# traveller59/second.pytorch

Measured on AMD Instinct MI355X. Metric: frames/sec VoxelNet fwd (car.fhd, ~16k active voxels), higher is better.
Workload: dtype bf16; 1 GPU; car.fhd.config VoxelNet forward (voxelise+VFE+SpMiddleFHD+RPNV2+rotated NMS), inference, batch=8 synthetic KITTI clouds/GPU (17000 pts, 16000 voxels each), random-init weights, inputs resident in HBM; parallelism=frame-dp1, launch_mode=graph, graph_branches=1, steps_in_flight=4, rpn_segments_serialized=True, rulebook_numbering=sorted, points_per_frame=17000

## Files before the change

include/second_hip.h:

```cpp
#ifndef SECOND_HIP_H
#define SECOND_HIP_H

#include <stddef.h>
#include <stdint.h>

#ifdef __cplusplus
extern "C" {
#endif

#define SEC_OK 0
#define SEC_E_INVALID -1
#define SEC_E_WORKSPACE -2
#define SEC_E_UNSUPPORTED -3
#define SEC_E_LAUNCH -4

#define SEC_F32 0
#define SEC_F16 1
#define SEC_BF16 2

#define SEC_ABI_VERSION 9
int sec_abi_version(void);
int sec_tensors_checksum(const void *const *h_ptrs, const long long *h_nbytes, int count, unsigned long long *sums, void *stream);
const char *sec_last_error(void);
const char *sec_last_kernel_name(void);

size_t sec_voxelize_workspace_bytes(int num_points, int batch, int max_voxels, int max_points);
int sec_simple_voxel_f32(const float *voxels, const int *num_points, int n, const int *num_dev, int max_points, int num_features,
                         int mean_features, void *mean, int mean_dtype, void *stream);
int sec_rows_differ_f32(const float *a, long long rows, const float *b, long long n, int *flag, void *stream);
int sec_voxelize_encode_f32(const float *points, const int *point_offsets, int num_points, int num_features,
                            int batch, const float *h_range6, const float *h_voxel_size3, int max_points,
                            int max_voxels, int cap_mode, float *voxels, int *coors,
                            int *num_points_per_voxel, int *voxel_offsets, void *mean, int mean_features,
                            int mean_dtype, int encoder, int out_pitch, void *workspace, size_t workspace_bytes, void *stream);
int sec_simple_voxel_radius_f32(const float *voxels, const int *num_points, int n, const int *num_dev, int max_points, int num_features,
                                int mean_features, void *out, int out_pitch, int out_dtype, void *stream);
int sec_voxelize_f32(const float *points, const int *point_offsets, int num_points, int num_features,
                     int batch, const float *h_range6, const float *h_voxel_size3, int max_points,
                     int max_voxels, int cap_mode, float *voxels, int *coors,
                     int *num_points_per_voxel, int *voxel_offsets, void *mean, int mean_features,
                     int mean_dtype, void *workspace, size_t workspace_bytes, void *stream);

size_t sec_rulebook_workspace_bytes(int n_in, int kvol, int max_out_per_in);


int sec_rulebook_subm3d(const int *indices, int n_in, const int *n_in_dev, int batch,
                        const int *h_shape3, const int *h_ksize3, const int *h_dilation3, int *nbr_out,
                        int *pairs, int *pair_num, void *workspace, size_t workspace_bytes,
                        void *stream);

int sec_rulebook_subm3d_after_conv(const int *indices, int n_in, const int *n_in_dev, int batch,
                                   const int *h_shape3, const int *h_ksize3, const int *h_dilation3,
                                   int *nbr_out, const void *conv_workspace, size_t conv_workspace_bytes,
                                   int conv_n_in, const int *h_conv_ksize3, const int *h_conv_stride3,
                                   const int *h_conv_dilation3, int conv_out_per_in_hint, void *stream);

int sec_rulebook_subm3d_after_voxelize(const int *indices, int n_in, const int *n_in_dev, int batch,
                                       const int *h_shape3, const int *h_ksize3, const int *h_dilation3,
                                       int *nbr_out, const void *vox_workspace, size_t vox_workspace_bytes,
                                       int vox_num_points, int vox_max_voxels, int vox_max_points,
                                       const int *h_vox_grid3_zyx, void *stream);

int sec_rulebook_conv3d_build(const int *indices, int n_in, const int *n_in_dev, int batch,
                              const int *h_in_shape3,
                              const int *h_out_shape3, const int *h_ksize3, const int *h_stride3,
                              const int *h_padding3, const int *h_dilation3, int *out_indices,
                              int out_cap, int *num_out, int out_per_in_hint, int *prefill_nbr_out,
                              int prefill_nbr_out_rows, int *prefill_nbr_in, void *workspace,
                              size_t workspace_bytes, void *stream);
int sec_rulebook_conv3d_tables(int n_in, const int *h_ksize3, const int *h_stride3,
                               const int *h_dilation3, int out_per_in_hint, int *nbr_out,
                               int nbr_out_rows, int *nbr_in, int prefilled, int *pairs, int *pair_num,
                               void *workspace, size_t workspace_bytes, void *stream);
size_t sec_rulebook_sorted_workspace_bytes(int n_in, int kvol, int batch, const int *h_out_shape3);
int sec_rulebook_conv3d_build_sorted(const int *indices, int n_in, const int *n_in_dev, int batch,
                                     const int *h_in_shape3, const int *h_out_shape3, const int *h_ksize3,
                                     const int *h_stride3, const int *h_padding3, const int *h_dilation3,
                                     int *out_indices, int out_cap, int *num_out, int *prefill_nbr_out,
                                     int prefill_nbr_out_rows, int *prefill_nbr_in,
                                     int *prefill_extra, long long prefill_extra_words,
                                     const void *in_sites_workspace, size_t in_sites_workspace_bytes,
                                     void *workspace, size_t workspace_bytes, void *stream);
int sec_rulebook_conv3d_tables_sorted(const int *indices, int n_in, const int *n_in_dev, int batch,
                                      const int *h_in_shape3, const int *h_out_shape3, const int *h_ksize3,
                                      const int *h_stride3, const int *h_padding3, const int *h_dilation3,
                                      int *nbr_out, int nbr_out_rows, int *nbr_in, int prefilled, int *out_indices,
                                      int out_cap, int *pairs, int *pair_num, void *workspace,
                                      size_t workspace_bytes, void *stream);
int sec_rulebook_subm3d_after_conv_sorted(const int *indices, int n_in, const int *n_in_dev, int batch,
                                          const int *h_shape3, const int *h_ksize3, const int *h_dilation3,
                                          int *nbr_out, int prefilled, const void *conv_workspace,
                                          size_t conv_workspace_bytes, void *stream);
void sec_conv_output_shape(const int *h_in_shape3, const int *h_ksize3, const int *h_stride3,
                           const int *h_padding3, const int *h_dilation3, int *h_out_shape3);

size_t sec_packed_weight_bytes(int kvol, int cin, int cout, int dtype);
size_t sec_packed_weight_x3_bytes(int kvol, int cin, int cout);
int sec_pack_conv_weight(const void *weight, int kvol, int cin, int cout, int dtype, void *packed,
                         void *stream);
int sec_indice_conv_fwd(const void *features, int n_in, int cin, const void *weight,
                        const void *packed_weight, int kvol, int cout, const int *nbr_out, int n_out,
                        const int *num_out_dev, const float *scale, const float *shift, int relu,
                        void *out, int dtype, int out_dtype, void *stream);
int sec_indice_conv_fwd_plan(int cin, int cout, int kvol, int n_out, int dtype, int out_dtype, int has_packed);
int sec_indice_conv_set_variant(int variant);
#define SEC_FP32_SPLIT16 0
#define SEC_FP32_EXACT 1
int sec_set_fp32_mode(int mode);
int sec_get_fp32_mode(void);
size_t sec_indice_conv_bwd_workspace_bytes(int kvol, int cin, int cout, int dtype);
int sec_indice_conv_bwd(const void *features, int n_in, int cin, const void *weight, int kvol, int cout,
                        const int *nbr_out, const int *nbr_in, int n_out, const void *dout,
                        void *dfeat, float *dweight, int dtype, void *workspace, size_t workspace_bytes,
                        const void *packed_dgrad, int dweight_zeroed, void *stream);
int sec_pack_conv_weight_train(const float *weight, int kvol, int cin, int cout, int subm, int dtype, void *weight16,
                               void *packed_fwd, void *packed_dgrad, float *zero_dweight, void *stream);
int sec_pack_conv_weight_train_multi(int n, const float *const *weights, const int *kvol, const int *cin, const int *cout,
                                     const int *subm, int dtype, void *const *weight16, void *const *packed_fwd,
                                     void *const *packed_dgrad, float *const *zero_dweight, void *stream);

int sec_sparse_to_dense(const void *features, const int *indices, int n, int c, const int *num_dev,
                        void *out, size_t out_elems, int64_t stride_b, int64_t stride_c,
                        int64_t stride_z, int64_t stride_y, int64_t stride_x, int dtype, void *stream);

int sec_sparse_site_map(const int *indices, int n, const int *num_dev, int batch, int d, int h, int w,
                        int *site_map, void *stream);
int sec_sparse_site_map_sorted(const void *conv_workspace, size_t conv_workspace_bytes, const int *num_dev, int rows_cap,
                               int batch, int d, int h, int w, int *site_map, void *stream);
size_t sec_rulebook_chain_workspace_bytes(int batch, int levels, const int *h_shapes);
int sec_rulebook_chain_sorted(const int *indices0, int n0, const int *n0_dev, int batch, int levels, const int *h_shapes,
                              const int *h_ksize, const int *h_stride, const int *h_pad, const int *h_out_cap,
                              int *const *h_nbr_out, int *const *h_out_indices, int *const *h_num_out,
                              int *const *h_subm_nbr, const void *vox_workspace, size_t vox_workspace_bytes,
                              int vox_num_points, int vox_max_voxels, int vox_max_points, const int *h_vox_grid3_zyx,
                              int *site_map, void *workspace, size_t workspace_bytes, void *stream);
int sec_conv2d_nhwc_gather(const void *features, long long feature_rows, const int *site_map, int batch, int h,
                           int w, const void *packed_weight, const float *bias, int cout, int relu,
                           const unsigned short *tile_order, const int *live_counts, const void *background, void *y,
                           int dtype, void *stream);

int sec_conv2d_nhwc_into(const void *x, int batch, int h, int w, int cin, const void *packed_weight, const float *bias, int cout,
                         int ksize, int stride, int pad, int relu, void *y, int y_channels, int y_channel_offset, int dtype, void *stream);

int sec_conv2d_nhwc_rows(const void *rows, long long feature_rows, const int *site_map, int batch, int h, int w, int cin,
                         const void *packed_weight, const float *bias, int cout, int ksize, int stride, int pad, int relu, void *y,
                         int dtype, void *stream);

size_t sec_rpn_tile_live_workspace_bytes(int batch, int h, int w);
int sec_rpn_tile_live(const int *site_map, int batch, int h, int w, int layers, unsigned short *tile_order, int *live_counts,
                      void *workspace, size_t workspace_bytes, void *stream);
int sec_conv2d_nhwc_tiles(const void *x, int batch, int h, int w, const void *packed_weight, const float *bias, int cout,
                          int relu, const unsigned short *tile_order, const int *live_counts, const void *background, void *y,
                          int dtype, void *stream);
int sec_conv1x1_chain_nhwc_tiles(const void *x, int batch, int h, int w, const void *packed_w1, const float *bias1, int relu1,
                                 const void *packed_w2, const float *bias2, int cout2, const unsigned short *tile_order,
                                 const int *live_counts, const void *background, void *y, int dtype, void *stream);
#define SEC_CHAIN_X_LIVE_ONLY 2
int sec_rpn_tile_live_masks(const int *site_map, int batch, int h, int w, int layers, unsigned short *tile_order, int *live_counts,
                            unsigned short *nbr_masks, void *workspace, size_t workspace_bytes, void *stream);
int sec_conv2d_nhwc_tiles_lazy(const void *x, int batch, int h, int w, const void *packed_weight, const float *bias, int cout,
                               int relu, const unsigned short *tile_order, const int *live_counts, const void *background,
                               const unsigned short *nbr_masks, const void *background_in, void *y, int dtype, void *stream);
int sec_conv2d_nhwc_tiles_tail(const void *x, int batch, int h, int w, const void *packed_weight, const float *bias, int relu,
                               const unsigned short *tile_order, const int *live_counts, const unsigned short *nbr_masks,
                               const void *background_in, const void *packed_w1, const float *bias1, int relu1, const void *packed_w2,
                               const float *bias2, int cout2, void *y_heads, int dtype, void *stream);

size_t sec_rpn_tile_cover_lds_bytes(int h, int w, int layers);
int sec_rpn_tile_cover(const int *site_map, int batch, int h, int w, int layers, unsigned short *tile_order, int *live_counts,
                       unsigned short *cover_order, int *cover_counts, unsigned *cover_cols, unsigned *cover_halo, void *workspace,
                       size_t workspace_bytes, void *stream);
int sec_conv2d_nhwc_gather_cover(const void *features, long long feature_rows, const int *site_map, int batch, int h, int w,
                                 const void *packed_weight, const float *bias, int cout, int relu, const unsigned short *cover_order,
                                 const int *cover_counts, void *y, int dtype, void *stream);
int sec_conv2d_nhwc_tiles_cover(const void *x, int batch, int h, int w, const void *packed_weight, const float *bias, int cout,
                                int relu, const unsigned short *cover_order, const int *cover_counts, const unsigned *cover_halo,
                                const void *background_in, void *y, int dtype, void *stream);
int sec_conv2d_nhwc_tiles_tail_cover(const void *x, int batch, int h, int w, const void *packed_weight, const float *bias, int relu,
                                     const unsigned short *cover_order, const int *cover_counts, const unsigned *cover_halo,
                                     const void *background_in, const void *packed_w1, const float *bias1, int relu1,
                                     const void *packed_w2, const float *bias2, int cout2, void *y_heads, int dtype, void *stream);

int sec_dense_to_sparse(const void *dense, const int *indices, int n, int c, const int *num_dev, void *rows,
                        int64_t stride_b, int64_t stride_c, int64_t stride_z, int64_t stride_y,
                        int64_t stride_x, int dtype, void *stream);

int sec_pillar_scatter(const void *features, const int *coords, int p, int c, const int *num_dev,
                       void *out, size_t out_elems, int64_t stride_b, int64_t stride_c, int64_t stride_y,
                       int64_t stride_x, int dtype, void *stream);

int sec_pfn_fwd(const float *voxels, const int *num_points, const int *coords, int num_pillars,
                const int *num_dev, int max_points, int num_features, const float *weight_t,
                const float *scale, const float *shift, int channels, float vx, float vy,
                float x_offset, float y_offset, void *out, int out_dtype, void *stream);
int sec_pfn_fwd_slots(const float *points, const void *vox_workspace, size_t vox_workspace_bytes, int vox_num_points,
                      int vox_batch, int vox_max_voxels, int max_points, int num_features, const int *num_points_per_voxel,
                      const int *coords, int num_pillars, const int *num_dev, const float *weight_t, const float *scale,
                      const float *shift, int channels, float vx, float vy, float x_offset, float y_offset, void *out,
                      int out_dtype, void *stream);
int sec_pfn_radius_fwd(const float *voxels, const int *num_points, const int *coords, int num_pillars,
                       const int *num_dev, int max_points, int num_features, const float *weight_t,
                       const float *scale, const float *shift, int channels, float vx, float vy,
                       float x_offset, float y_offset, void *out, int out_dtype, void *stream);
int sec_pfn_radius_fwd_slots(const float *points, const void *vox_workspace, size_t vox_workspace_bytes, int vox_num_points,
                             int vox_batch, int vox_max_voxels, int max_points, int num_features, const int *num_points_per_voxel,
                             const int *coords, int num_pillars, const int *num_dev, const float *weight_t, const float *scale,
                             const float *shift, int channels, float vx, float vy, float x_offset, float y_offset, void *out,
                             int out_dtype, void *stream);

size_t sec_pfn_train_workspace_bytes(int num_pillars, int channels);
int sec_pfn_train_fwd(const float *voxels, const int *num_points, const int *coords, int num_pillars, int max_points,
                      int num_features, const float *weight_t, const float *gamma, const float *beta, float eps, float momentum,
                      float *running_mean, float *running_var, int channels, float vx, float vy, float x_offset, float y_offset,
                      float *out, signed char *argmax, float *stats, void *workspace, size_t workspace_bytes, void *stream);
int sec_pfn_train_bwd(const float *voxels, const int *num_points, const int *coords, int num_pillars, int max_points,
                      int num_features, const float *weight_t, const float *gamma, const float *stats, int channels, float vx,
                      float vy, float x_offset, float y_offset, const float *grad_out, const float *out, const signed char *argmax,
                      float *dweight_t, float *dgamma, float *dbeta, void *workspace, size_t workspace_bytes, void *stream);
// ... 306 lines not shown
```

second.pytorch_amd/csrc/indice_conv.hip:

```cpp
#include "common.hpp"
#include <stdlib.h>
#include <type_traits>

namespace sec {

template <typename T> struct Cvt;
template <> struct Cvt<float> {
    static __device__ __forceinline__ float to(float v) { return v; }
    static __device__ __forceinline__ float from(float v) { return v; }
};
template <> struct Cvt<__half> {
    static __device__ __forceinline__ float to(__half v) { return __half2float(v); }
    static __device__ __forceinline__ __half from(float v) { return __float2half_rn(v); }
};
template <> struct Cvt<__hip_bfloat16> {
    static __device__ __forceinline__ float to(__hip_bfloat16 v) { return __bfloat162float(v); }
    static __device__ __forceinline__ __hip_bfloat16 from(float v) { return __float2bfloat16(v); }
};

__device__ __forceinline__ float epilogue(float v, const float *scale, const float *shift, int c, int relu) {
    if (scale) v = __fmul_rn(v, scale[c]);
    if (shift) v = __fadd_rn(v, shift[c]);
    if (relu) v = v > 0.0f ? v : 0.0f;
    return v;
// ... 412 lines not shown
    static constexpr int ASLOT = 32 * LPR, BSLOT = BPIECES * 64;
    static constexpr int RING = 3;
};

typedef float f32x2p __attribute__((ext_vector_type(2)));
template <typename T> __device__ __forceinline__ unsigned pack2_16(float a, float b);
template <> __device__ __forceinline__ unsigned pack2_16<__hip_bfloat16>(float a, float b) {
    typedef __bf16 bf16x2p __attribute__((ext_vector_type(2)));
    const f32x2p v = {a, b};
    return __builtin_bit_cast(unsigned, __builtin_convertvector(v, bf16x2p));
}
template <> __device__ __forceinline__ unsigned pack2_16<__half>(float a, float b) {
    typedef _Float16 f16x2p __attribute__((ext_vector_type(2)));
    const f32x2p v = {a, b};
    return __builtin_bit_cast(unsigned, __builtin_convertvector(v, f16x2p));
}

template <typename T, int COUT, bool FUSED>
__device__ __forceinline__ void rows_store_impl(f32x16 (&acc)[(COUT + 31) / 32], T *__restrict__ out, long long row, bool valid, int h,
                                                const float *__restrict__ aff, bool has_scale, bool has_shift, int relu) {
    if (FUSED) { has_scale = has_shift = true; relu = 1; }
    constexpr int NT = (COUT + 31) / 32, NG = COUT >= 32 ? 4 : COUT / 8;
    static_assert(COUT % 16 == 0, "whole 16-byte runs per half-wave pair");
    T *orow = out + (size_t)row * COUT;
    float4 sc4[NT][NG], sh4[NT][NG];
#pragma unroll
    for (int t = 0; t < NT; ++t)
#pragma unroll
        for (int g = 0; g < NG; ++g) {
            const int c = t * 32 + 8 * g + 4 * h;
            if (has_scale) sc4[t][g] = *reinterpret_cast<const float4 *>(aff + c);
            if (has_shift) sh4[t][g] = *reinterpret_cast<const float4 *>(aff + COUT + c);
        }
#pragma unroll
    for (int t = 0; t < NT; ++t) {
        unsigned lo[NG], hi[NG];
#pragma unroll
        for (int g = 0; g < NG; ++g) {
            const float sc[4] = {sc4[t][g].x, sc4[t][g].y, sc4[t][g].z, sc4[t][g].w};
            const float sh[4] = {sh4[t][g].x, sh4[t][g].y, sh4[t][g].z, sh4[t][g].w};
            float v4[4];
#pragma unroll
            for (int j = 0; j < 4; ++j) v4[j] = epilogue_v(acc[t][4 * g + j], sc[j], sh[j], has_scale, has_shift, relu);
            lo[g] = pack2_16<T>(v4[0], v4[1]);
            hi[g] = pack2_16<T>(v4[2], v4[3]);
        }
#pragma unroll
        for (int pr = 0; pr < NG / 2; ++pr) {
            const auto sx = __builtin_amdgcn_permlane32_swap(lo[2 * pr], lo[2 * pr + 1], false, false);
            const auto sy = __builtin_amdgcn_permlane32_swap(hi[2 * pr], hi[2 * pr + 1], false, false);
            if (valid) *reinterpret_cast<uint4 *>(orow + t * 32 + 8 * (2 * pr + h)) = make_uint4(sx[0], sy[0], sx[1], sy[1]);
        }
    }
}
template <typename T, int COUT>
__device__ __forceinline__ void rows_store(f32x16 (&acc)[(COUT + 31) / 32], T *__restrict__ out, long long row, bool valid, int h,
                                           const float *__restrict__ aff, bool has_scale, bool has_shift, int relu) {
    if (has_scale && has_shift && relu) rows_store_impl<T, COUT, true>(acc, out, row, valid, h, aff, true, true, 1);
    else rows_store_impl<T, COUT, false>(acc, out, row, valid, h, aff, has_scale, has_shift, relu);
}

template <int COUT>
__device__ __forceinline__ void rows_stage_affine(float *aff, const float *__restrict__ scale, const float *__restrict__ shift) {
    const int c = threadIdx.x;
    if (c < COUT) {
        if (scale) aff[c] = scale[c];
        if (shift) aff[COUT + c] = shift[c];
    }
}

#ifdef SEC_CONV_TIMELINE
#define SEC_RTL(...) __VA_ARGS__
#else
#define SEC_RTL(...)
#endif

#ifdef SEC_CONV_EXPERIMENTS
#include "../../tools/kernel_experiments/indice_conv_rows_ab.inc"
#endif

typedef unsigned int u32x4_t __attribute__((ext_vector_type(4)));
constexpr int kBalWgs = 256;
enum : int {
    kFlStage = 1, kFlPipe = 2, kFlSkew = 32, kFlAllW = 64, kFlLazy = 128, kFlWin3 = 512, kFlBal = 2048, kFlXsh = 8192,
    kFlAblNoGather = 4, kFlAblFewLines = 8, kFlAblOneLine = 16, kFlAblNoWeights = 4096,
};
#if defined(__HIP_DEVICE_COMPILE__) && defined(SEC_PACKED_F32_EXEMPTION)
#define SEC_PACKED_F32_OK __attribute__((target("packed-fp32-ops")))
#else
#define SEC_PACKED_F32_OK
#endif
template <int CTRL> __device__ __forceinline__ int rows_lane_shift(int v) {
    return __builtin_amdgcn_mov_dpp(v, CTRL, 0xf, 0xf, true);
}
constexpr int kDppWaveShl1 = 0x130, kDppWaveShr1 = 0x138;
template <bool LEFT> __device__ __forceinline__ bool rows_xshare(int t, int c, int r) {
    const int n = rows_lane_shift<LEFT ? kDppWaveShr1 : kDppWaveShl1>(c);
    return t >= 0 && t == n && (LEFT ? r > 0 : r < 31);
}
template <typename T, int CIN, int COUT, int KVOL, int DIST, int WAVES, int MINW, int FL>
SEC_PACKED_F32_OK __global__ __launch_bounds__(WAVES * 64, MINW) void k_conv_rows_buf(const T *__restrict__ feat, long long feat_bytes,
                                                                   const T *__restrict__ packed, const int *__restrict__ nbr,
                                                                   int n_out, const int *__restrict__ num_out_dev,
                                                                   const float *__restrict__ scale, const float *__restrict__ shift,
                                                                   int relu, T *__restrict__ out) {
    using C = RowsCfg<T, CIN, COUT>;
    constexpr int NBW = (C::BPIECES + WAVES - 1) / WAVES;
    constexpr int ROWB = CIN * (int)sizeof(T);
    constexpr bool STAGE = (FL & kFlStage) != 0, PIPE = (FL & kFlPipe) != 0;
    constexpr bool ALLW = (FL & kFlAllW) != 0;
    constexpr bool LAZY = (FL & kFlLazy) != 0 && STAGE && !ALLW;
    constexpr bool SKEW = (FL & kFlSkew) != 0 && WAVES == 8 && PIPE;
    const bool early = SKEW && __builtin_amdgcn_readfirstlane((int)threadIdx.x >> 8) != 0;
    constexpr int TBL16 = 32 * KVOL / 4;
    static_assert(NBW >= 1 && NBW <= 2, "one or two weight pieces per wave");
    static_assert(C::KS <= 4, "up to four 16-channel k-steps per row");
    static_assert(!STAGE || (32 * KVOL) % 4 == 0, "tile table in whole 16-byte pieces");
    static_assert(!ALLW || (STAGE && PIPE), "the all-weights form stages its tables and double-buffers its B fragments");
    constexpr bool WIN3 = (FL & kFlWin3) != 0;
    constexpr bool XSH = (FL & kFlXsh) != 0 && STAGE && KVOL == 27 && DIST >= 3 && (ALLW || (WIN3 && LAZY));
    static_assert(!WIN3 || (STAGE && !PIPE && !ALLW && KVOL % 3 == 0 && DIST <= 3), "window form: non-pipelined, 3 offsets per window");
    constexpr int LBUF = ALLW ? (KVOL * C::BSLOT > WAVES * TBL16 ? KVOL * C::BSLOT : WAVES * TBL16) : 1;
    __shared__ __attribute__((aligned(16))) uint4 lbuf[LBUF];
    __shared__ __attribute__((aligned(16))) uint4 bring[ALLW ? 1 : (WIN3 ? 6 : 3)][ALLW ? 1 : C::BSLOT];
    __shared__ __attribute__((aligned(16))) float aff[2 * COUT];
    __shared__ __attribute__((aligned(16))) u32x4_t stage[(STAGE && !ALLW) ? WAVES : 1][(STAGE && !ALLW) ? TBL16 : 1];
    rows_stage_affine<COUT>(aff, scale, shift);
    const int n_cap = n_out;
    if (num_out_dev) n_out = *num_out_dev;
    const int lane = threadIdx.x & 63, w = threadIdx.x >> 6;
    const int r = lane & 31, h = lane >> 5;
    constexpr bool BAL = (FL & kFlBal) != 0;
    int rw = 32;
    if constexpr (BAL) {
        const int per_wg = (n_out + kBalWgs - 1) / kBalWgs;
        rw = ((per_wg + WAVES - 1) / WAVES + 3) & ~3;
        rw = rw < 4 ? 4 : (rw > 32 ? 32 : rw);
    }
    int bid = blockIdx.x;
    if (relu & 0x10000) {
        const int nact = (int)(((long long)n_out + rw * WAVES - 1) / (rw * WAVES));
        const int per = (nact + 7) >> 3;
        bid = (bid & 7) * per + (bid >> 3);
        if ((int)(blockIdx.x >> 3) >= per) return;
    }
    relu &= 1;
    if ((long long)bid * (rw * WAVES) >= n_out) return;
    const long long row = (long long)bid * (rw * WAVES) + w * rw + r;
    const bool valid = row < n_out && r < rw;
    SEC_RTL(long long *tl = g_timeline; long long tl0 = 0, tl1 = 0, tl2 = 0; if (tl) tl0 = clock64();)
    const __amdgpu_buffer_rsrc_t rsrc = __builtin_amdgcn_make_buffer_rsrc(const_cast<T *>(feat), 0, (int)feat_bytes, 0x00020000);
    const int piece0 = (w * NBW) % C::BPIECES;
    const u32x4_t *wpv = reinterpret_cast<const u32x4_t *>(packed) + (size_t)piece0 * 64 + lane;
    unsigned off[KVOL];
    unsigned shm = 0;
    if constexpr (STAGE) {
        const long long tile_row0 = (long long)bid * (rw * WAVES) + w * rw;
        const long long tbl_bytes = (long long)n_cap * KVOL * 4;
        const int *tile = nbr + tile_row0 * KVOL;
        const long long left = tbl_bytes - tile_row0 * KVOL * 4;
        const __amdgpu_buffer_rsrc_t trs = __builtin_amdgcn_make_buffer_rsrc(
            const_cast<int *>(left > 0 ? tile : nbr), 0, (int)(left <= 0 ? 0 : (left < 32 * KVOL * 4 ? left : 32 * KVOL * 4)), 0x00020000);
        u32x4_t *stg = ALLW ? reinterpret_cast<u32x4_t *>(lbuf) + w * TBL16 : &stage[w][0];
#pragma unroll
        for (int i = 0; i < (TBL16 + 63) / 64; ++i) {
            const int p16 = i * 64 + lane;
            if (p16 < TBL16) stg[p16] = __builtin_amdgcn_raw_buffer_load_b128(trs, p16 * 16, 0, 0);
        }
        __builtin_amdgcn_wave_barrier();
        const int *mine = reinterpret_cast<const int *>(stg) + r * KVOL;
        if constexpr (!LAZY) {
#pragma unroll
            for (int k = 0; k < KVOL; ++k) {
                int t = valid ? mine[k] : -1;
                if constexpr (XSH) {
                    if (k % 3 != 1) {
                        const int c = valid ? mine[k - k % 3 + 1] : -1;
                        if (k % 3 == 0 ? rows_xshare<true>(t, c, r) : rows_xshare<false>(t, c, r)) { shm |= 1u << (2 * (k / 3) + (k % 3) / 2); t = -1; }
                    }
                }
                off[k] = t >= 0 ? (unsigned)t * ROWB + h * 16 : 0x80000000u;
            }
        }
    } else {
        const int *nrow = nbr + (size_t)(valid ? row : 0) * KVOL;
#pragma unroll
        for (int k = 0; k < KVOL; ++k) {
            const int t = valid ? nrow[k] : -1;
            off[k] = t >= 0 ? (unsigned)t * ROWB + h * 16 : 0x80000000u;
        }
    }
#ifdef SEC_CONV_ABLATIONS
    if constexpr ((FL & kFlAblNoGather) != 0) {
#pragma unroll
        for (int k = 0; k < KVOL; ++k) off[k] = 0x80000000u;
    }
    if constexpr ((FL & kFlAblFewLines) != 0) {
#pragma unroll
        for (int k = 0; k < KVOL; ++k) off[k] = (unsigned)__shfl((int)off[k], lane & ~3, 64);
    }
    if constexpr ((FL & kFlAblOneLine) != 0) {
#pragma unroll
        for (int k = 0; k < KVOL; ++k) off[k] = h * 16;
    }
#endif
    SEC_RTL(if (tl) { cwait_vmcnt<0>(); tl1 = clock64(); })
    f32x16 acc[C::NT];
#pragma unroll
    for (int t = 0; t < C::NT; ++t)
#pragma unroll
        for (int i = 0; i < 16; ++i) acc[t][i] = 0.0f;
    u32x4_t areg[DIST][C::KS];
    auto afrag = [&](int k, int s) __attribute__((always_inline)) -> uint4 {
        u32x4_t a = areg[k % DIST][s];
        if constexpr (XSH) {
            if (k % 3 != 1) {
                const bool sh = ((shm >> (2 * (k / 3) + (k % 3) / 2)) & 1u) != 0;
                const u32x4_t c = areg[(k - k % 3 + 1) % DIST][s];
#pragma unroll
                for (int i = 0; i < 4; ++i) {
                    const int n = k % 3 == 0 ? rows_lane_shift<kDppWaveShr1>((int)c[i]) : rows_lane_shift<kDppWaveShl1>((int)c[i]);
                    a[i] = sh ? (unsigned)n : a[i];
                }
            }
        }
        return __builtin_bit_cast(uint4, a);
    };
#define SEC_XSH_REFILL(k, FETCH)                                                                                      \
    if constexpr (XSH) {                                                                                              \
        if ((k) % 3 == 0) { if ((k) + DIST < KVOL) FETCH((k) + DIST) }                                                \
        else if ((k) % 3 == 2) {                                                                                      \
            if ((k) - 1 + DIST < KVOL) FETCH((k) - 1 + DIST)                                                          \
            if ((k) + DIST < KVOL) FETCH((k) + DIST)                                                                  \
        }                                                                                                             \
    } else {                                                                                                          \
        if ((k) + DIST < KVOL) FETCH((k) + DIST)                                                                      \
    }
    if constexpr (ALLW) {
#define SEC_FETCH_A(k)                                                                                                \
    {                                                                                                                 \
        areg[(k) % DIST][0] = __builtin_amdgcn_raw_buffer_load_b128(rsrc, off[k], 0, 0);                              \
        if (C::KS > 1) areg[(k) % DIST][1 % C::KS] = __builtin_amdgcn_raw_buffer_load_b128(rsrc, off[k] + 32, 0, 0);  \
        if (C::KS > 2) areg[(k) % DIST][2 % C::KS] = __builtin_amdgcn_raw_buffer_load_b128(rsrc, off[k] + 64, 0, 0);  \
        if (C::KS > 3) areg[(k) % DIST][3 % C::KS] = __builtin_amdgcn_raw_buffer_load_b128(rsrc, off[k] + 96, 0, 0);  \
    }
#pragma unroll
        for (int k = 0; k < DIST && k < KVOL; ++k) SEC_FETCH_A(k)
        __syncthreads();
        {
            const uint4 *pk = reinterpret_cast<const uint4 *>(packed);
            for (int i = threadIdx.x; i < KVOL * C::BSLOT; i += WAVES * 64) lbuf[i] = pk[i];
        }
        __syncthreads();
        uint4 bf[2][C::KS * C::NT];
#pragma unroll
        for (int i = 0; i < C::KS * C::NT; ++i) bf[0][i] = lbuf[i * 64 + lane];
#pragma unroll
        for (int k = 0; k < KVOL; ++k) {
            if (k + 1 < KVOL) {
#pragma unroll
                for (int i = 0; i < C::KS * C::NT; ++i) bf[(k + 1) & 1][i] = lbuf[(k + 1) * C::BSLOT + i * 64 + lane];
            }
            __builtin_amdgcn_sched_barrier(0);
#pragma unroll
            for (int s = 0; s < C::KS; ++s) {
                const uint4 a = afrag(k, s);
#pragma unroll
                for (int t = 0; t < C::NT; ++t) acc[t] = Mfma<T>::run(bf[k & 1][s * C::NT + t], a, acc[t]);
            }
            __builtin_amdgcn_sched_barrier(0);
            SEC_XSH_REFILL(k, SEC_FETCH_A)
        }
#undef SEC_FETCH_A
        SEC_RTL(if (tl) tl2 = clock64();)
        rows_store<T, COUT>(acc, out, row, valid, h, aff, scale != nullptr, shift != nullptr, relu);
        return;
    }
    u32x4_t wr0[DIST], wr1[DIST];
    u32x4_t *bslot = reinterpret_cast<u32x4_t *>(&bring[0][piece0 * 64 + lane]);
    const int *lazy_tbl = reinterpret_cast<const int *>(&stage[(STAGE && !ALLW) ? w : 0][0]) + r * KVOL;
    auto off_of = [&](int k) -> unsigned {
        if constexpr (LAZY) {
            int t = valid ? lazy_tbl[k] : -1;
            if constexpr (XSH) {
                if (k % 3 != 1) {
                    const int c = valid ? lazy_tbl[k - k % 3 + 1] : -1;
                    if (k % 3 == 0 ? rows_xshare<true>(t, c, r) : rows_xshare<false>(t, c, r)) { shm |= 1u << (2 * (k / 3) + (k % 3) / 2); t = -1; }
                }
            }
#ifdef SEC_CONV_ABLATIONS
            if constexpr ((FL & kFlAblNoGather) != 0) return 0x80000000u;
            if constexpr ((FL & kFlAblOneLine) != 0) return t >= 0 ? (unsigned)(h * 16) : 0x80000000u;
#endif
            return t >= 0 ? (unsigned)t * ROWB + h * 16 : 0x80000000u;
        } else {
            return off[k];
        }
    };
#define SEC_FETCH(k)                                                                                                  \
    {                                                                                                                 \
        const unsigned o_ = off_of(k);                                                                                \
        wr0[(k) % DIST] = wpv[(size_t)(k) * C::BSLOT];                                                                \
        if (NBW > 1) wr1[(k) % DIST] = wpv[(size_t)(k) * C::BSLOT + 64];                                              \
        areg[(k) % DIST][0] = __builtin_amdgcn_raw_buffer_load_b128(rsrc, o_, 0, 0);                                  \
        if (C::KS > 1) areg[(k) % DIST][1 % C::KS] = __builtin_amdgcn_raw_buffer_load_b128(rsrc, o_ + 32, 0, 0);      \
        if (C::KS > 2) areg[(k) % DIST][2 % C::KS] = __builtin_amdgcn_raw_buffer_load_b128(rsrc, o_ + 64, 0, 0);      \
        if (C::KS > 3) areg[(k) % DIST][3 % C::KS] = __builtin_amdgcn_raw_buffer_load_b128(rsrc, o_ + 96, 0, 0);      \
    }
#define SEC_WPUT(k)                                                                                                   \
    {                                                                                                                 \
        bslot[((k) % 3) * C::BSLOT] = wr0[(k) % DIST];                                                                \
        if (NBW > 1) bslot[((k) % 3) * C::BSLOT + 64] = wr1[(k) % DIST];                                              \
    }
    if constexpr (!(WIN3 && XSH)) {
#pragma unroll
        for (int k = 0; k < DIST && k < KVOL; ++k) SEC_FETCH(k)
    }
    SEC_RTL(long long ts_wait = 0, ts_comp = 0, ts_issue = 0;)
    if constexpr (WIN3) {
        u32x4_t ww0[3], ww1[3];
#define SEC_GFETCH(k)                                                                                                 \
    {                                                                                                                 \
        const unsigned o_ = off_of(k);                                                                                \
        areg[(k) % DIST][0] = __builtin_amdgcn_raw_buffer_load_b128(rsrc, o_, 0, 0);                                  \
        if (C::KS > 1) areg[(k) % DIST][1 % C::KS] = __builtin_amdgcn_raw_buffer_load_b128(rsrc, o_ + 32, 0, 0);      \
        if (C::KS > 2) areg[(k) % DIST][2 % C::KS] = __builtin_amdgcn_raw_buffer_load_b128(rsrc, o_ + 64, 0, 0);      \
        if (C::KS > 3) areg[(k) % DIST][3 % C::KS] = __builtin_amdgcn_raw_buffer_load_b128(rsrc, o_ + 96, 0, 0);      \
    }
#ifdef SEC_CONV_ABLATIONS
#define SEC_WLOAD(g)                                                                                                  \
    {                                                                                                                 \
        _Pragma("unroll") for (int j_ = 0; j_ < 3; ++j_) {                                                            \
            if constexpr ((FL & kFlAblNoWeights) != 0) { ww0[j_] = u32x4_t{(unsigned)lane, 0u, 0u, 0u}; if (NBW > 1) ww1[j_] = ww0[j_]; }  \
            else {                                                                                                    \
            ww0[j_] = wpv[(size_t)(3 * (g) + j_) * C::BSLOT];                                                         \
            if (NBW > 1) ww1[j_] = wpv[(size_t)(3 * (g) + j_) * C::BSLOT + 64];                                       \
            }                                                                                                         \
        }                                                                                                             \
    }
#else
#define SEC_WLOAD(g)                                                                                                  \
    {                                                                                                                 \
        _Pragma("unroll") for (int j_ = 0; j_ < 3; ++j_) {                                                            \
            ww0[j_] = wpv[(size_t)(3 * (g) + j_) * C::BSLOT];                                                         \
            if (NBW > 1) ww1[j_] = wpv[(size_t)(3 * (g) + j_) * C::BSLOT + 64];                                       \
        }                                                                                                             \
    }
#endif
#define SEC_WSTORE(g)                                                                                                 \
    {                                                                                                                 \
        _Pragma("unroll") for (int j_ = 0; j_ < 3; ++j_) {                                                            \
            bslot[((((g) & 1) * 3) + j_) * C::BSLOT] = ww0[j_];                                                       \
            if (NBW > 1) bslot[((((g) & 1) * 3) + j_) * C::BSLOT + 64] = ww1[j_];                                     \
        }                                                                                                             \
    }
        SEC_WLOAD(0)
#pragma unroll
        for (int k = 0; k < DIST && k < KVOL; ++k) SEC_GFETCH(k)
        SEC_WSTORE(0)
        if (KVOL > 3) SEC_WLOAD(1)
#pragma unroll
        for (int g = 0; g < KVOL / 3; ++g) {
            __syncthreads();
#pragma unroll
            for (int j = 0; j < 3; ++j) {
                const int k = 3 * g + j;
                uint4 bf[C::KS * C::NT];
#pragma unroll
                for (int i = 0; i < C::KS * C::NT; ++i) bf[i] = bring[(g & 1) * 3 + j][i * 64 + lane];
                __builtin_amdgcn_sched_barrier(0);
#pragma unroll
                for (int s2 = 0; s2 < C::KS; ++s2) {
                    const uint4 a = afrag(k, s2);
#pragma unroll
                    for (int t = 0; t < C::NT; ++t) acc[t] = Mfma<T>::run(bf[s2 * C::NT + t], a, acc[t]);
                }
                __builtin_amdgcn_sched_barrier(0);
                SEC_XSH_REFILL(k, SEC_GFETCH)
            }
            if (g + 1 < KVOL / 3) {
                SEC_WSTORE(g + 1)
                if (g + 2 < KVOL / 3) SEC_WLOAD(g + 2)
            }
        }
#undef SEC_GFETCH
#undef SEC_WLOAD
#undef SEC_WSTORE
    } else if constexpr (!PIPE) {
        SEC_WPUT(0)
#pragma unroll
        for (int k = 0; k < KVOL; ++k) {
            SEC_RTL(long long s0 = 0, s1 = 0, s2 = 0; if (tl) s0 = clock64();)
            if (k + 1 < KVOL) SEC_WPUT(k + 1)
            __syncthreads();
            SEC_RTL(if (tl) s1 = clock64();)
            uint4 bf[C::KS * C::NT];
#pragma unroll
            for (int i = 0; i < C::KS * C::NT; ++i) bf[i] = bring[k % 3][i * 64 + lane];
            __builtin_amdgcn_sched_barrier(0);
#pragma unroll
            for (int s = 0; s < C::KS; ++s) {
                const uint4 a = __builtin_bit_cast(uint4, areg[k % DIST][s]);
#pragma unroll
                for (int t = 0; t < C::NT; ++t) acc[t] = Mfma<T>::run(bf[s * C::NT + t], a, acc[t]);
            }
            __builtin_amdgcn_sched_barrier(0);
            SEC_RTL(if (tl) s2 = clock64();)
            if (k + DIST < KVOL) SEC_FETCH(k + DIST)
            SEC_RTL(if (tl) { const long long s3 = clock64(); ts_wait += s1 - s0; ts_comp += s2 - s1; ts_issue += s3 - s2; })
        }
    } else {
        static_assert(!PIPE || DIST >= 3, "W[k+2] must have left the ring before its registers are refilled");
        uint4 bf[2][C::KS * C::NT];
        SEC_WPUT(0)
        if (KVOL > 1) SEC_WPUT(1)
        __syncthreads();
#pragma unroll
        for (int i = 0; i < C::KS * C::NT; ++i) bf[0][i] = bring[0][i * 64 + lane];
#pragma unroll
        for (int k = 0; k < KVOL; ++k) {
            if (k + 2 < KVOL) SEC_WPUT(k + 2)
            if (k + 1 < KVOL) {
                __syncthreads();
#pragma unroll
                for (int i = 0; i < C::KS * C::NT; ++i) bf[(k + 1) & 1][i] = bring[(k + 1) % 3][i * 64 + lane];
            }
            __builtin_amdgcn_sched_barrier(0);
            if constexpr (SKEW) {
                if (early && k >= 1 && k - 1 + DIST < KVOL) SEC_FETCH(k - 1 + DIST)
                __builtin_amdgcn_sched_barrier(0);
            }
#pragma unroll
            for (int s = 0; s < C::KS; ++s) {
                const uint4 a = __builtin_bit_cast(uint4, areg[k % DIST][s]);
#pragma unroll
                for (int t = 0; t < C::NT; ++t) acc[t] = Mfma<T>::run(bf[k & 1][s * C::NT + t], a, acc[t]);
            }
            __builtin_amdgcn_sched_barrier(0);
            if (!(SKEW && early) && k + DIST < KVOL) SEC_FETCH(k + DIST)
// ... 77 lines not shown
        const u32x4_t *wp = reinterpret_cast<const u32x4_t *>(packed) + lane;
        typedef unsigned int u32x2_t __attribute__((ext_vector_type(2)));
        u32x4_t bfr[7];
        u32x2_t lo[7], hi[7];
#pragma unroll
        for (int s = 0; s < 7; ++s) {
            bfr[s] = wp[s * 64];
            const int k0 = 4 * s + 2 * h, k1 = k0 + 1;
            const int t0 = valid ? mine[k0] : -1;
            const int t1 = (valid && k1 < KVOL) ? mine[k1 < KVOL ? k1 : 0] : -1;
            lo[s] = __builtin_amdgcn_raw_buffer_load_b64(rsrc, t0 >= 0 ? (unsigned)t0 * 8u : 0x80000000u, 0, 0);
            hi[s] = __builtin_amdgcn_raw_buffer_load_b64(rsrc, t1 >= 0 ? (unsigned)t1 * 8u : 0x80000000u, 0, 0);
        }
        f32x16 acc[1];
#pragma unroll
        for (int i = 0; i < 16; ++i) acc[0][i] = 0.0f;
#pragma unroll
        for (int s = 0; s < 7; ++s) {
            const uint4 a = make_uint4(lo[s].x, lo[s].y, hi[s].x, hi[s].y);
            acc[0] = Mfma<T>::run(__builtin_bit_cast(uint4, bfr[s]), a, acc[0]);
        }
        __syncthreads();
        rows_store<T, COUT>(acc, out, row, valid, h, aff, scale != nullptr, shift != nullptr, relu);
    } else {
        __syncthreads();
    }
}

enum ConvVariant : int {
    kVarWave = 0,
    kVarAuto = 1,
    kVarSks = 8,
    kVarRows = 22,
    kVarAutoPlain = 29,
    kVarF32Valu = 30,
    kVarF32Mfma = 31,
    kVarF32SplitUnpacked = 32,
    kVarWgradCompact = 41,
    kVarXshOffAuto = 80, kVarXshOnAuto = 81,
    kVarXshOffRows = 82, kVarXshOnRows = 83,
};
static int g_variant_override = -1;
static int g_fp32_mode = 0;

struct ConvSetting { int variant, xshare; };
static ConvSetting conv_setting() {
    switch (g_variant_override) {
    case kVarXshOffAuto: return {kVarAuto, 0};
    case kVarXshOnAuto: return {kVarAuto, 1};
    case kVarXshOffRows: return {kVarRows, 0};
    case kVarXshOnRows: return {kVarRows, 1};
    default: break;
    }
    static int env = -2;
    if (env == -2) { const char *e = getenv("SEC_CONV_XSHARE"); env = e ? (atoi(e) != 0) : -1; }
    return {g_variant_override < 0 ? kVarAuto : g_variant_override, env};
}
static int conv_variant() { return conv_setting().variant; }

enum { PLAN_GENERIC = 0, PLAN_TILED = 1, PLAN_C4 = 2, PLAN_MFMA_WAVE = 3, PLAN_MFMA_SK = 4, PLAN_MFMA_SKS = 5, PLAN_ROWS = 6,
       PLAN_ROWS_COMPACT = 7, PLAN_ROWS_TOUCH = 8, PLAN_ROWS_COMPACT_TOUCH = 9, PLAN_ROWS_REG = 10, PLAN_ROWS_BUF = 11, PLAN_C4_MFMA = 12, PLAN_ROWS_M2 = 13, PLAN_ROWS_LDS = 14, PLAN_ROWS_KS = 15, PLAN_EXPERIMENT = 99 };

#define SEC_MFMA_SHAPES(X) X(16, 16) X(16, 32) X(32, 32) X(32, 64) X(64, 64) X(64, 128) X(128, 128) X(16, 64) X(64, 32) X(32, 16) X(128, 64)
static bool mfma_shape(int cin, int cout) {
#define SEC_IS(CI, CO) if (cin == CI && cout == CO) return true;
    SEC_MFMA_SHAPES(SEC_IS)
#undef SEC_IS
    return false;
}

constexpr int kRowsMin = 40000, kRowsMinSmall = 8192;

constexpr bool rows_shape_narrow(int cin, int cout) { return (cin == 16 && (cout == 16 || cout == 32)) || (cin == 32 && cout == 32); }
constexpr bool rows_shape_wide(int cin, int cout) { return cin == 32 && cout == 64; }
constexpr bool rows_shape_64(int cin, int cout) { return cin == 64 && cout == 64; }
constexpr bool buf_shape(int cin, int cout, int kvol) {
    if (kvol == 3) return rows_shape_64(cin, cout);
    return kvol == 27 && (rows_shape_narrow(cin, cout) || rows_shape_wide(cin, cout) || rows_shape_64(cin, cout));
}
constexpr int kFlNarrow = kFlStage + kFlPipe + kFlAllW + kFlBal;
constexpr int kFlWide = kFlStage + kFlPipe + kFlBal;
constexpr int kFl64 = kFlStage + kFlLazy + kFlWin3 + kFlBal;
constexpr int kFl64K3 = kFlStage + kFlPipe;
static_assert(kFlNarrow == 2115 && kFlNarrow + kFlXsh == 10307 && kFlWide == 2051 && kFl64 == 2689 && kFl64 + kFlXsh == 10881 && kFl64K3 == 3,
              "the decimal FL values are part of the kernel names that tests and bench tables quote");
constexpr bool kXshare32 = true, kXshare64w8 = true, kXshare64w4 = false;
enum RowsForm : int { kRowsNone = 0, kRowsNarrow, kRowsNarrowXsh, kRowsWide, kRows64W8, kRows64W8Xsh, kRows64W4, kRows64W4Xsh, kRows64K3 };

static int rows_form(int cin, int cout, int kvol, bool mid, int xshare) {
    auto xsh = [&](bool dflt) { return xshare < 0 ? dflt : xshare != 0; };
    if (kvol == 3) return kRows64K3;
    if (rows_shape_narrow(cin, cout)) return cin == 32 && xsh(kXshare32) ? kRowsNarrowXsh : kRowsNarrow;
    if (rows_shape_wide(cin, cout)) return kRowsWide;
    if (mid) return xsh(kXshare64w4) ? kRows64W4Xsh : kRows64W4;
    return xsh(kXshare64w8) ? kRows64W8Xsh : kRows64W8;
}

struct ConvPlan { int id, form; };
#ifdef SEC_CONV_EXPERIMENTS
#include "../../tools/kernel_experiments/indice_conv_dispatch.inc"
#endif

static ConvPlan conv_fwd_decide(int cin, int cout, int kvol, int rows, bool same_dtype, bool has_packed, bool has_feat, long long feat_bytes,
                                int variant, int xshare) {
    const bool fits = feat_bytes < 0x7fffffffll;
    if (!has_packed) return {PLAN_GENERIC, kRowsNone};
    if (cin == 4 && cout == 16 && kvol == 27)
        return {same_dtype && variant != kVarAutoPlain && fits ? PLAN_C4_MFMA : PLAN_GENERIC, kRowsNone};
    if (!mfma_shape(cin, cout)) return {PLAN_GENERIC, kRowsNone};
    ConvPlan p = {PLAN_MFMA_SK, kRowsNone};
    if (variant == kVarSks || ((variant == kVarAuto || variant == kVarAutoPlain) && cout <= 32)) p.id = PLAN_MFMA_SKS;
    else if (variant == kVarWave) p.id = PLAN_MFMA_WAVE;
    if (same_dtype && has_feat && fits && buf_shape(cin, cout, kvol)) {
        const bool mid = rows_shape_64(cin, cout) && kvol == 27 && rows >= kRowsMinSmall && rows < kRowsMin;
        if (variant == kVarRows || (variant == kVarAuto && (rows >= kRowsMin || mid)))
            p = {PLAN_ROWS_BUF, rows_form(cin, cout, kvol, variant == kVarAuto && mid, xshare)};
    }
#ifdef SEC_CONV_EXPERIMENTS
    experiment_plan(cin, cout, kvol, rows, same_dtype, has_feat, fits, variant, xshare, &p);
#endif
    return p;
}
static ConvPlan conv_fwd_plan_now(int cin, int cout, int kvol, int rows, bool same_dtype, bool has_packed, bool has_feat, long long feat_bytes) {
    const ConvSetting cs = conv_setting();
    return conv_fwd_decide(cin, cout, kvol, rows, same_dtype, has_packed, has_feat, feat_bytes, cs.variant, cs.xshare);
}

template <typename T, int CIN, int COUT>
static bool launch_rows_form(int form, const void *feat, long long n_feat, const void *packed, const int *nbr, int n_out, const int *num_out_dev,
                             const float *scale, const float *shift, int relu, void *out, hipStream_t st) {
#define SEC_FORM(FORM, SHAPE, KV, D, W, M, FLG)                                                                                  \
    case FORM:                                                                                                                   \
        if constexpr (SHAPE) {                                                                                                   \
            launch_rows_buf<T, CIN, COUT, D, W, M, FLG, KV>(feat, n_feat, packed, nbr, n_out, num_out_dev, scale, shift, relu, out, st); \
            return true;                                                                                                         \
        }                                                                                                                        \
        break;
    switch (form) {
    SEC_FORM(kRowsNarrow, rows_shape_narrow(CIN, COUT), 27, 6, 8, 2, kFlNarrow)
    SEC_FORM(kRowsNarrowXsh, rows_shape_narrow(CIN, COUT) && CIN == 32, 27, 6, 8, 2, kFlNarrow + kFlXsh)
    SEC_FORM(kRowsWide, rows_shape_wide(CIN, COUT), 27, 4, 8, 2, kFlWide)
    SEC_FORM(kRows64W8, rows_shape_64(CIN, COUT), 27, 3, 8, 3, kFl64)
    SEC_FORM(kRows64W8Xsh, rows_shape_64(CIN, COUT), 27, 3, 8, 3, kFl64 + kFlXsh)
    SEC_FORM(kRows64W4, rows_shape_64(CIN, COUT), 27, 3, 4, 2, kFl64)
    SEC_FORM(kRows64W4Xsh, rows_shape_64(CIN, COUT), 27, 3, 4, 2, kFl64 + kFlXsh)
    SEC_FORM(kRows64K3, rows_shape_64(CIN, COUT), 3, 3, 8, 2, kFl64K3)
    default: break;
    }
#undef SEC_FORM
    return false;
}

template <typename T, typename OT, int CIN, int COUT>
static void launch_mfma(const ConvPlan &p, const void *feat, long long n_feat, const void *packed, const int *nbr, int n_out,
                        const int *num_out_dev, int kvol, const float *scale, const float *shift, int relu, void *out, hipStream_t st) {
#ifdef SEC_CONV_EXPERIMENTS
    if (experiment_launch<T, OT, CIN, COUT>(p, feat, n_feat, packed, nbr, n_out, num_out_dev, kvol, scale, shift, relu, out, st)) return;
#endif
    if constexpr (std::is_same<T, OT>::value && buf_shape(CIN, COUT, 27)) {
        if (p.id == PLAN_ROWS_BUF && launch_rows_form<T, CIN, COUT>(p.form, feat, n_feat, packed, nbr, n_out, num_out_dev, scale, shift, relu, out, st))
            return;
    }
    if (p.id == PLAN_MFMA_SKS) {
        hipLaunchKernelGGL((k_conv_mfma_sks<T, OT, CIN, COUT, 4>), dim3((div_up(n_out, 32) + 7) / 8 * 8, (COUT + 31) / 32),
                           dim3(256), 0, st, (const T *)feat, (const T *)packed, nbr, n_out, num_out_dev, kvol, scale, shift,
                           relu, (OT *)out);
        return;
    }
    if (p.id == PLAN_MFMA_WAVE) {
        constexpr int MT = 1;
        int rows_per_block = (kBlock / 64) * 32 * MT;
        hipLaunchKernelGGL((k_conv_mfma<T, OT, CIN, COUT, MT>), dim3(div_up(n_out, rows_per_block)), dim3(kBlock), 0, st,
                           (const T *)feat, (const T *)packed, nbr, n_out, num_out_dev, kvol, scale, shift, relu, (OT *)out);
        return;
    }
    constexpr int NW = 4;
    hipLaunchKernelGGL((k_conv_mfma_sk<T, OT, CIN, COUT, NW>), dim3((div_up(n_out, 32) + 7) / 8 * 8), dim3(NW * 64), 0, st,
                       (const T *)feat, (const T *)packed, nbr, n_out, num_out_dev, kvol, scale, shift,
                       relu | kReluXcdOrder, (OT *)out);
}

template <typename T, typename OT>
static bool dispatch_mfma(const ConvPlan &p, int cin, int cout, const void *feat, long long n_feat, const void *packed, const int *nbr,
                          int n_out, const int *num_out_dev, int kvol, const float *scale, const float *shift, int relu, void *out,
                          hipStream_t st) {
    if (p.id == PLAN_GENERIC || p.id == PLAN_C4_MFMA) return false;
#define SEC_CASE(CI, CO)                                                                                         \
    if (cin == CI && cout == CO) {                                                                               \
        launch_mfma<T, OT, CI, CO>(p, feat, n_feat, packed, nbr, n_out, num_out_dev, kvol, scale, shift, relu, out, st); \
        return true;                                                                                             \
    }
    SEC_MFMA_SHAPES(SEC_CASE)
#undef SEC_CASE
    return false;
}

template <int CIN, int COUT, int WAVES>
__global__ __launch_bounds__(WAVES * 64) void k_conv_rows_x3_f32(const float *__restrict__ feat, const float *__restrict__ w,
                                                                const int *__restrict__ nbr, int n_out, const int *__restrict__ num_out_dev,
                                                                int kvol, int w_t, int mirror, const float *__restrict__ scale,
                                                                const float *__restrict__ shift, int relu, float *__restrict__ out) {
    static_assert(CIN % 16 == 0 && COUT % 32 == 0, "16-channel k-steps, 32-column MFMA tiles");
    constexpr int KS = CIN / 16, NT = COUT / 32, ROWS = WAVES * 32, NTH = WAVES * 64;
    constexpr int PIECES = KS * NT * 64;
    constexpr int PPT = (PIECES + NTH - 1) / NTH;
    __shared__ __attribute__((aligned(16))) uint4 sB[2][2][PIECES];
    __shared__ int s_nbr[ROWS * 27];
    if (num_out_dev) n_out = *num_out_dev;
    const int tid = threadIdx.x, wave = tid >> 6, lane = tid & 63, r = lane & 31, h = lane >> 5;
    const long long base = (long long)blockIdx.x * ROWS;
    if (base >= n_out) return;
    {
        const long long lim = ((long long)n_out - base) * kvol;
        const int *src = nbr + base * kvol;
        for (int e = tid; e < ROWS * kvol; e += NTH) s_nbr[e] = e < lim ? src[e] : -1;
    }
    float wreg[PPT][8];
    auto load_w = [&](int k) {
        const float *wk = w + (size_t)(mirror ? kvol - 1 - k : k) * CIN * COUT;
#pragma unroll
        for (int q = 0; q < PPT; ++q) {
            const int p = q * NTH + tid;
            if (PIECES % NTH != 0 && p >= PIECES) break;
            const int l = p & 63, st = p >> 6, t = st % NT, sidx = st / NT;
            const int ci = sidx * 16 + (l >> 5) * 8, co = t * 32 + (l & 31);
            if (w_t) {
                const float4 a = *reinterpret_cast<const float4 *>(wk + (size_t)co * CIN + ci);
                const float4 b = *reinterpret_cast<const float4 *>(wk + (size_t)co * CIN + ci + 4);
                wreg[q][0] = a.x; wreg[q][1] = a.y; wreg[q][2] = a.z; wreg[q][3] = a.w;
                wreg[q][4] = b.x; wreg[q][5] = b.y; wreg[q][6] = b.z; wreg[q][7] = b.w;
            } else {
#pragma unroll
                for (int e = 0; e < 8; ++e) wreg[q][e] = wk[(size_t)(ci + e) * COUT + co];
            }
        }
    };
    auto split8 = [](const float (&v)[8], uint4 &hi, uint4 &lo) {
        const unsigned h0 = pack2_16<__hip_bfloat16>(v[0], v[1]), h1 = pack2_16<__hip_bfloat16>(v[2], v[3]);
        const unsigned h2 = pack2_16<__hip_bfloat16>(v[4], v[5]), h3 = pack2_16<__hip_bfloat16>(v[6], v[7]);
        hi = make_uint4(h0, h1, h2, h3);
        lo = make_uint4(pack2_16<__hip_bfloat16>(v[0] - __uint_as_float(h0 << 16), v[1] - __uint_as_float(h0 & 0xffff0000u)),
                        pack2_16<__hip_bfloat16>(v[2] - __uint_as_float(h1 << 16), v[3] - __uint_as_float(h1 & 0xffff0000u)),
                        pack2_16<__hip_bfloat16>(v[4] - __uint_as_float(h2 << 16), v[5] - __uint_as_float(h2 & 0xffff0000u)),
                        pack2_16<__hip_bfloat16>(v[6] - __uint_as_float(h3 << 16), v[7] - __uint_as_float(h3 & 0xffff0000u)));
    };
    auto store_w = [&](int buf) {
#pragma unroll
        for (int q = 0; q < PPT; ++q) {
            const int p = q * NTH + tid;
            if (PIECES % NTH != 0 && p >= PIECES) break;
            uint4 hi, lo;
            split8(wreg[q], hi, lo);
            sB[buf][0][p] = hi;
            sB[buf][1][p] = lo;
        }
    };
    load_w(0);
    store_w(0);
    f32x16 acc[NT];
#pragma unroll
    for (int t = 0; t < NT; ++t)
#pragma unroll
        for (int i = 0; i < 16; ++i) acc[t][i] = 0.0f;
    float4 a[2 * KS], an[2 * KS];
    auto gather = [&](int k, float4 (&dst)[2 * KS]) -> bool {
        const int idx = s_nbr[(wave * 32 + r) * kvol + k];
        const bool any = __ballot(idx >= 0) != 0ull;
        if (any) {
            const float4 *row = reinterpret_cast<const float4 *>(feat + (size_t)(idx >= 0 ? idx : 0) * CIN) + 2 * h;
#pragma unroll
            for (int sidx = 0; sidx < KS; ++sidx) {
                dst[2 * sidx] = idx >= 0 ? row[4 * sidx] : make_float4(0.0f, 0.0f, 0.0f, 0.0f);
// ... 782 lines not shown
    if (cin == CI && cout == CO) {                                                                                        \
        set_last_kernel("k_conv_wgrad_tiled<%s, %d, %d> chunk=%d", dtype_name<T>(), CI, CO, chunk);                       \
        hipLaunchKernelGGL((k_conv_wgrad_tiled<T, CI, CO>), grid, dim3(kBlock), 0, st, (const T *)feat, (const T *)dout, nbr,  \
                           n_out, kvol, chunk, dw);                                                                       \
        return true;                                                                                                      \
    }
    SEC_WG(4, 16) SEC_WG(16, 16) SEC_WG(16, 32) SEC_WG(32, 32) SEC_WG(32, 64) SEC_WG(64, 64) SEC_WG(64, 128) SEC_WG(128, 128)
#undef SEC_WG
    return false;
}

static size_t elt_size(int dtype) { return dtype == SEC_F32 ? 4 : 2; }

}

using namespace sec;

#ifdef SEC_CONV_TIMELINE
extern "C" __attribute__((visibility("default"))) int sec__debug_timeline(long long *buf) {
    return hipMemcpyToSymbol(HIP_SYMBOL(sec::g_timeline), &buf, sizeof(buf)) == hipSuccess ? 0 : -4;
}
#endif

SEC_API size_t sec_packed_weight_bytes(int kvol, int cin, int cout, int dtype) {
    if (dtype != SEC_F32 && cin == 4 && cout == 16 && kvol == 27) return (size_t)7 * 64 * 8 * elt_size(dtype);
    if (dtype == SEC_F32 || cin % 16 != 0 || kvol <= 0 || cout <= 0) return 0;
    return (size_t)kvol * cin * ((cout + 31) / 32) * 32 * elt_size(dtype);
}

SEC_API int sec_pack_conv_weight(const void *weight, int kvol, int cin, int cout, int dtype, void *packed, void *stream) {
    if (!weight || !packed || sec_packed_weight_bytes(kvol, cin, cout, dtype) == 0) return SEC_E_INVALID;
    hipStream_t st = (hipStream_t)stream;
    if (cin == 4) {
        if (dtype == SEC_BF16)
            hipLaunchKernelGGL(k_pack_weight_c4<__hip_bfloat16>, dim3(div_up(7 * 64 * 8, kBlock)), dim3(kBlock), 0, st,
                               (const __hip_bfloat16 *)weight, cout, (__hip_bfloat16 *)packed);
        else
            hipLaunchKernelGGL(k_pack_weight_c4<__half>, dim3(div_up(7 * 64 * 8, kBlock)), dim3(kBlock), 0, st, (const __half *)weight, cout,
                               (__half *)packed);
        return check_launch();
    }
    long long total = (long long)kvol * cin * ((cout + 31) / 32) * 32;
    if (dtype == SEC_BF16)
        hipLaunchKernelGGL(k_pack_weight<__hip_bfloat16>, dim3(div_up(total, kBlock)), dim3(kBlock), 0, st,
                           (const __hip_bfloat16 *)weight, kvol, cin, cout, (__hip_bfloat16 *)packed);
    else
        hipLaunchKernelGGL(k_pack_weight<__half>, dim3(div_up(total, kBlock)), dim3(kBlock), 0, st, (const __half *)weight,
                           kvol, cin, cout, (__half *)packed);
    return check_launch();
}

SEC_API int sec_set_fp32_mode(int mode) {
    if (mode != 0 && mode != 1) return SEC_E_INVALID;
    g_fp32_mode = mode;
    return SEC_OK;
}
SEC_API int sec_get_fp32_mode(void) { return g_fp32_mode; }

SEC_API int sec_indice_conv_set_variant(int variant) {
    g_variant_override = variant;
    return SEC_OK;
}

SEC_API int sec_indice_conv_fwd_plan(int cin, int cout, int kvol, int n_out, int dtype, int out_dtype, int has_packed) {
    if (dtype != SEC_F32) {
        const ConvPlan p = conv_fwd_plan_now(cin, cout, kvol, n_out, out_dtype == dtype, has_packed != 0, true, -1);
        if (p.id != PLAN_GENERIC) return p.id;
    }
    if (cin == 4 && cout == 16 && (size_t)kvol * 4 * 16 * sizeof(float) <= 48 * 1024) return PLAN_C4;
    static const int tiled_shapes[][2] = {{16, 16}, {16, 32}, {32, 16}, {32, 32}, {32, 64}, {64, 32}, {64, 64}};
    for (auto &sh : tiled_shapes)
        if (sh[0] == cin && sh[1] == cout) return PLAN_TILED;
    return PLAN_GENERIC;
}

SEC_API size_t sec_packed_weight_x3_bytes(int kvol, int cin, int cout) {
    return x3p_shape(cin, cout, kvol) ? (size_t)kvol * 2 * cin * ((cout + 31) / 32 * 32) * 2 : 0;
}

SEC_API int sec_indice_conv_fwd(const void *features, int n_in, int cin, const void *weight, const void *packed_weight,
                                int kvol, int cout, const int *nbr_out, int n_out, const int *num_out_dev,
                                const float *scale, const float *shift, int relu, void *out, int dtype, int out_dtype,
                                void *stream) {
    if (n_in < 0 || n_out < 0 || cin <= 0 || cout <= 0 || kvol <= 0 || !weight) return SEC_E_INVALID;
    if (dtype < 0 || dtype > 2 || (out_dtype != dtype && out_dtype != SEC_F32)) return SEC_E_UNSUPPORTED;
    if (n_out == 0) return SEC_OK;
    if (!nbr_out || !out || (n_in > 0 && !features)) return SEC_E_INVALID;
    hipStream_t st = (hipStream_t)stream;
    bool done = false;
    ConvPlan p = {PLAN_GENERIC, kRowsNone};
    if (dtype != SEC_F32)
        p = conv_fwd_plan_now(cin, cout, kvol, n_out, out_dtype == dtype, packed_weight != nullptr, features != nullptr, (long long)n_in * cin * 2);
    if (p.id == PLAN_C4_MFMA) {
        const long long fb = (long long)n_in * 8;
        const int c4_xcd = rows_xcd_order();
        const int c4_blocks = c4_xcd ? (div_up(n_out, 128) + 7) / 8 * 8 : div_up(n_out, 128);
        const int c4_relu = (relu & 1) | (c4_xcd << 16);
        if (dtype == SEC_BF16)
            hipLaunchKernelGGL((k_conv_c4_mfma<__hip_bfloat16, 16>), dim3(c4_blocks), dim3(kBlock), 0, st, (const __hip_bfloat16 *)features,
                               fb, (const __hip_bfloat16 *)packed_weight, nbr_out, n_out, num_out_dev, scale, shift, c4_relu, (__hip_bfloat16 *)out);
        else
            hipLaunchKernelGGL((k_conv_c4_mfma<__half, 16>), dim3(c4_blocks), dim3(kBlock), 0, st, (const __half *)features, fb,
                               (const __half *)packed_weight, nbr_out, n_out, num_out_dev, scale, shift, c4_relu, (__half *)out);
        return check_launch();
    }
    if (p.id != PLAN_GENERIC) {
        if (dtype == SEC_BF16) {
            done = out_dtype == SEC_F32
                       ? dispatch_mfma<__hip_bfloat16, float>(p, cin, cout, features, n_in, packed_weight, nbr_out, n_out, num_out_dev, kvol, scale, shift, relu, out, st)
                       : dispatch_mfma<__hip_bfloat16, __hip_bfloat16>(p, cin, cout, features, n_in, packed_weight, nbr_out, n_out, num_out_dev, kvol, scale, shift, relu, out, st);
        } else {
            done = out_dtype == SEC_F32
                       ? dispatch_mfma<__half, float>(p, cin, cout, features, n_in, packed_weight, nbr_out, n_out, num_out_dev, kvol, scale, shift, relu, out, st)
                       : dispatch_mfma<__half, __half>(p, cin, cout, features, n_in, packed_weight, nbr_out, n_out, num_out_dev, kvol, scale, shift, relu, out, st);
        }
    }
    if (!done && packed_weight && dtype == SEC_F32 && out_dtype == SEC_F32 && conv_variant() != kVarF32Valu && conv_variant() != kVarF32Mfma &&
        conv_variant() != kVarF32SplitUnpacked && g_fp32_mode == 0)
        done = launch_x3p(features, n_in, packed_weight, nbr_out, n_out, num_out_dev, cin, cout, kvol, scale, shift, relu, out, st);
    if (!done) {
#define SEC_GEN(T, OT) launch_generic<T, OT>(features, weight, nbr_out, n_out, num_out_dev, cin, cout, kvol, scale, shift, relu, out, st)
        if (dtype == SEC_F32) SEC_GEN(float, float);
        else if (dtype == SEC_BF16) { if (out_dtype == SEC_F32) SEC_GEN(__hip_bfloat16, float); else SEC_GEN(__hip_bfloat16, __hip_bfloat16); }
        else { if (out_dtype == SEC_F32) SEC_GEN(__half, float); else SEC_GEN(__half, __half); }
#undef SEC_GEN
    }
    return check_launch();
}

template <typename T>
__device__ __forceinline__ void pack_weight_train_at(long long g, const float *__restrict__ w, int kvol, int cin, int cout, int mirror,
                                                     T *__restrict__ w16, T *__restrict__ packed, long long total_fwd,
                                                     T *__restrict__ packed_t, long long total_t, float *__restrict__ zero_dw) {
    const long long total0 = (long long)kvol * cin * cout;
    if (g < total0) w16[g] = Cvt<T>::from(w[g]);
    if (zero_dw && g < total0) zero_dw[g] = 0.0f;
    const int e = (int)(g & 7), lane = (int)((g >> 3) & 63);
    if (packed && g < total_fwd) {
        if (cin == 4) {
            const int s_ = (int)(g >> 9);
            const int K = s_ * 16 + (lane >> 5) * 8 + e, kk = K >> 2, ci = K & 3, c = lane & 31;
            packed[g] = (kk < 27 && c < cout) ? Cvt<T>::from(w[((size_t)kk * 4 + ci) * cout + c]) : Cvt<T>::from(0.0f);
        } else {
            const int ks = cin / 16, nt = (cout + 31) / 32;
            long long q = g >> 9;
            const int t = (int)(q % nt);
            q /= nt;
            const int sidx = (int)(q % ks), k = (int)(q / ks);
            const int ci = sidx * 16 + (lane >> 5) * 8 + e, co = t * 32 + (lane & 31);
            packed[g] = co < cout ? Cvt<T>::from(w[((size_t)k * cin + ci) * cout + co]) : Cvt<T>::from(0.0f);
        }
    }
    if (packed_t && g < total_t) {
        const int ks = cout / 16, nt = (cin + 31) / 32;
        long long q = g >> 9;
        const int t = (int)(q % nt);
        q /= nt;
        const int sidx = (int)(q % ks), k = (int)(q / ks);
        const int co = sidx * 16 + (lane >> 5) * 8 + e, ci = t * 32 + (lane & 31);
        const int km = mirror ? kvol - 1 - k : k;
        packed_t[g] = ci < cin ? Cvt<T>::from(w[((size_t)km * cin + ci) * cout + co]) : Cvt<T>::from(0.0f);
    }
}

template <typename T>
__global__ __launch_bounds__(kBlock) void k_pack_weight_train(const float *__restrict__ w, int kvol, int cin, int cout, int mirror,
                                                             T *__restrict__ w16, T *__restrict__ packed, long long total_fwd,
                                                             T *__restrict__ packed_t, long long total_t, float *__restrict__ zero_dw) {
    pack_weight_train_at<T>((long long)blockIdx.x * kBlock + threadIdx.x, w, kvol, cin, cout, mirror, w16, packed, total_fwd, packed_t, total_t, zero_dw);
}

constexpr int kPackMulti = 16;
struct PackSparseDesc {
    const float *w;
    void *w16, *packed, *packed_t;
    float *zero_dw;
    long long total_fwd, total_t;
    int kvol, cin, cout, mirror, blk0;
};
struct PackSparseArgs {
    PackSparseDesc d[kPackMulti];
    int n;
};
template <typename T>
__global__ __launch_bounds__(kBlock) void k_pack_weight_train_multi(PackSparseArgs a) {
    int i = 0;
    while (i + 1 < a.n && (int)blockIdx.x >= a.d[i + 1].blk0) ++i;
    const PackSparseDesc &d = a.d[i];
    pack_weight_train_at<T>((long long)(blockIdx.x - d.blk0) * kBlock + threadIdx.x, d.w, d.kvol, d.cin, d.cout, d.mirror, (T *)d.w16, (T *)d.packed,
                            d.total_fwd, (T *)d.packed_t, d.total_t, d.zero_dw);
}

template <typename T>
static int run_bwd(const void *features, int n_in, int cin, const void *weight, int kvol, int cout, const int *nbr_out,
                   const int *nbr_in, int n_out, const void *dout, void *dfeat, float *dweight, void *workspace,
                   size_t workspace_bytes, int dtype, hipStream_t st, const void *packed_dgrad = nullptr, bool dweight_zeroed = false) {
    int rc;
// ... 107 lines not shown
```

second.pytorch_amd/csrc/rulebook.hip:

```cpp
#include "common.hpp"

namespace sec {

constexpr int kMaxKvol = 128;

struct RbGeom {
    int in_shape[3], out_shape[3], ksize[3], stride[3], pad[3], dil[3];
    int kvol, n_in, batch;
    int cand[3], ncand;
    uint32_t mask;
};

__device__ __forceinline__ unsigned long long cell_key(int b, int z, int y, int x, const int *shape) {
    unsigned long long vol = (unsigned long long)shape[0] * shape[1] * shape[2];
    return (unsigned long long)b * vol + ((unsigned long long)z * shape[1] + y) * shape[2] + x;
}

__device__ __forceinline__ int live_rows(const RbGeom &g, const int *n_dev) {
    if (!n_dev) return g.n_in;
    int n = *n_dev;
    return n < g.n_in ? n : g.n_in;
}

__global__ __launch_bounds__(kBlock) void k_rb_init(unsigned long long *__restrict__ a, long long na, unsigned long long va,
// ... 651 lines not shown
    int r = prefix8[blk];
    const unsigned w[8] = {a.x, a.y, a.z, a.w, b.x, b.y, b.z, b.w};
    unsigned word = 0u;
#pragma unroll
    for (int q = 0; q < 8; ++q) {
        word = wi == (unsigned)q ? w[q] : word;
        r += wi > (unsigned)q ? __popc(w[q]) : 0;
    }
    return (word & bit) ? r + __popc(word & (bit - 1u)) : -1;
}

__global__ __launch_bounds__(kBlock) void k_bm_site_map(const unsigned *__restrict__ bm, const int *__restrict__ prefix8,
                                                       const int *__restrict__ num_dev, int rows_cap, long long cells,
                                                       int *__restrict__ map) {
    const long long i = (long long)blockIdx.x * kBlock + threadIdx.x;
    if (i >= cells) return;
    int rows = num_dev ? *num_dev : rows_cap;
    if (rows > rows_cap) rows = rows_cap;
    const int r = bm_rank(bm, prefix8, (unsigned)i);
    map[i] = (r >= 0 && r < rows) ? r + 1 : 0;
}

template <int GEO>
__global__ __launch_bounds__(kBlock) void k_bm_tables(const int *__restrict__ indices, RbGeom g, const int *__restrict__ n_dev,
                                                     const unsigned *__restrict__ bm, const int *__restrict__ prefix,
                                                     int *__restrict__ nbr_in, int *__restrict__ nbr_out, int nbr_out_rows,
                                                     int *__restrict__ out_indices, int out_cap) {
    using G = Geo<GEO>;
    const int ncand = G::fixed ? G::NCAND : g.ncand, kvol = G::fixed ? G::KVOL : g.kvol;
    long long t = (long long)blockIdx.x * kBlock + threadIdx.x;
    if (t >= (long long)g.n_in * ncand) return;
    const int j = (int)(t / ncand), c = (int)(t % ncand);
    if (j >= live_rows(g, n_dev)) return;
    const int4 q = *reinterpret_cast<const int4 *>(indices + (size_t)j * 4);
    int k, out[3];
    unsigned lin;
    if (!bm_candidate<GEO>(g, q, c, &k, &lin, out)) return;
    const int o = bm_rank(bm, prefix, lin);
    if (o < 0) return;
    if (nbr_in) nbr_in[(size_t)j * kvol + k] = o;
    if (o < nbr_out_rows) nbr_out[(size_t)o * kvol + k] = j;
    if (out_indices && o < out_cap) *reinterpret_cast<int4 *>(out_indices + (size_t)o * 4) = make_int4(q.x, out[0], out[1], out[2]);
}

template <bool K3>
__global__ __launch_bounds__(kBlock) void k_subm_nbr_bm(const int *__restrict__ indices, RbGeom g, const int *__restrict__ n_dev,
                                                       const unsigned *__restrict__ bm, const int *__restrict__ prefix,
                                                       int *__restrict__ nbr) {
    if (K3) { g.kvol = 27; g.ksize[0] = g.ksize[1] = g.ksize[2] = 3; }
    const int half = K3 ? 13 : g.kvol / 2;
    long long t = (long long)blockIdx.x * kBlock + threadIdx.x;
    if (t >= (long long)live_rows(g, n_dev) * (half + 1)) return;
    int o = (int)(t / (half + 1)), k = (int)(t % (half + 1));
    if (k == half) { nbr[(size_t)o * g.kvol + half] = o; return; }
    int kx = K3 ? k % 3 : k % g.ksize[2], ky = K3 ? (k / 3) % 3 : (k / g.ksize[2]) % g.ksize[1],
        kz = K3 ? k / 9 : k / (g.ksize[2] * g.ksize[1]);
    int4 c = *reinterpret_cast<const int4 *>(indices + (size_t)o * 4);
    int z = c.y + (kz - g.ksize[0] / 2) * g.dil[0];
    int y = c.z + (ky - g.ksize[1] / 2) * g.dil[1];
    int x = c.w + (kx - g.ksize[2] / 2) * g.dil[2];
    if (z >= 0 && z < g.in_shape[0] && y >= 0 && y < g.in_shape[1] && x >= 0 && x < g.in_shape[2]) {
        const unsigned lin = (((unsigned)c.x * g.in_shape[0] + z) * g.in_shape[1] + y) * g.in_shape[2] + x;
        const int j = bm_rank(bm, prefix, lin);
        if ((unsigned)j < (unsigned)g.n_in) {
            nbr[(size_t)o * g.kvol + k] = j;
            nbr[(size_t)j * g.kvol + (g.kvol - 1 - k)] = o;
        }
    }
}


constexpr int kChainMaxLevels = 6;
struct ChainLevel {
    int shape[3];
    int ksize[3], pad[3];
    int geo, kvol;
    int out_cap;
    long long n_words;
    unsigned *bm;
    int *prefix8;
    unsigned long long *status;
    int tile0, ntiles, wpt64;
    int *nbr_out, *out_indices, *num_out, *subm_nbr;
    int sblk0, sblks, cblk0, cblks;
    int eblk0, eblks;
};
struct ChainParams {
    ChainLevel lv[kChainMaxLevels + 1];
    int levels, batch;
    int n0;
    const int *indices0, *n0_dev;
    int *ticket;
    int cand_blks, map_blk0;
    int *site_map;
    long long map_cells;
};

__device__ __forceinline__ int chain_live0(const ChainParams &P) {
    if (!P.n0_dev) return P.n0;
    const int n = *P.n0_dev;
    return n < P.n0 ? n : P.n0;
}

__global__ __launch_bounds__(kBlock) void k_chain_front(const int *__restrict__ indices, RbGeom gs, RbGeom gc, const int *__restrict__ n_dev,
                                                       const unsigned long long *__restrict__ keys, const int *__restrict__ svid,
                                                       int *__restrict__ subm0, unsigned *__restrict__ bm1, int nb_subm, int nb_set,
                                                       int *__restrict__ fill, long long fill_words) {
    const int grp = blockIdx.x / 10, role = blockIdx.x % 10;
    const int blk = role < 7 ? grp * 7 + role : role < 9 ? nb_subm + grp * 2 + (role - 7) : nb_subm + nb_set + grp;
    if (role < 7 ? blk >= nb_subm : role < 9 ? blk >= nb_subm + nb_set : false) return;
    if (blk < nb_subm) {
        const long long t = (long long)blk * kBlock + threadIdx.x;
        if (t >= (long long)live_rows(gs, n_dev) * 14) return;
        const int o = (int)(t / 14), k = (int)(t % 14);
        if (k == 13) { subm0[(size_t)o * 27 + 13] = o; return; }
        const int kx = k % 3, ky = (k / 3) % 3, kz = k / 9;
        const int4 c = *reinterpret_cast<const int4 *>(indices + (size_t)o * 4);
        const int z = c.y + kz - 1, y = c.z + ky - 1, x = c.w + kx - 1;
        if (z >= 0 && z < gs.in_shape[0] && y >= 0 && y < gs.in_shape[1] && x >= 0 && x < gs.in_shape[2]) {
            const int s = hash_find(keys, gs.mask, cell_key(c.x, z, y, x, gs.in_shape));
            const int j = s >= 0 ? svid[s] : -1;
            if ((unsigned)j < (unsigned)gs.n_in) {
                subm0[(size_t)o * 27 + k] = j;
                subm0[(size_t)j * 27 + (26 - k)] = o;
            }
        }
        return;
    }
    if (blk < nb_subm + nb_set) {
        const long long t = (long long)(blk - nb_subm) * kBlock + threadIdx.x;
        if (t >= (long long)gc.n_in * 4) return;
        const int j = (int)(t >> 2), c = (int)(t & 3);
        if (j >= live_rows(gc, n_dev)) return;
        const int4 q = *reinterpret_cast<const int4 *>(indices + (size_t)j * 4);
        int kz, ky, oz, oy;
        if (!cand_offset_fixed<3, 2>(q.y, gc.pad[0], gc.out_shape[0], c >> 1, &kz, &oz)) return;
        if (!cand_offset_fixed<3, 2>(q.z, gc.pad[1], gc.out_shape[1], c & 1, &ky, &oy)) return;
        int kx, ox0, ox1;
        const bool v0 = cand_offset_fixed<3, 2>(q.w, gc.pad[2], gc.out_shape[2], 0, &kx, &ox0);
        const bool v1 = cand_offset_fixed<3, 2>(q.w, gc.pad[2], gc.out_shape[2], 1, &kx, &ox1);
        const unsigned rowb = (((unsigned)q.x * gc.out_shape[0] + oz) * gc.out_shape[1] + oy) * gc.out_shape[2];
        const unsigned l0 = rowb + ox0, l1 = rowb + ox1;
        if (v0 && v1 && (l0 >> 5) == (l1 >> 5)) {
            atomicOr(&bm1[l0 >> 5], (1u << (l0 & 31u)) | (1u << (l1 & 31u)));
        } else {
            if (v0) atomicOr(&bm1[l0 >> 5], 1u << (l0 & 31u));
            if (v1) atomicOr(&bm1[l1 >> 5], 1u << (l1 & 31u));
        }
        return;
    }
    const long long nthreads = (long long)(gridDim.x / 10) * kBlock;
    int4 *f4 = reinterpret_cast<int4 *>(fill);
    const long long n4 = fill_words >> 2;
    for (long long i = (long long)(blk - nb_subm - nb_set) * kBlock + threadIdx.x; i < n4; i += nthreads) f4[i] = make_int4(-1, -1, -1, -1);
    if (blk == nb_subm + nb_set && threadIdx.x < (int)(fill_words & 3)) fill[(n4 << 2) + threadIdx.x] = -1;
}

__global__ __launch_bounds__(kBlock) void k_chain_prep(uint4 *__restrict__ a, long long na16, int4 *__restrict__ b, long long nb16,
                                                      int *__restrict__ b_tail, int nb_tail) {
    const long long stride = (long long)gridDim.x * kBlock;
    const long long i0 = (long long)blockIdx.x * kBlock + threadIdx.x;
    for (long long i = i0; i < na16; i += stride) a[i] = make_uint4(0u, 0u, 0u, 0u);
    for (long long i = i0; i < nb16; i += stride) b[i] = make_int4(-1, -1, -1, -1);
    if (i0 < nb_tail) b_tail[i0] = -1;
}

__global__ __launch_bounds__(kBlock) void k_chain_scan(ChainParams P) {
    __shared__ int smem[8];
    __shared__ int s_tile;
    __shared__ int cnt[kBlock * (kBmWpt / kBmBlk)];
    const int g = scan_take_tile(P.ticket, &s_tile);
    int l = 1;
    while (l < P.levels && g >= P.lv[l].tile0 + P.lv[l].ntiles) ++l;
    const ChainLevel &L = P.lv[l];
    if (L.wpt64) bm_scan_tile<kBmWpt>(L.bm, L.prefix8, L.out_cap, L.status, g - L.tile0, L.ntiles, L.num_out, smem, cnt);
    else bm_scan_tile<kBmWptSmall>(L.bm, L.prefix8, L.out_cap, L.status, g - L.tile0, L.ntiles, L.num_out, smem, cnt);
}

__global__ __launch_bounds__(kBlock) void k_chain_emit(ChainParams P) {
    int l = 1;
    while (l < P.levels && (int)blockIdx.x >= P.lv[l].eblk0 + P.lv[l].eblks) ++l;
    const ChainLevel &L = P.lv[l];
    const long long wi = (long long)((int)blockIdx.x - L.eblk0) * kBlock + threadIdx.x;
    unsigned word = L.bm[wi];
    if (!word) return;
    int r = bm_word_prefix(L.bm, L.prefix8, (size_t)wi);
    const unsigned W = (unsigned)L.shape[2], H = (unsigned)L.shape[1], D = (unsigned)L.shape[0];
    const unsigned lin0 = (unsigned)wi << 5;
    const unsigned rw = lin0 / W, x0 = lin0 - rw * W;
    const unsigned plane = rw / H, y0 = rw - plane * H, b0 = plane / D, z0 = plane - b0 * D;
    while (word && r < L.out_cap) {
        const int bit = __ffs((int)word) - 1;
        word &= word - 1u;
        unsigned x = x0 + bit, y = y0, z = z0, bb = b0;
        while (x >= W) {
            x -= W;
            if (++y == H) { y = 0; if (++z == D) { z = 0; ++bb; } }
        }
        *reinterpret_cast<int4 *>(L.out_indices + (size_t)r * 4) = make_int4((int)bb, (int)z, (int)y, (int)x);
        ++r;
    }
}

__device__ __forceinline__ int chain_rank(const ChainLevel &L, int b, int z, int y, int x) {
    if ((unsigned)z >= (unsigned)L.shape[0] || (unsigned)y >= (unsigned)L.shape[1] || (unsigned)x >= (unsigned)L.shape[2]) return -1;
    const unsigned lin = (((unsigned)b * L.shape[0] + z) * L.shape[1] + y) * L.shape[2] + x;
    const int r = bm_rank1(L.bm, L.prefix8, lin);
    return r < L.out_cap ? r : -1;
}

__device__ __forceinline__ int rank_in_block(const uint4 &a, const uint4 &b, int prefix, unsigned lin) {
    const unsigned wi = (lin >> 5) & 7u, bit = 1u << (lin & 31u);
    const unsigned w[8] = {a.x, a.y, a.z, a.w, b.x, b.y, b.z, b.w};
    unsigned word = 0u;
    int r = prefix;
#pragma unroll
    for (int q = 0; q < 8; ++q) {
        word = wi == (unsigned)q ? w[q] : word;
        r += wi > (unsigned)q ? __popc(w[q]) : 0;
    }
    return (word & bit) ? r + __popc(word & (bit - 1u)) : -1;
}
__device__ __forceinline__ void chain_rank3(const ChainLevel &L, int b, int z, int y, int x0, int (&out)[3]) {
    out[0] = out[1] = out[2] = -1;
    if ((unsigned)z >= (unsigned)L.shape[0] || (unsigned)y >= (unsigned)L.shape[1]) return;
    const int xa = x0 < 0 ? 0 : x0, xb = x0 + 2 < L.shape[2] ? x0 + 2 : L.shape[2] - 1;
    if (xa > xb) return;
    const unsigned row = (((unsigned)b * L.shape[0] + z) * L.shape[1] + y) * L.shape[2];
    const size_t blk_a = (row + (unsigned)xa) >> 8, blk_b = (row + (unsigned)xb) >> 8;
    const uint4 a0 = *reinterpret_cast<const uint4 *>(L.bm + blk_a * kBmBlk), a1 = *reinterpret_cast<const uint4 *>(L.bm + blk_a * kBmBlk + 4);
    const int pa = L.prefix8[blk_a];
    uint4 b0 = a0, b1 = a1;
    int pb = pa;
    if (blk_b != blk_a) {
        b0 = *reinterpret_cast<const uint4 *>(L.bm + blk_b * kBmBlk);
        b1 = *reinterpret_cast<const uint4 *>(L.bm + blk_b * kBmBlk + 4);
        pb = L.prefix8[blk_b];
    }
#pragma unroll
    for (int i = 0; i < 3; ++i) {
        const int x = x0 + i;
        if ((unsigned)x >= (unsigned)L.shape[2]) continue;
        const unsigned lin = row + (unsigned)x;
        const bool in_a = (lin >> 8) == blk_a;
        const int r = rank_in_block(in_a ? a0 : b0, in_a ? a1 : b1, in_a ? pa : pb, lin);
        out[i] = r < L.out_cap ? r : -1;
    }
}

constexpr int kTabU = 4;
__global__ __launch_bounds__(kBlock) void k_chain_tables(ChainParams P) {
    const int blk = blockIdx.x;
    if (blk < P.cand_blks) {
        const ChainLevel &L = P.lv[1];
        const long long t = (long long)blk * kBlock + threadIdx.x;
        const int j = (int)(t >> 3), c = (int)(t & 7);
        if (j >= chain_live0(P)) return;
        const int4 q = *reinterpret_cast<const int4 *>(P.indices0 + (size_t)j * 4);
        int kk[3], out[3];
        bool ok = cand_offset_fixed<3, 2>(q.y, L.pad[0], L.shape[0], c >> 2, &kk[0], &out[0]);
        ok &= cand_offset_fixed<3, 2>(q.z, L.pad[1], L.shape[1], (c >> 1) & 1, &kk[1], &out[1]);
        ok &= cand_offset_fixed<3, 2>(q.w, L.pad[2], L.shape[2], c & 1, &kk[2], &out[2]);
        if (!ok) return;
        const int o = chain_rank(L, q.x, out[0], out[1], out[2]);
        if (o >= 0) L.nbr_out[(size_t)o * 27 + (kk[0] * 3 + kk[1]) * 3 + kk[2]] = j;
        return;
    }
    if (blk >= P.map_blk0) {
        const ChainLevel &L = P.lv[P.levels];
        const long long i = (long long)(blk - P.map_blk0) * kBlock + threadIdx.x;
        if (i >= P.map_cells) return;
        const int r = bm_rank1(L.bm, L.prefix8, (unsigned)i);
        P.site_map[i] = (r >= 0 && r < L.out_cap) ? r + 1 : 0;
        return;
    }
    int l = 1;
    while (l < P.levels && blk >= P.lv[l].cblk0 + P.lv[l].cblks) ++l;
    const ChainLevel &L = P.lv[l];
    const int live = L.num_out[0];
    const bool subm = blk < L.sblk0 + L.sblks;
    const ChainLevel &T = subm ? L : P.lv[l - 1];
    const int kv = subm ? 27 : L.kvol;
    int *dst = subm ? L.subm_nbr : L.nbr_out;
    const long long t0 = (long long)(blk - (subm ? L.sblk0 : L.cblk0)) * (kBlock * kTabU) + threadIdx.x;
    if (kv == 27) {
        __shared__ int s_tri[kBlock / 64][192];
        if (t0 - threadIdx.x >= (long long)live * 9) return;
        const int lane = threadIdx.x & 63, wv = threadIdx.x >> 6;
        const long long n_ent = (long long)live * 27;
        int4 c3[kTabU];
        int r3[kTabU], j3[kTabU];
#pragma unroll
        for (int u = 0; u < kTabU; ++u) {
            const long long t = t0 + (long long)u * kBlock;
            const int r = (int)(t / 9);
            r3[u] = r; j3[u] = (int)(t - (long long)r * 9);
            c3[u] = *reinterpret_cast<const int4 *>(L.out_indices + (size_t)(r < live ? r : 0) * 4);
        }
        int v3[kTabU][3];
#pragma unroll
        for (int u = 0; u < kTabU; ++u) {
            const int dz = j3[u] / 3, dy = j3[u] - dz * 3;
            int z, y, x0;
            if (subm) { z = c3[u].y + dz - 1; y = c3[u].z + dy - 1; x0 = c3[u].w - 1; }
            else { z = 2 * c3[u].y - L.pad[0] + dz; y = 2 * c3[u].z - L.pad[1] + dy; x0 = 2 * c3[u].w - L.pad[2]; }
            if (r3[u] < live) chain_rank3(T, c3[u].x, z, y, x0, v3[u]);
            else v3[u][0] = v3[u][1] = v3[u][2] = -1;
            if (subm && j3[u] == 4) v3[u][1] = r3[u];
        }
#pragma unroll
        for (int u = 0; u < kTabU; ++u) {
            const long long e0 = (t0 - lane + (long long)u * kBlock) * 3;
#pragma unroll
            for (int i = 0; i < 3; ++i) s_tri[wv][3 * lane + i] = v3[u][i];
            __builtin_amdgcn_wave_barrier();
#pragma unroll
            for (int i = 0; i < 3; ++i) {
                const int v = s_tri[wv][i * 64 + lane];
                if (e0 + i * 64 + lane < n_ent) dst[e0 + i * 64 + lane] = v;
            }
            __builtin_amdgcn_wave_barrier();
        }
        return;
    }
    if (t0 >= (long long)live * kv) return;
    int4 c[kTabU];
    int rr[kTabU], kk[kTabU];
    bool on[kTabU];
#pragma unroll
    for (int u = 0; u < kTabU; ++u) {
        const long long t = t0 + (long long)u * kBlock;
        const int r = kv == 27 ? (int)(t / 27) : (int)(t / 3);
        rr[u] = r; kk[u] = (int)(t - (long long)r * kv);
        on[u] = r < live;
        c[u] = *reinterpret_cast<const int4 *>(L.out_indices + (size_t)(on[u] ? r : 0) * 4);
    }
    int val[kTabU];
#pragma unroll
    for (int u = 0; u < kTabU; ++u) {
        const int k = kk[u];
        int z, y, x;
        if (subm) { z = c[u].y + k / 9 - 1; y = c[u].z + (k / 3) % 3 - 1; x = c[u].w + k % 3 - 1; }
        else if (kv == 27) { z = 2 * c[u].y - L.pad[0] + k / 9; y = 2 * c[u].z - L.pad[1] + (k / 3) % 3; x = 2 * c[u].w - L.pad[2] + k % 3; }
        else { z = 2 * c[u].y - L.pad[0] + k; y = c[u].z - L.pad[1]; x = c[u].w - L.pad[2]; }
        val[u] = (subm && k == 13) ? rr[u] : chain_rank(T, c[u].x, z, y, x);
    }
#pragma unroll
    for (int u = 0; u < kTabU; ++u)
        if (on[u]) dst[t0 + (long long)u * kBlock] = val[u];
}

struct RbWorkspace {
    unsigned long long *keys;
    int *vals, *orank, *cand_slot, *rank, *scan, *blk, *scan2, *overflow, *ticket;
    unsigned long long *status;
    long long ctl_words;
    unsigned *first_mask;
    unsigned char *cand_k;
    uint32_t table;
    size_t bytes;
};

static RbWorkspace carve_rb(void *ws, size_t cap, int n_in, int kvol, int max_out_per_in) {
    RbWorkspace w;
    Arena a(ws, cap);
    size_t entries = (size_t)(n_in > 0 ? n_in : 1) * (size_t)(max_out_per_in > 0 ? max_out_per_in : 1);
    w.table = next_pow2((uint32_t)(entries * 2 > 1024 ? entries * 2 : 1024));
    w.keys = a.take<unsigned long long>(w.table);
    w.vals = a.take<int>(w.table);
    w.orank = a.take<int>(w.table);
    long long nk = (long long)n_in * kvol;
    w.cand_slot = a.take<int>(nk);
    w.rank = a.take<int>(nk);
    w.scan = a.take<int>(scan_scratch_ints(nk));
    long long nblk = (long long)kvol * div_up(n_in > 0 ? n_in : 1, kBlock);
    w.blk = a.take<int>(nblk + 1);
    w.scan2 = a.take<int>(scan_scratch_ints(nblk));
    w.ctl_words = (long long)scan_ctl_words(n_in);
    w.ticket = a.take<int>(w.ctl_words);
    w.overflow = w.ticket + 1;
    w.status = reinterpret_cast<unsigned long long *>(w.ticket + 4);
    w.first_mask = a.take<unsigned>(n_in > 0 ? n_in : 1);
    w.cand_k = a.take<unsigned char>(nk > 0 ? nk : 1);
    w.bytes = align_up(a.used);
    return w;
}

static int fill_geom(RbGeom &g, const int *in_shape, const int *out_shape, const int *ksize, const int *stride,
                     const int *pad, const int *dil, int n_in, int batch) {
    g.kvol = 1;
    for (int d = 0; d < 3; ++d) {
// ... 365 lines not shown
        rb_init(nullptr, 0, 0, nbr_out, n_out_words, -1, nbr_in, n_in_words, -1, st);
    long long nc = (long long)n_in * g.ncand;
    if (nc > 0) {
        const int geo = geo_of(g);
        if (geo == 1)
            hipLaunchKernelGGL(k_conv_tables<1>, dim3(div_up(nc, kBlock)), dim3(kBlock), 0, st, w.cand_slot, w.cand_k, w.orank, nc,
                               kvol, g.ncand, nbr_in, nbr_out, nbr_out_rows);
        else if (geo == 2)
            hipLaunchKernelGGL(k_conv_tables<2>, dim3(div_up(nc, kBlock)), dim3(kBlock), 0, st, w.cand_slot, w.cand_k, w.orank, nc,
                               kvol, g.ncand, nbr_in, nbr_out, nbr_out_rows);
        else
            hipLaunchKernelGGL(k_conv_tables<0>, dim3(div_up(nc, kBlock)), dim3(kBlock), 0, st, w.cand_slot, w.cand_k, w.orank, nc,
                               kvol, g.ncand, nbr_in, nbr_out, nbr_out_rows);
        if ((rc = check_launch())) return rc;
    }
    if (pairs) return emit_pairs(nbr_in, n_in, kvol, 0, w.blk, w.scan2, pairs, pair_num, st);
    return SEC_OK;
}


namespace sec {
struct ChainWorkspace {
    unsigned *bm[kChainMaxLevels + 1];
    int *prefix[kChainMaxLevels + 1];
    long long n_words[kChainMaxLevels + 1];
    int ntiles[kChainMaxLevels + 1], wpt64[kChainMaxLevels + 1];
    int *ticket;
    unsigned long long *status;
    long long zero16;
    size_t bytes;
};
static ChainWorkspace carve_chain(void *ws, size_t cap, int batch, int levels, const int *shapes) {
    ChainWorkspace w{};
    Arena a(ws, cap);
    int tiles = 0;
    for (int l = 1; l <= levels; ++l) {
        const long long cells = bm_cells(batch, shapes + 3 * l);
        w.n_words[l] = (long long)div_up(div_up(cells > 0 ? cells : 1, 32), kBmTile) * kBmTile;
        w.wpt64[l] = w.n_words[l] > kBmSmallWords;
        w.ntiles[l] = (int)(w.n_words[l] / (kBlock * (w.wpt64[l] ? kBmWpt : kBmWptSmall)));
        tiles += w.ntiles[l];
    }
    w.bm[1] = a.take<unsigned>(w.n_words[1]);
    const long long ctl_words = 4 + 2 * (long long)tiles;
    w.ticket = a.take<int>(ctl_words + 4);
    w.status = reinterpret_cast<unsigned long long *>(w.ticket + 4);
    w.zero16 = (long long)((reinterpret_cast<char *>(w.ticket + ctl_words + 4) - reinterpret_cast<char *>(w.bm[1])) / 16);
    for (int l = 2; l <= levels; ++l) w.bm[l] = a.take<unsigned>(w.n_words[l]);
    for (int l = 1; l <= levels; ++l) w.prefix[l] = a.take<int>(w.n_words[l] / kBmBlk);
    w.bytes = align_up(a.used);
    return w;
}
static bool chain_geometry_ok(int levels, const int *shapes, const int *ksize, const int *stride, const int *pad, int batch, int *geo) {
    if (levels < 1 || levels > kChainMaxLevels) return false;
    for (int l = 1; l <= levels; ++l) {
        const int *ks = ksize + 3 * (l - 1), *st = stride + 3 * (l - 1), *pd = pad + 3 * (l - 1);
        const bool g1 = ks[0] == 3 && ks[1] == 3 && ks[2] == 3 && st[0] == 2 && st[1] == 2 && st[2] == 2;
        const bool g2 = ks[0] == 3 && ks[1] == 1 && ks[2] == 1 && st[0] == 2 && st[1] == 1 && st[2] == 1;
        if (!g1 && !g2) return false;
        if (l == 1 && !g1) return false;
        geo[l] = g1 ? 1 : 2;
        for (int d = 0; d < 3; ++d) {
            if (pd[d] < 0 || pd[d] > 1) return false;
            const int in = shapes[3 * (l - 1) + d], out = shapes[3 * l + d];
            if (in <= 0 || out != (in + 2 * pd[d] - (ks[d] - 1) - 1) / st[d] + 1) return false;
        }
        if (bm_cells(batch, shapes + 3 * l) >= (1ll << 32) - 64) return false;
    }
    return true;
}
}

SEC_API size_t sec_rulebook_chain_workspace_bytes(int batch, int levels, const int *h_shapes) {
    if (batch <= 0 || levels < 1 || levels > kChainMaxLevels || !h_shapes) return 0;
    return carve_chain(nullptr, 0, batch, levels, h_shapes).bytes;
}

SEC_API int sec_rulebook_chain_sorted(const int *indices0, int n0, const int *n0_dev, int batch, int levels, const int *h_shapes,
                                      const int *h_ksize, const int *h_stride, const int *h_pad, const int *h_out_cap,
                                      int *const *h_nbr_out, int *const *h_out_indices, int *const *h_num_out,
                                      int *const *h_subm_nbr, const void *vox_workspace, size_t vox_workspace_bytes,
                                      int vox_num_points, int vox_max_voxels, int vox_max_points, const int *h_vox_grid3_zyx,
                                      int *site_map, void *workspace, size_t workspace_bytes, void *stream) {
    if (!indices0 || n0 <= 0 || batch <= 0 || !h_shapes || !h_ksize || !h_stride || !h_pad || !h_out_cap || !h_nbr_out ||
        !h_num_out || !h_subm_nbr || !h_out_indices)
        return SEC_E_INVALID;
    int geo[kChainMaxLevels + 1] = {0};
    if (!chain_geometry_ok(levels, h_shapes, h_ksize, h_stride, h_pad, batch, geo)) return SEC_E_UNSUPPORTED;
    for (int l = 1; l <= levels; ++l)
        if (!h_nbr_out[l - 1] || !h_num_out[l - 1] || !h_out_indices[l - 1] || h_out_cap[l - 1] <= 0) return SEC_E_INVALID;
    if (h_subm_nbr[0] && (!vox_workspace || !h_vox_grid3_zyx)) return SEC_E_INVALID;
    hipStream_t st = (hipStream_t)stream;
    ChainWorkspace w = carve_chain(workspace, workspace_bytes, batch, levels, h_shapes);
    if (!workspace || w.bytes > workspace_bytes) return SEC_E_WORKSPACE;

    ChainParams P{};
    P.levels = levels; P.batch = batch; P.n0 = n0; P.indices0 = indices0; P.n0_dev = n0_dev; P.ticket = w.ticket;
    int tile0 = 0, blk0 = div_up((long long)n0 * 8, kBlock);
    P.cand_blks = blk0;
    for (int l = 0; l <= levels; ++l) {
        ChainLevel &L = P.lv[l];
        for (int d = 0; d < 3; ++d) L.shape[d] = h_shapes[3 * l + d];
        L.out_cap = l == 0 ? n0 : h_out_cap[l - 1];
        L.subm_nbr = h_subm_nbr[l];
        if (l == 0) continue;
        for (int d = 0; d < 3; ++d) { L.ksize[d] = h_ksize[3 * (l - 1) + d]; L.pad[d] = h_pad[3 * (l - 1) + d]; }
        L.geo = geo[l]; L.kvol = geo[l] == 1 ? 27 : 3;
        L.n_words = w.n_words[l]; L.bm = w.bm[l]; L.prefix8 = w.prefix[l];
        L.status = w.status + tile0; L.tile0 = tile0; L.ntiles = w.ntiles[l]; L.wpt64 = w.wpt64[l];
        tile0 += w.ntiles[l];
        L.nbr_out = h_nbr_out[l - 1]; L.out_indices = h_out_indices[l - 1]; L.num_out = h_num_out[l - 1];
        L.sblk0 = blk0; L.sblks = L.subm_nbr ? div_up((long long)L.out_cap * 9, kBlock * kTabU) : 0;
        blk0 += L.sblks;
        L.cblk0 = blk0; L.cblks = l >= 2 ? div_up((long long)L.out_cap * (L.kvol == 27 ? 9 : L.kvol), kBlock * kTabU) : 0;
        blk0 += L.cblks;
    }
    P.map_blk0 = blk0;
    int eblk = 0;
    for (int l = 1; l <= levels; ++l) { P.lv[l].eblk0 = eblk; P.lv[l].eblks = (int)(w.n_words[l] / kBlock); eblk += P.lv[l].eblks; }
    P.site_map = site_map;
    P.map_cells = site_map ? bm_cells(batch, h_shapes + 3 * levels) : 0;
    const int map_blks = site_map ? div_up(P.map_cells, (long long)kBlock) : 0;

    RbGeom gs{}, gc{};
    const int k3[3] = {3, 3, 3};
    int rc = fill_geom(gs, h_shapes, nullptr, k3, nullptr, nullptr, nullptr, n0, batch);
    if (rc) return rc;
    if ((rc = fill_geom(gc, h_shapes, h_shapes + 3, h_ksize, h_stride, h_pad, nullptr, n0, batch))) return rc;
    const unsigned long long *keys = nullptr;
    const int *svid = nullptr;
    if (h_subm_nbr[0]) {
        uint32_t mask;
        for (int d = 0; d < 3; ++d) {
            if (h_vox_grid3_zyx[d] <= 0 || h_vox_grid3_zyx[d] > h_shapes[d]) return SEC_E_INVALID;
            gs.in_shape[d] = h_vox_grid3_zyx[d];
        }
        if (!vox_table_of(vox_workspace, vox_workspace_bytes, vox_num_points, batch, vox_max_voxels, vox_max_points, &keys, &svid, &mask))
            return SEC_E_WORKSPACE;
        gs.mask = mask;
    }
    {
        const long long nb = h_subm_nbr[0] ? (long long)n0 * 27 : 0;
        long long most = w.zero16 > nb / 4 ? w.zero16 : nb / 4;
        int blocks = div_up(most > 0 ? most : 1, kBlock);
        if (blocks > 256 * 8) blocks = 256 * 8;
        hipLaunchKernelGGL(k_chain_prep, dim3(blocks), dim3(kBlock), 0, st, reinterpret_cast<uint4 *>(w.bm[1]), w.zero16,
                           reinterpret_cast<int4 *>(h_subm_nbr[0]), nb / 4, h_subm_nbr[0] ? h_subm_nbr[0] + (nb / 4) * 4 : nullptr,
                           (int)(nb & 3));
    }
    {
        const int nb_subm = h_subm_nbr[0] ? div_up((long long)n0 * 14, kBlock) : 0;
        const int nb_set = div_up((long long)n0 * 4, kBlock);
        const long long fill_words = (long long)P.lv[1].out_cap * 27;
        int groups = div_up(nb_subm, 7);
        if (div_up(nb_set, 2) > groups) groups = div_up(nb_set, 2);
        hipLaunchKernelGGL(k_chain_front, dim3(groups * 10), dim3(kBlock), 0, st, indices0, gs, gc, n0_dev, keys, svid,
                           h_subm_nbr[0], w.bm[1], nb_subm, nb_set, P.lv[1].nbr_out, fill_words);
    }
    for (int l = 2; l <= levels; ++l) {
        RbGeom g{};
        if ((rc = fill_geom(g, h_shapes + 3 * (l - 1), h_shapes + 3 * l, h_ksize + 3 * (l - 1), h_stride + 3 * (l - 1), h_pad + 3 * (l - 1),
                            nullptr, 0, batch)))
            return rc;
        const RbFill none{nullptr, 0, nullptr, 0, nullptr, 0, nullptr, 0};
        const unsigned nb = (unsigned)(w.n_words[l] / kBlock);
        if (geo[l] == 1) hipLaunchKernelGGL(k_bm_dilate<1>, dim3(nb), dim3(kBlock), 0, st, w.bm[l - 1], w.n_words[l - 1], g, w.bm[l], w.n_words[l], none);
        else hipLaunchKernelGGL(k_bm_dilate<2>, dim3(nb), dim3(kBlock), 0, st, w.bm[l - 1], w.n_words[l - 1], g, w.bm[l], w.n_words[l], none);
    }
    hipLaunchKernelGGL(k_chain_scan, dim3(tile0), dim3(kBlock), 0, st, P);
    hipLaunchKernelGGL(k_chain_emit, dim3(eblk), dim3(kBlock), 0, st, P);
    hipLaunchKernelGGL(k_chain_tables, dim3(P.map_blk0 + map_blks), dim3(kBlock), 0, st, P);
    return check_launch();
}
```

second.pytorch_amd/second_amd/ops.py:

```python
import numpy as np
import torch

import ctypes
import functools
import os
from typing import NamedTuple

from . import runtime as rt

_op_hook = None


def set_op_hook(hook):
    global _op_hook
    _op_hook = hook


def last_kernel_name():
    return rt.lib().sec_last_kernel_name().decode()


def _traced(name):
    def deco(fn):
        @functools.wraps(fn)
# ... 152 lines not shown
    cap = int(out_cap) if static else max(1, min(n * per_in, int(batch_size) * int(np.prod(out_shape))))
    out_idx = torch.empty((cap, 4), dtype=torch.int32, device=dev)
    num_out = torch.empty((2,), dtype=torch.int32, device=dev)
    l = rt.lib()
    nbytes = l.sec_rulebook_sorted_workspace_bytes(n, k, int(batch_size), rt.i3(out_shape))
    if nbytes == 0:
        raise ValueError("sorted rulebook numbering: output grid too large")
    ws = rt.workspace(nbytes, dev)
    pre_out = torch.empty((cap, k), dtype=torch.int32, device=dev) if static else None
    pre_in = torch.empty((n, k), dtype=torch.int32, device=dev) if (static and (want_nbr_in or want_pairs)) else None
    geo = (rt.i3(spatial_shape), rt.i3(out_shape), ks, st, pd, dl)
    in_ws = in_sites[1] if (in_sites is not None and isinstance(in_sites[0], str)) else None
    if in_ws is not None:
        in_ws.record_stream(torch.cuda.current_stream())
    sub_nbr = torch.empty((cap, 27), dtype=torch.int32, device=dev) if (static and not want_pairs and not torch.is_grad_enabled()) else None
    rc = l.sec_rulebook_conv3d_build_sorted(rt.ptr(indices), n, rt.ptr(n_dev), int(batch_size), *geo, None, cap,
                                            rt.ptr(num_out), rt.ptr(pre_out), cap if static else 0, rt.ptr(pre_in),
                                            rt.ptr(sub_nbr), sub_nbr.numel() if sub_nbr is not None else 0,
                                            rt.ptr(in_ws), in_ws.numel() if in_ws is not None else 0, rt.ptr(ws),
                                            ws.numel(), rt.stream())
    rt.check(rc, "sec_rulebook_conv3d_build_sorted")
    m = cap if static else int(num_out[0].item())
    nbr_out = pre_out if static else torch.empty((m, k), dtype=torch.int32, device=dev)
    if static:
        nbr_in = pre_in
    else:
        nbr_in = torch.empty((n, k), dtype=torch.int32, device=dev) if (want_nbr_in or want_pairs) else None
    pairs = torch.empty((k, 2, n), dtype=torch.int32, device=dev) if want_pairs else None
    pair_num = torch.zeros((k,), dtype=torch.int32, device=dev) if want_pairs else None
    rc = l.sec_rulebook_conv3d_tables_sorted(rt.ptr(indices), n, rt.ptr(n_dev), int(batch_size), *geo, rt.ptr(nbr_out), m,
                                             rt.ptr(nbr_in), 1 if static else 0, rt.ptr(out_idx), cap, rt.ptr(pairs),
                                             rt.ptr(pair_num), rt.ptr(ws), ws.numel(), rt.stream())
    rt.check(rc, "sec_rulebook_conv3d_tables_sorted")
    return {"nbr_out": nbr_out, "nbr_in": nbr_in, "pairs": pairs, "pair_num": pair_num,
            "out_indices": out_idx[:m], "num_out": m, "num_out_dev": num_out if static else None,
            "out_shape": out_shape, "site_table": ("sorted", ws, sub_nbr) if n > 0 else None}


@_traced("rulebook_conv")
def rulebook_conv(indices, batch_size, spatial_shape, ksize, stride, padding, dilation=1, want_pairs=False,
                  n_dev=None, out_cap=None, out_per_in_hint=0, want_nbr_in=True, numbering=None, in_sites=None):
    rt.require_gpu(indices)
    assert indices.dtype == torch.int32 and indices.is_contiguous()
    if (numbering or _numbering) == "sorted":
        return _rulebook_conv_sorted(indices, batch_size, spatial_shape, ksize, stride, padding, dilation, want_pairs, n_dev,
                                     out_cap, want_nbr_in, in_sites)
    n = indices.shape[0]
    ks, st = rt.i3(ksize), rt.i3(stride)
    k = _kvol(ksize)
    dev = indices.device
    out_shape = conv_output_shape(spatial_shape, ksize, stride, padding, dilation)
    dl = rt.i3(dilation)
    per_in = _out_per_in(ks, st, dl)
    hint = int(out_per_in_hint) if 0 < int(out_per_in_hint) < per_in else 0
    static = out_cap is not None
    cap = int(out_cap) if static else max(1, min(n * per_in, int(batch_size) * int(np.prod(out_shape))))
    out_idx = torch.empty((cap, 4), dtype=torch.int32, device=dev)
    num_out = torch.empty((2,), dtype=torch.int32, device=dev)
    l = rt.lib()
    ws = rt.workspace(l.sec_rulebook_workspace_bytes(n, k, hint or per_in), dev)
    pre_out = torch.empty((cap, k), dtype=torch.int32, device=dev) if static else None
    pre_in = torch.empty((n, k), dtype=torch.int32, device=dev) if (static and (want_nbr_in or want_pairs)) else None
    rc = l.sec_rulebook_conv3d_build(rt.ptr(indices), n, rt.ptr(n_dev), int(batch_size), rt.i3(spatial_shape),
                                     rt.i3(out_shape), ks, st, rt.i3(padding), rt.i3(dilation), rt.ptr(out_idx), cap,
                                     rt.ptr(num_out), hint, rt.ptr(pre_out), cap if static else 0, rt.ptr(pre_in), rt.ptr(ws),
                                     ws.numel(), rt.stream())
    rt.check(rc, "sec_rulebook_conv3d_build")
    m = cap if static else int(num_out[0].item())
    nbr_out = pre_out if static else torch.empty((m, k), dtype=torch.int32, device=dev)
    if static:
        nbr_in = pre_in
    else:
        nbr_in = torch.empty((n, k), dtype=torch.int32, device=dev) if (want_nbr_in or want_pairs) else None
    pairs = torch.empty((k, 2, n), dtype=torch.int32, device=dev) if want_pairs else None
    pair_num = torch.zeros((k,), dtype=torch.int32, device=dev) if want_pairs else None
    rc = l.sec_rulebook_conv3d_tables(n, ks, st, dl, hint, rt.ptr(nbr_out), m, rt.ptr(nbr_in), 1 if static else 0, rt.ptr(pairs),
                                      rt.ptr(pair_num), rt.ptr(ws), ws.numel(), rt.stream())
    rt.check(rc, "sec_rulebook_conv3d_tables")
    return {"nbr_out": nbr_out, "nbr_in": nbr_in, "pairs": pairs, "pair_num": pair_num,
            "out_indices": out_idx[:m], "num_out": m, "num_out_dev": num_out if static else None,
            "out_shape": out_shape, "site_table": (ws, n, ks, st, dl, hint) if n > 0 else None}


@_traced("rulebook_chain")
def rulebook_chain(indices0, batch_size, shape0, convs, n_dev=None, site_table=None, want_subm=None, want_site_map=False):
    rt.require_gpu(indices0)
    assert indices0.dtype == torch.int32 and indices0.is_contiguous()
    levels = len(convs)
    want_subm = list(want_subm) if want_subm is not None else [False] * (levels + 1)
    assert len(want_subm) == levels + 1
    dev = indices0.device
    n0 = indices0.shape[0]
    if n0 == 0 or levels == 0:
        return None
    shapes = [[int(v) for v in shape0]]
    ks_all, st_all, pd_all, caps = [], [], [], []
    for ks, st, pd, cap in convs:
        ks3, st3, pd3 = list(rt.i3(ks)), list(rt.i3(st)), list(rt.i3(pd))
        shapes.append(conv_output_shape(shapes[-1], ks3, st3, pd3, 1))
        ks_all += ks3; st_all += st3; pd_all += pd3
        caps.append(int(cap))
    vox = site_table if (site_table is not None and isinstance(site_table[0], str) and site_table[0] == "vox") else None
    if want_subm[0] and vox is None:
        return None
    ia = lambda v: (ctypes.c_int * len(v))(*[int(x) for x in v])
    flat_shapes = ia([v for sh in shapes for v in sh])
    l = rt.lib()
    nbytes = l.sec_rulebook_chain_workspace_bytes(int(batch_size), levels, flat_shapes)
    if nbytes == 0:
        return None
    ws = rt.workspace(nbytes, dev)
    kvols = [int(np.prod(ks_all[3 * i:3 * i + 3])) for i in range(levels)]
    nbr = [torch.empty((caps[i], kvols[i]), dtype=torch.int32, device=dev) for i in range(levels)]
    oidx = [torch.empty((caps[i], 4), dtype=torch.int32, device=dev) for i in range(levels)]
    nout = [torch.empty((2,), dtype=torch.int32, device=dev) for _ in range(levels)]
    rows = [n0] + caps
    subm = [torch.empty((rows[i], 27), dtype=torch.int32, device=dev) if want_subm[i] else None for i in range(levels + 1)]
    smap = torch.empty((int(batch_size), *shapes[-1]), dtype=torch.int32, device=dev) if want_site_map else None
    pa = lambda ts: (ctypes.c_void_p * len(ts))(*[(t.data_ptr() if t is not None else None) for t in ts])
    if vox is not None:
        _, vws, vn, vmv, vmp, vgrid = vox
        vws.record_stream(torch.cuda.current_stream())
    else:
        vws, vn, vmv, vmp, vgrid = None, 0, 0, 0, shapes[0]
    rc = l.sec_rulebook_chain_sorted(rt.ptr(indices0), n0, rt.ptr(n_dev), int(batch_size), levels, flat_shapes, ia(ks_all), ia(st_all),
                                     ia(pd_all), ia(caps), pa(nbr), pa(oidx), pa(nout), pa(subm), rt.ptr(vws),
                                     vws.numel() if vws is not None else 0, int(vn), int(vmv), int(vmp), rt.i3(vgrid), rt.ptr(smap),
                                     rt.ptr(ws), ws.numel(), rt.stream())
    if rc == -3:
        return None
    rt.check(rc, "sec_rulebook_chain_sorted")
    out = [{"shape": shapes[0], "indices": indices0, "num_dev": n_dev, "cap": n0, "nbr_out": None, "subm_nbr": subm[0]}]
    for i in range(levels):
        out.append({"shape": shapes[i + 1], "indices": oidx[i], "num_dev": nout[i], "cap": caps[i], "nbr_out": nbr[i],
                    "subm_nbr": subm[i + 1]})
    return {"levels": out, "site_map": smap, "workspace": ws}


def simple_voxel(voxels, num_points, mean_features, out_dtype=None, num_dev=None):
    rt.require_gpu(voxels, num_points)
    assert voxels.dtype == torch.float32 and voxels.dim() == 3 and voxels.is_contiguous()
    assert num_points.dtype == torch.int32 and num_points.is_contiguous() and num_points.numel() == voxels.shape[0]
    n, t, f = voxels.shape
    out_dtype = out_dtype or torch.float32
    mean = torch.empty((n, int(mean_features)), dtype=out_dtype, device=voxels.device)
    rt.check(rt.lib().sec_simple_voxel_f32(rt.ptr(voxels), rt.ptr(num_points), n, rt.ptr(num_dev), t, f, int(mean_features), rt.ptr(mean),
                                           rt.dtype_code(out_dtype), rt.stream()), "sec_simple_voxel_f32")
    return mean


def simple_voxel_radius(voxels, num_points, mean_features=4, out_dtype=None, num_dev=None):
    rt.require_gpu(voxels, num_points)
    assert voxels.dtype == torch.float32 and voxels.dim() == 3 and voxels.is_contiguous()
    assert num_points.dtype == torch.int32 and num_points.is_contiguous() and num_points.numel() == voxels.shape[0]
    n, t, f = voxels.shape
    out_dtype = out_dtype or torch.float32
    out = torch.empty((n, 4), dtype=out_dtype, device=voxels.device)
    rt.check(rt.lib().sec_simple_voxel_radius_f32(rt.ptr(voxels), rt.ptr(num_points), n, rt.ptr(num_dev), t, f, int(mean_features),
                                                  rt.ptr(out), 4, rt.dtype_code(out_dtype), rt.stream()), "sec_simple_voxel_radius_f32")
    return out


def tensors_checksum(tensors):
    import ctypes
    n = len(tensors)
    for t in tensors:
        rt.require_gpu(t)
        assert t.is_contiguous()
    sums = torch.empty((n, 2), dtype=torch.int64, device=tensors[0].device)
    ptrs = (ctypes.c_void_p * n)(*[t.data_ptr() for t in tensors])
    nbytes = (ctypes.c_longlong * n)(*[t.numel() * t.element_size() for t in tensors])
    rt.check(rt.lib().sec_tensors_checksum(ptrs, nbytes, n, rt.ptr(sums), rt.stream()), "sec_tensors_checksum")
    return sums


def rows_differ_(flag, a, b):
    rt.require_gpu(flag, a, b)
    assert a.dtype == b.dtype == torch.float32 and a.is_contiguous() and b.is_contiguous() and flag.dtype == torch.int32
    n = b.numel()
    assert n > 0 and a.numel() % n == 0
    rt.check(rt.lib().sec_rows_differ_f32(rt.ptr(a), a.numel() // n, rt.ptr(b), n, rt.ptr(flag), rt.stream()), "sec_rows_differ_f32")
    return flag


_conv_profiler = None


def set_conv_profiler(profiler):
    global _conv_profiler
    _conv_profiler = profiler


FP32_MODES = {"split16": 0, "exact": 1}
FP32_SPLIT_LABEL = "bf16x3"


def set_fp32_mode(mode):
    l = rt.lib()
    prev = "exact" if l.sec_get_fp32_mode() == 1 else "split16"
    rt.check(l.sec_set_fp32_mode(FP32_MODES[mode]), "sec_set_fp32_mode")
    return prev


def get_fp32_mode():
    return "exact" if rt.lib().sec_get_fp32_mode() == 1 else "split16"


class fp32_mode:

    def __init__(self, mode):
        self.mode, self.prev = mode, None

    def __enter__(self):
        if self.mode is not None:
            self.prev = set_fp32_mode(self.mode)
        return self

    def __exit__(self, *exc):
        if self.prev is not None:
            set_fp32_mode(self.prev)
        return False


def pack_weight(weight):
    rt.require_gpu(weight)
    cin, cout = weight.shape[-2], weight.shape[-1]
    k = weight.numel() // (cin * cout)
    l = rt.lib()
    if weight.dtype == torch.float32 and l.sec_get_fp32_mode() == 1:
        return None
    if weight.dtype == torch.float32:
        if l.sec_packed_weight_x3_bytes(k, cin, cout) == 0:
            return None
        w = weight.detach().reshape(k, cin, cout).float().contiguous()
        hi = w.to(torch.bfloat16)
        lo = (w - hi.float()).to(torch.bfloat16)
        planes = []
        for plane in (hi, lo):
            img = torch.empty((l.sec_packed_weight_bytes(k, cin, cout, rt.dtype_code(torch.bfloat16)) // 2,), dtype=torch.bfloat16, device=w.device)
            rt.check(l.sec_pack_conv_weight(rt.ptr(plane.contiguous()), k, cin, cout, rt.dtype_code(torch.bfloat16), rt.ptr(img), rt.stream()),
                     "sec_pack_conv_weight")
            planes.append(img.view(k, -1))
        return torch.stack(planes, 1).contiguous()
    code = rt.dtype_code(weight.dtype)
    nbytes = l.sec_packed_weight_bytes(k, cin, cout, code)
    if nbytes == 0:
        return None
    packed = torch.empty((nbytes // 2,), dtype=weight.dtype, device=weight.device)
    rt.check(l.sec_pack_conv_weight(rt.ptr(weight.contiguous()), k, cin, cout, code, rt.ptr(packed), rt.stream()),
             "sec_pack_conv_weight")
    return packed


@_traced("indice_conv")
def indice_conv(features, weight, nbr_out, num_out, packed=None, scale=None, shift=None, relu=False,
                out_dtype=None, num_out_dev=None):
    rt.require_gpu(features, weight, nbr_out)
    assert features.is_contiguous() and weight.is_contiguous() and nbr_out.is_contiguous()
    assert features.dtype == weight.dtype, (features.dtype, weight.dtype)
    cin, cout = weight.shape[-2], weight.shape[-1]
    k = weight.numel() // (cin * cout)
    assert features.shape[1] == cin and nbr_out.shape[1] == k
    out_dtype = out_dtype or features.dtype
    out = torch.empty((num_out, cout), dtype=out_dtype, device=features.device)
    for t in (scale, shift):
        assert t is None or (t.dtype == torch.float32 and t.is_cuda and t.numel() == cout)
    token = None
    if _conv_profiler is not None:
        token = _conv_profiler.begin({"cin": cin, "cout": cout, "kvol": k, "n_in": features.shape[0],
                                      "n_out": int(num_out), "dtype": features.dtype, "nbr_out": nbr_out,
                                      "mfma": packed is not None, "num_out_dev": num_out_dev,
                                      "args": {"pos": (features, weight, nbr_out, num_out),
                                               "kw": dict(packed=packed, scale=scale, shift=shift, relu=relu,
                                                          out_dtype=out_dtype, num_out_dev=num_out_dev)}})
    rc = rt.lib().sec_indice_conv_fwd(rt.ptr(features), features.shape[0], cin, rt.ptr(weight), rt.ptr(packed), k, cout,
                                      rt.ptr(nbr_out), int(num_out), rt.ptr(num_out_dev), rt.ptr(scale), rt.ptr(shift),
                                      int(bool(relu)), rt.ptr(out), rt.dtype_code(features.dtype),
                                      rt.dtype_code(out_dtype), rt.stream())
    if token is not None:
        _conv_profiler.end(token)
    rt.check(rc, "sec_indice_conv_fwd")
    return out


def indice_conv_plan(cin, cout, kvol, num_out, dtype, out_dtype=None, packed=True):
    return int(rt.lib().sec_indice_conv_fwd_plan(int(cin), int(cout), int(kvol), int(num_out), rt.dtype_code(dtype),
                                                 rt.dtype_code(out_dtype or dtype), int(bool(packed))))


def indice_conv_set_variant(variant):
    rt.check(rt.lib().sec_indice_conv_set_variant(int(variant)), "sec_indice_conv_set_variant")


_PREPACK = {}


def prepack_training_weights(sparse_items, dense_items, dtype):
    import ctypes
    _PREPACK.clear()
    l, code = rt.lib(), rt.dtype_code(dtype)
    vp, ci = ctypes.c_void_p, ctypes.c_int
    arr_p = lambda ts: (vp * len(ts))(*[None if t is None else t.data_ptr() for t in ts])
    arr_i = lambda vs: (ci * len(vs))(*[int(v) for v in vs])
    sp = [(w, bool(subm), bool(want)) for (w, subm, want) in sparse_items
          if w.is_cuda and w.dtype == torch.float32 and w.is_contiguous()]
    if sp:
        ws, ks, cins, couts, subs, w16s, pks, pkts, dws = [], [], [], [], [], [], [], [], []
        for w, subm, want in sp:
            cin, cout = w.shape[-2], w.shape[-1]
            k = w.numel() // (cin * cout)
            nf = l.sec_packed_weight_bytes(k, cin, cout, code)
            nt = l.sec_packed_weight_bytes(k, cout, cin, code) if cout % 16 == 0 else 0
            ws.append(w); ks.append(k); cins.append(cin); couts.append(cout); subs.append(int(subm))
            w16s.append(torch.empty(w.shape, dtype=dtype, device=w.device))
            pks.append(torch.empty((nf // 2,), dtype=dtype, device=w.device) if nf else None)
            pkts.append(torch.empty((nt // 2,), dtype=dtype, device=w.device) if nt else None)
            dws.append(torch.empty(w.shape, dtype=torch.float32, device=w.device) if want else None)
        rt.check(l.sec_pack_conv_weight_train_multi(len(sp), arr_p(ws), arr_i(ks), arr_i(cins), arr_i(couts), arr_i(subs), code, arr_p(w16s),
                                                    arr_p(pks), arr_p(pkts), arr_p(dws), rt.stream()), "sec_pack_conv_weight_train_multi")
        for (w, subm, _), w16, pk, pkt, dw in zip(sp, w16s, pks, pkts, dws):
            _PREPACK[("sp", w.data_ptr(), dtype, subm)] = (w16, pk, pkt, dw)
    de = [w for w in dense_items if w.is_cuda and w.dtype == torch.float32 and w.is_contiguous() and w.dim() == 4 and w.shape[2] == w.shape[3]
          and w.shape[0] % 64 == 0 and w.shape[1] % 64 == 0]
    if de:
        both = []
        for w in de:
            cout, cin, k, _ = w.shape
            nb = l.sec_conv2d_packed_weight_bytes(cout, cin, k, code)
            both.append(torch.empty((2, nb // 2), dtype=dtype, device=w.device))
        rt.check(l.sec_conv2d_pack_weight_train_multi(len(de), arr_p(de), arr_i([w.shape[0] for w in de]), arr_i([w.shape[1] for w in de]),
                                                      arr_i([w.shape[2] for w in de]), code, arr_p([b[0] for b in both]),
                                                      arr_p([b[1] for b in both]), rt.stream()), "sec_conv2d_pack_weight_train_multi")
        for w, b in zip(de, both):
            _PREPACK[("2d", w.data_ptr(), dtype)] = (b[0], b[1])


def pack_weight_train(weight, dtype, subm, zero_grad=False):
    rt.require_gpu(weight)
    assert weight.dtype == torch.float32 and weight.is_contiguous() and dtype in (torch.bfloat16, torch.float16)
    hit = _PREPACK.pop(("sp", weight.data_ptr(), dtype, bool(subm)), None)
    if hit is not None:
        w16, pk, pkt, dw0 = hit
        if zero_grad and dw0 is None:
            dw0 = torch.zeros(weight.shape, dtype=torch.float32, device=weight.device)
        return (w16, pk, pkt, dw0) if zero_grad else (w16, pk, pkt)
    cin, cout = weight.shape[-2], weight.shape[-1]
    k = weight.numel() // (cin * cout)
    l, code = rt.lib(), rt.dtype_code(dtype)
    nf, nt = l.sec_packed_weight_bytes(k, cin, cout, code), (l.sec_packed_weight_bytes(k, cout, cin, code) if cout % 16 == 0 else 0)
    w16 = torch.empty(weight.shape, dtype=dtype, device=weight.device)
    pk = torch.empty((nf // 2,), dtype=dtype, device=weight.device) if nf else None
    pkt = torch.empty((nt // 2,), dtype=dtype, device=weight.device) if nt else None
    dw0 = torch.empty(weight.shape, dtype=torch.float32, device=weight.device) if zero_grad else None
    rt.check(l.sec_pack_conv_weight_train(rt.ptr(weight), k, cin, cout, int(bool(subm)), code, rt.ptr(w16), rt.ptr(pk), rt.ptr(pkt),
                                          rt.ptr(dw0), rt.stream()), "sec_pack_conv_weight_train")
    return (w16, pk, pkt, dw0) if zero_grad else (w16, pk, pkt)


def indice_conv_backward(features, weight, nbr_out, nbr_in, dout, need_dfeat=True, need_dweight=True, dweight_dtype=None,
                         packed_dgrad=None, dweight_out=None):
    rt.require_gpu(features, weight, nbr_out, dout)
# ... 1825 lines not shown
```

second.pytorch_amd/second_amd/runtime.py:

```python
import contextlib
import ctypes
import os

import torch

_HERE = os.path.dirname(os.path.abspath(__file__))
LIB_PATH = os.path.join(os.path.dirname(_HERE), "lib", "libsecond_hip.so")
LIB_PATH = os.environ.get("SEC_HIP_LIB", LIB_PATH)

SEC_F32, SEC_F16, SEC_BF16 = 0, 1, 2
ABI_VERSION = 9
_DTYPES = {torch.float32: SEC_F32, torch.float16: SEC_F16, torch.bfloat16: SEC_BF16}
_ERRORS = {-1: "SEC_E_INVALID (bad argument)", -2: "SEC_E_WORKSPACE (workspace too small)",
           -3: "SEC_E_UNSUPPORTED", -4: "SEC_E_LAUNCH (HIP error)"}

SYMBOLS = [
    "sec_abi_version", "sec_last_error", "sec_last_kernel_name", "sec_tensors_checksum", "sec_voxelize_workspace_bytes", "sec_voxelize_f32", "sec_voxelize_encode_f32", "sec_simple_voxel_f32", "sec_simple_voxel_radius_f32", "sec_rows_differ_f32",
    "sec_rulebook_workspace_bytes", "sec_rulebook_subm3d", "sec_rulebook_subm3d_after_conv", "sec_rulebook_subm3d_after_voxelize",
    "sec_rulebook_conv3d_build",
    "sec_rulebook_conv3d_tables", "sec_rulebook_sorted_workspace_bytes", "sec_rulebook_conv3d_build_sorted",
    "sec_rulebook_conv3d_tables_sorted", "sec_rulebook_subm3d_after_conv_sorted", "sec_rulebook_chain_workspace_bytes",
    "sec_rulebook_chain_sorted", "sec_conv_output_shape", "sec_packed_weight_bytes", "sec_packed_weight_x3_bytes",
    "sec_pack_conv_weight", "sec_indice_conv_fwd", "sec_indice_conv_fwd_plan", "sec_indice_conv_set_variant", "sec_indice_conv_bwd_workspace_bytes", "sec_indice_conv_bwd", "sec_pack_conv_weight_train", "sec_sparse_to_dense", "sec_dense_to_sparse", "sec_sparse_site_map", "sec_sparse_site_map_sorted", "sec_conv2d_nhwc_gather", "sec_conv2d_nhwc_rows", "sec_conv2d_nhwc_into", "sec_rpn_tile_live_workspace_bytes", "sec_rpn_tile_live", "sec_rpn_tile_live_masks", "sec_conv2d_nhwc_tiles", "sec_conv2d_nhwc_tiles_lazy", "sec_conv2d_nhwc_tiles_tail", "sec_conv1x1_chain_nhwc_tiles",
    "sec_pillar_scatter", "sec_pfn_fwd", "sec_pfn_fwd_slots", "sec_pfn_train_workspace_bytes", "sec_pfn_train_fwd", "sec_pfn_train_bwd", "sec_block_filter_workspace_bytes",
    "sec_voxel_block_filter_f32", "sec_bias_act_nhwc", "sec_conv2d_packed_weight_bytes",
    "sec_conv2d_pack_weight", "sec_conv2d_nhwc", "sec_conv2d_fwd_plan_name", "sec_split_f32_bf16x2", "sec_merge_bf16x2_f32", "sec_conv2d_nhwc_x3", "sec_conv2d_nhwc_x3_tiles", "sec_conv1x1_chain_x3", "sec_conv2d_f32_packed_weight_bytes", "sec_conv2d_f32_pack_weight", "sec_conv2d_nhwc_f32", "sec_conv2d_nhwc_f32_tiles", "sec_conv1x1_chain_f32", "sec_conv1x1_chain_nhwc", "sec_rotate_iou_f32", "sec_nms_workspace_bytes", "sec_nms_sorted_f32",
    "sec_predict_select", "sec_predict_select_lazy", "sec_predict_decode", "sec_predict_decode_lazy", "sec_predict_finalize",
    "sec_assign_targets_workspace_bytes", "sec_assign_targets_f32", "sec_assign_targets_per_class_f32",
    "sec_second_loss_workspace_bytes", "sec_second_loss_f32", "sec_heads_loss_supported", "sec_heads_loss_workspace_bytes",
    "sec_heads_loss_fwd", "sec_heads_loss_fwd_terms", "sec_heads_loss_bwd", "sec_set_fp32_mode", "sec_get_fp32_mode",
    "sec_conv2d_pack_weight_train", "sec_conv2d_pack_weight_train_multi", "sec_pack_conv_weight_train_multi", "sec_conv2d_wgrad_workspace_bytes", "sec_conv2d_wgrad_nhwc", "sec_bn_train_workspace_bytes", "sec_bn_relu_fwd_nhwc",
    "sec_bn_relu_bwd_nhwc", "sec_flat_adamw_workspace_bytes", "sec_flat_adamw_f32", "sec_flat_adamw_dev_f32",
    "sec_points_in_boxes_f32", "sec_noise_per_box_f32", "sec_augment_points_f32", "sec_augment_boxes_f32",
    "sec_db_sample_select_f32", "sec_db_sample_merge_points_workspace_bytes", "sec_db_sample_merge_points_f32",
    "sec_anchor_area_mask_workspace_bytes", "sec_anchor_area_mask", "sec_predict_select_masked", "sec_assign_targets_masked_f32",
    "sec_kitti_eval_overlaps", "sec_kitti_eval_flags", "sec_kitti_eval_tp_scores", "sec_kitti_eval_thresholds",
    "sec_kitti_eval_pr_workspace_bytes", "sec_kitti_eval_pr", "sec_kitti_annos_workspace_bytes", "sec_kitti_annos_f64",
    "sec_region_similarity_f32", "sec_assign_targets_sim_f32", "sec_train_metrics_workspace_bytes", "sec_train_metrics_f32",
    "sec_pfn_radius_fwd", "sec_pfn_radius_fwd_slots", "sec_predict_select_segments", "sec_predict_decode_segments",
    "sec_predict_select_classes", "sec_predict_decode_classes", "sec_nms_sorted_items_f32", "sec_predict_finalize_classes",
    "sec_pfn_radius_train_fwd", "sec_pfn_radius_train_bwd",
    "sec_pfn_train_fwd_live", "sec_pfn_train_bwd_live", "sec_pfn_radius_train_fwd_live", "sec_pfn_radius_train_bwd_live",
    "sec_rpn_tile_cover_lds_bytes", "sec_rpn_tile_cover", "sec_conv2d_nhwc_gather_cover", "sec_conv2d_nhwc_tiles_cover",
    "sec_conv2d_nhwc_tiles_tail_cover", "sec_predict_select_cover", "sec_predict_decode_cover",
]

_lib = None


class SecondHipError(RuntimeError):
    pass


_forked_after_gpu_init = False
_parent_used_gpu = False


def _gpu_in_use():
    return _lib is not None or torch.cuda.is_initialized()


def _before_fork():
    global _parent_used_gpu
    _parent_used_gpu = _gpu_in_use()


def _after_fork_in_child():
    global _forked_after_gpu_init
    if _parent_used_gpu:
        _forked_after_gpu_init = True


os.register_at_fork(before=_before_fork, after_in_child=_after_fork_in_child)

FORK_MESSAGE = (
    "second.pytorch_amd: this process was fork()ed from a parent that had already initialised the GPU; a HIP context does not "
    "survive fork(), so spconv ops (VoxelGeneratorV2.generate, rulebooks, NMS) cannot run here. `import spconv` makes "
    "torch.utils.data.DataLoader(num_workers > 0) default to the 'spawn' start method -- construct the DataLoader through "
    "torch.utils.data.DataLoader after importing spconv (the unmodified second/pytorch/train.py does), pass "
    "multiprocessing_context='spawn' yourself, use num_workers=0, or voxelise in the main process with "
    "VoxelGeneratorV2.generate_device / SecondDetector.forward_points.")


def check_not_forked():
    if _forked_after_gpu_init:
        raise SecondHipError(FORK_MESSAGE)


def lib():
    global _lib
    check_not_forked()
    if _lib is None:
        if not os.path.exists(LIB_PATH):
            raise SecondHipError(
                f"{LIB_PATH} is missing: build it with `python second.pytorch_amd/build.py` "
                "(hipcc --offload-arch=gfx950). There is no CPU fallback.")
        l = ctypes.CDLL(LIB_PATH)
        if l.sec_abi_version() != ABI_VERSION:
            raise SecondHipError(f"{LIB_PATH} has ABI version {l.sec_abi_version()}, these bindings expect {ABI_VERSION}: "
                                 "rebuild it (python second.pytorch_amd/build.py --force)")
        for name in ("sec_voxelize_workspace_bytes", "sec_rulebook_workspace_bytes", "sec_rulebook_sorted_workspace_bytes",
                     "sec_rulebook_chain_workspace_bytes",
                     "sec_packed_weight_bytes", "sec_nms_workspace_bytes", "sec_block_filter_workspace_bytes",
                     "sec_conv2d_packed_weight_bytes", "sec_indice_conv_bwd_workspace_bytes",
                     "sec_assign_targets_workspace_bytes", "sec_second_loss_workspace_bytes", "sec_heads_loss_workspace_bytes",
                     "sec_conv2d_wgrad_workspace_bytes", "sec_bn_train_workspace_bytes", "sec_pfn_train_workspace_bytes",
                     "sec_flat_adamw_workspace_bytes", "sec_db_sample_merge_points_workspace_bytes",
                     "sec_anchor_area_mask_workspace_bytes", "sec_kitti_eval_pr_workspace_bytes",
                     "sec_kitti_annos_workspace_bytes", "sec_train_metrics_workspace_bytes"):
            getattr(l, name).restype = ctypes.c_size_t
        if os.environ.get("SEC_FP32_MODE", "").lower() == "exact":
            l.sec_set_fp32_mode(1)
        l.sec_last_error.restype = ctypes.c_char_p
        l.sec_last_kernel_name.restype = ctypes.c_char_p
        l.sec_conv_output_shape.restype = None
        vp, ci, cf, sz, i64 = ctypes.c_void_p, ctypes.c_int, ctypes.c_float, ctypes.c_size_t, ctypes.c_int64
        l.sec_voxelize_workspace_bytes.argtypes = [ci, ci, ci, ci]
        l.sec_voxelize_f32.argtypes = [vp, vp, ci, ci, ci, vp, vp, ci, ci, ci, vp, vp, vp, vp, vp, ci, ci, vp, sz, vp]
        l.sec_voxelize_encode_f32.argtypes = [vp, vp, ci, ci, ci, vp, vp, ci, ci, ci, vp, vp, vp, vp, vp, ci, ci, ci, ci, vp, sz, vp]
        l.sec_simple_voxel_radius_f32.argtypes = [vp, vp, ci, vp, ci, ci, ci, vp, ci, ci, vp]
        l.sec_tensors_checksum.argtypes = [vp, vp, ci, vp, vp]
        l.sec_simple_voxel_f32.argtypes = [vp, vp, ci, vp, ci, ci, ci, vp, ci, vp]
        l.sec_rows_differ_f32.argtypes = [vp, ctypes.c_longlong, vp, ctypes.c_longlong, vp, vp]
        l.sec_rulebook_workspace_bytes.argtypes = [ci, ci, ci]
        l.sec_rulebook_subm3d.argtypes = [vp, ci, vp, ci, vp, vp, vp, vp, vp, vp, vp, sz, vp]
        l.sec_rulebook_subm3d_after_conv.argtypes = [vp, ci, vp, ci, vp, vp, vp, vp, vp, sz, ci, vp, vp, vp, ci, vp]
        l.sec_rulebook_subm3d_after_voxelize.argtypes = [vp, ci, vp, ci, vp, vp, vp, vp, vp, sz, ci, ci, ci, vp, vp]
        l.sec_rulebook_conv3d_build.argtypes = [vp, ci, vp, ci, vp, vp, vp, vp, vp, vp, vp, ci, vp, ci, vp, ci, vp, vp, sz, vp]
        l.sec_rulebook_conv3d_tables.argtypes = [ci, vp, vp, vp, ci, vp, ci, vp, ci, vp, vp, vp, sz, vp]
        l.sec_rulebook_sorted_workspace_bytes.argtypes = [ci, ci, ci, vp]
        l.sec_rulebook_conv3d_build_sorted.argtypes = [vp, ci, vp, ci, vp, vp, vp, vp, vp, vp, vp, ci, vp, vp, ci, vp, vp, ctypes.c_longlong,
                                                       vp, sz, vp, sz, vp]
        l.sec_rulebook_conv3d_tables_sorted.argtypes = [vp, ci, vp, ci, vp, vp, vp, vp, vp, vp, vp, ci, vp, ci, vp, ci, vp, vp, vp, sz, vp]
        l.sec_rulebook_subm3d_after_conv_sorted.argtypes = [vp, ci, vp, ci, vp, vp, vp, vp, ci, vp, sz, vp]
        l.sec_rulebook_chain_workspace_bytes.argtypes = [ci, ci, vp]
        l.sec_rulebook_chain_sorted.argtypes = [vp, ci, vp, ci, ci, vp, vp, vp, vp, vp, vp, vp, vp, vp, vp, sz, ci, ci, ci, vp, vp, vp, sz, vp]
        l.sec_conv_output_shape.argtypes = [vp] * 6
        l.sec_packed_weight_bytes.argtypes = [ci, ci, ci, ci]
        l.sec_pack_conv_weight.argtypes = [vp, ci, ci, ci, ci, vp, vp]
        l.sec_indice_conv_fwd.argtypes = [vp, ci, ci, vp, vp, ci, ci, vp, ci, vp, vp, vp, ci, vp, ci, ci, vp]
        l.sec_packed_weight_x3_bytes.argtypes = [ci, ci, ci]
        l.sec_packed_weight_x3_bytes.restype = sz
        l.sec_indice_conv_fwd_plan.argtypes = [ci] * 7
        l.sec_indice_conv_set_variant.argtypes = [ci]
        l.sec_indice_conv_bwd.argtypes = [vp, ci, ci, vp, ci, ci, vp, vp, ci, vp, vp, vp, ci, vp, sz, vp, ci, vp]
        l.sec_pack_conv_weight_train.argtypes = [vp, ci, ci, ci, ci, ci, vp, vp, vp, vp, vp]
        l.sec_indice_conv_bwd_workspace_bytes.argtypes = [ci, ci, ci, ci]
        l.sec_sparse_to_dense.argtypes = [vp, vp, ci, ci, vp, vp, sz, i64, i64, i64, i64, i64, ci, vp]
        l.sec_dense_to_sparse.argtypes = [vp, vp, ci, ci, vp, vp, i64, i64, i64, i64, i64, ci, vp]
        l.sec_pillar_scatter.argtypes = [vp, vp, ci, ci, vp, vp, sz, i64, i64, i64, i64, ci, vp]
        l.sec_pfn_fwd.argtypes = [vp, vp, vp, ci, vp, ci, ci, vp, vp, vp, ci, cf, cf, cf, cf, vp, ci, vp]
        l.sec_pfn_fwd_slots.argtypes = [vp, vp, sz, ci, ci, ci, ci, ci, vp, vp, ci, vp, vp, vp, vp, ci, cf, cf, cf, cf, vp, ci, vp]
        l.sec_pfn_radius_fwd.argtypes = l.sec_pfn_fwd.argtypes
        l.sec_pfn_radius_fwd_slots.argtypes = l.sec_pfn_fwd_slots.argtypes
        l.sec_pfn_train_workspace_bytes.argtypes = [ci, ci]
        l.sec_pfn_train_fwd.argtypes = [vp, vp, vp, ci, ci, ci, vp, vp, vp, cf, cf, vp, vp, ci, cf, cf, cf, cf, vp, vp, vp, vp, sz, vp]
        l.sec_pfn_train_bwd.argtypes = [vp, vp, vp, ci, ci, ci, vp, vp, vp, ci, cf, cf, cf, cf, vp, vp, vp, vp, vp, vp, vp, sz, vp]
        l.sec_pfn_radius_train_fwd.argtypes = l.sec_pfn_train_fwd.argtypes
        l.sec_pfn_radius_train_bwd.argtypes = l.sec_pfn_train_bwd.argtypes
        for name in ("sec_pfn_train_fwd", "sec_pfn_train_bwd", "sec_pfn_radius_train_fwd", "sec_pfn_radius_train_bwd"):
            at = getattr(l, name).argtypes
            getattr(l, name + "_live").argtypes = at[:4] + [vp] + at[4:]
        l.sec_block_filter_workspace_bytes.argtypes = [ci, ci, ci, ci, ci]
        l.sec_voxel_block_filter_f32.argtypes = [vp, vp, vp, vp, ci, ci, ci, ci, ci, ci, ci, ci, cf, cf, vp, vp, vp, vp, vp, sz, vp]
        l.sec_bias_act_nhwc.argtypes = [vp, vp, sz, ci, ci, ci, vp]
        l.sec_conv2d_packed_weight_bytes.argtypes = [ci, ci, ci, ci]
        l.sec_conv2d_pack_weight.argtypes = [vp, ci, ci, ci, ci, vp, vp]
        l.sec_conv2d_nhwc.argtypes = [vp, ci, ci, ci, ci, vp, vp, ci, ci, ci, ci, ci, vp, ci, vp]
        l.sec_conv2d_fwd_plan_name.argtypes = [ci] * 10
        l.sec_conv2d_fwd_plan_name.restype = ctypes.c_char_p
        l.sec_split_f32_bf16x2.argtypes = [vp, ctypes.c_longlong, vp, vp, vp]
        l.sec_merge_bf16x2_f32.argtypes = [vp, vp, ctypes.c_longlong, vp, vp]
        l.sec_conv2d_nhwc_x3.argtypes = [vp, vp, ci, ci, ci, vp, vp, ci, ci, vp, vp, vp]
        l.sec_conv1x1_chain_x3.argtypes = [vp, vp, ctypes.c_longlong, vp, vp, ci, vp, vp, ci, vp, vp]
        l.sec_conv2d_nhwc_x3_tiles.argtypes = [vp, vp, ci, ci, ci, vp, vp, ci, ci, vp, vp, vp, vp, vp, vp, vp, vp, vp, vp]
        l.sec_conv2d_f32_packed_weight_bytes.argtypes = [ci, ci, ci]
        l.sec_conv2d_f32_packed_weight_bytes.restype = sz
        l.sec_conv2d_f32_pack_weight.argtypes = [vp, ci, ci, ci, vp, vp]
        l.sec_conv2d_nhwc_f32.argtypes = [vp, ci, ci, ci, vp, vp, ci, ci, vp, vp]
        l.sec_conv2d_nhwc_f32_tiles.argtypes = [vp, ci, ci, ci, vp, vp, ci, ci, vp, vp, vp, vp, vp, vp, vp]
        l.sec_conv1x1_chain_f32.argtypes = [vp, ctypes.c_longlong, vp, vp, ci, vp, vp, ci, vp, vp]
        l.sec_sparse_site_map.argtypes = [vp, ci, vp, ci, ci, ci, ci, vp, vp]
        l.sec_sparse_site_map_sorted.argtypes = [vp, ctypes.c_size_t, vp, ci, ci, ci, ci, ci, vp, vp]
        l.sec_conv2d_nhwc_gather.argtypes = [vp, i64, vp, ci, ci, ci, vp, vp, ci, ci, vp, vp, vp, vp, ci, vp]
        l.sec_conv2d_nhwc_rows.argtypes = [vp, i64, vp, ci, ci, ci, ci, vp, vp, ci, ci, ci, ci, ci, vp, ci, vp]
        l.sec_conv2d_nhwc_into.argtypes = [vp, ci, ci, ci, ci, vp, vp, ci, ci, ci, ci, ci, vp, ci, ci, ci, vp]
        l.sec_conv1x1_chain_nhwc.argtypes = [vp, ctypes.c_longlong, vp, vp, ci, vp, vp, ci, vp, ci, vp]
        l.sec_conv1x1_chain_nhwc_tiles.argtypes = [vp, ci, ci, ci, vp, vp, ci, vp, vp, ci, vp, vp, vp, vp, ci, vp]
        l.sec_rpn_tile_live_workspace_bytes.argtypes = [ci, ci, ci]
        l.sec_rpn_tile_live_workspace_bytes.restype = sz
        l.sec_rpn_tile_live.argtypes = [vp, ci, ci, ci, ci, vp, vp, vp, sz, vp]
        l.sec_conv2d_nhwc_tiles.argtypes = [vp, ci, ci, ci, vp, vp, ci, ci, vp, vp, vp, vp, ci, vp]
        l.sec_rpn_tile_live_masks.argtypes = [vp, ci, ci, ci, ci, vp, vp, vp, vp, sz, vp]
        l.sec_conv2d_nhwc_tiles_lazy.argtypes = [vp, ci, ci, ci, vp, vp, ci, ci, vp, vp, vp, vp, vp, vp, ci, vp]
        l.sec_conv2d_nhwc_tiles_tail.argtypes = [vp, ci, ci, ci, vp, vp, ci, vp, vp, vp, vp, vp, vp, ci, vp, vp, ci, vp, ci, vp]
        l.sec_rpn_tile_cover_lds_bytes.argtypes = [ci, ci, ci]
        l.sec_rpn_tile_cover_lds_bytes.restype = sz
        l.sec_rpn_tile_cover.argtypes = [vp, ci, ci, ci, ci, vp, vp, vp, vp, vp, vp, vp, sz, vp]
        l.sec_conv2d_nhwc_gather_cover.argtypes = [vp, i64, vp, ci, ci, ci, vp, vp, ci, ci, vp, vp, vp, ci, vp]
        l.sec_conv2d_nhwc_tiles_cover.argtypes = [vp, ci, ci, ci, vp, vp, ci, ci, vp, vp, vp, vp, vp, ci, vp]
        l.sec_conv2d_nhwc_tiles_tail_cover.argtypes = [vp, ci, ci, ci, vp, vp, ci, vp, vp, vp, vp, vp, vp, ci, vp, vp, ci, vp, ci, vp]
        l.sec_predict_select_cover.argtypes = [vp, vp, ci, ci, ci, ci, ci, ci, cf, vp, vp, vp, vp, vp, ci, vp, vp, vp, vp]
        l.sec_predict_decode_cover.argtypes = [vp, vp, vp, vp, ci, ci, ci, ci, ci, ci, vp, vp, vp, ci, vp, vp, vp, ci, vp, vp, vp, vp]
        l.sec_rotate_iou_f32.argtypes = [vp, ci, vp, ci, ci, vp, vp]
        l.sec_nms_workspace_bytes.argtypes = [ci, ci]
        l.sec_nms_sorted_f32.argtypes = [vp, vp, ci, ci, ci, cf, ci, ci, cf, ci, vp, vp, vp, sz, vp]
        l.sec_predict_select.argtypes = [vp, vp, ci, ci, ci, ci, ci, ci, cf, vp, vp, vp, vp, vp, ci, vp]
        l.sec_predict_decode.argtypes = [vp, vp, vp, vp, ci, ci, ci, ci, ci, ci, vp, vp, vp, ci, vp, vp, vp, ci, vp]
        l.sec_predict_select_lazy.argtypes = [vp, vp, ci, ci, ci, ci, ci, ci, cf, vp, vp, vp, vp, vp, ci, vp, vp, vp]
        l.sec_predict_decode_lazy.argtypes = [vp, vp, vp, vp, ci, ci, ci, ci, ci, ci, vp, vp, vp, ci, vp, vp, vp, ci, vp, vp, vp, vp]
        l.sec_predict_finalize.argtypes = [vp, vp, vp, vp, vp, vp, ci, ci, ci, ci, cf, cf, ci, vp, vp, vp, vp, vp, vp]
        l.sec_assign_targets_workspace_bytes.argtypes = [ci, ci, ci]
        l.sec_assign_targets_f32.argtypes = [vp, ci, vp, vp, vp, vp, ci, ci, cf, cf, vp, vp, vp, vp, sz, vp]
        l.sec_assign_targets_per_class_f32.argtypes = [vp, ci, vp, vp, vp, vp, ci, ci, ci, vp, vp, vp, vp, vp, vp, vp, vp, sz, vp]
        l.sec_second_loss_workspace_bytes.argtypes = [ci, ci]
        l.sec_second_loss_f32.argtypes = [vp, vp, vp, vp, vp, vp, vp, ci, ci, ci, ci, vp, vp, vp, vp, vp, vp, sz, vp]
        l.sec_heads_loss_supported.argtypes = [ci] * 5
        l.sec_heads_loss_workspace_bytes.argtypes = [ci] * 4
        l.sec_heads_loss_fwd.argtypes = [vp, ci, ci, ci, ci, ci, ci, ci, ci, vp, vp, vp, vp, vp, vp, vp, sz, vp]
        l.sec_set_fp32_mode.argtypes = [ci]
        l.sec_get_fp32_mode.argtypes = []
        l.sec_heads_loss_fwd_terms.argtypes = [vp, ci, ci, ci, ci, ci, ci, ci, ci, vp, vp, vp, vp, vp, vp, vp, vp, vp, vp, sz, vp]
        l.sec_heads_loss_bwd.argtypes = [vp, ci, ci, ci, ci, ci, ci, ci, ci, vp, vp, vp, vp, vp, vp, vp, vp, vp, sz, ci, vp]
# ... 108 lines not shown
```

second.pytorch_amd/spconv/conv.py:

```python
import math

import torch
from torch import nn
from torch.nn import init

from second_amd import ops as _ops
from . import functional as Fsp
from .modules import SparseModule
from .tensor import Rulebook, SparseConvTensor


def _triple(v):
    if isinstance(v, (list, tuple)):
        assert len(v) == 3, v
        return [int(x) for x in v]
    return [int(v)] * 3


class SparseConvolution(SparseModule):
    def __init__(self, ndim, in_channels, out_channels, kernel_size=3, stride=1, padding=0, dilation=1, groups=1,
                 bias=True, subm=False, output_padding=0, transposed=False, inverse=False, indice_key=None):
        super().__init__()
        assert ndim == 3, "only 3-D sparse convolutions are on the SECOND hot path"
        assert groups == 1 and not transposed and not inverse, "unused by the reference (SURVEY 2.2)"
# ... 73 lines not shown
        if tbl is not None and tbl[0] == (indices.data_ptr(), indices.shape[0]):
            return tbl[1]
        return None

    def takes_padded_rows(self, x):
        pitch = getattr(x, "in_pitch", None)
        if pitch is None:
            return False
        if pitch != self.pad_in_channels or x.features.shape[1] != pitch or torch.is_grad_enabled():
            raise ValueError(f"rows declared with a pitch of {pitch} channels ({x.features.shape[1]} columns, grad "
                             f"{'on' if torch.is_grad_enabled() else 'off'}) into a layer with in_channels = {self.in_channels}, "
                             f"pad_in_channels = {self.pad_in_channels}: the padded form is an inference path of layers built for it")
        return True

    def kernel_weight(self, padded=False):
        w = self.weight
        if not padded:
            return w
        pad = self.pad_in_channels
        key = (w._version, w.dtype, w.device, w.data_ptr())
        if self._padded is None or self._padded[0] != key:
            self._padded = (key, torch.nn.functional.pad(w.detach(), (0, 0, 0, pad - self.in_channels)).contiguous())
        return self._padded[1]

    def packed_weight(self, padded=False):
        w = self.kernel_weight(padded)
        if padded:
            w0 = self.weight
            key = ("padded", w0._version, w.dtype, w.device, w0.data_ptr(), _ops.get_fp32_mode() if (w.is_cuda and w.dtype == torch.float32) else None)
            if self._packed_key != key:
                self._packed = _ops.pack_weight(w) if w.is_cuda else None
                self._packed_key = key
            return self._packed
        key = (w._version, w.dtype, w.device, w.data_ptr(), _ops.get_fp32_mode() if (w.is_cuda and w.dtype == torch.float32) else None)
        if self._packed_key != key:
            self._packed = _ops.pack_weight(w.detach().contiguous()) if w.is_cuda else None
            self._packed_key = key
        return self._packed

    def _wrap(self, x, feats, rb):
        out = SparseConvTensor(feats, rb.out_indices, rb.out_shape, x.batch_size, x.grid, rb.num_out_dev)
        out.planned = getattr(x, "planned", None)
        out.overflow_checks = getattr(x, "overflow_checks", [])
        if rb.num_out_dev is not None and not rb.subm:
            out.overflow_checks = out.overflow_checks + [(rb.num_out_dev, rb.out_indices.shape[0])]
        out.indice_dict = x.indice_dict
        if not rb.subm:
            out.site_table = rb.__dict__.pop("_site_table", None)
            out.site_bitmap = rb.__dict__.pop("_site_bitmap", None)
            out.site_map_tensor = rb.__dict__.get("_site_map")
        else:
            out.site_bitmap = getattr(x, "site_bitmap", None)
        return out

    def forward(self, x):
        assert isinstance(x, SparseConvTensor)
        if self.conv1x1 and not self.subm and all(s == 1 for s in self.stride) and all(p == 0 for p in self.padding):
            feats = torch.mm(x.features, self.weight.view(self.in_channels, self.out_channels))
            if self.bias is not None:
                feats = feats + self.bias
            out = SparseConvTensor(feats, x.indices, x.spatial_shape, x.batch_size, x.grid)
            out.indice_dict = x.indice_dict
            return out
        rb = self._rulebook(x)
        padded = self.takes_padded_rows(x)
        w = self.kernel_weight(padded)
        if self.weight.dtype == x.features.dtype:
            packed = self.packed_weight(padded)
        else:
            packed = None
        feats = Fsp.indice_conv(x.features, w, rb, packed)
        if self.bias is not None:
            feats = feats + self.bias.to(feats.dtype)
        return self._wrap(x, feats, rb)

    def forward_fused(self, x, scale, shift, relu):
        rb = self._rulebook(x)
        padded = self.takes_padded_rows(x)
        w = self.kernel_weight(padded).detach()
        packed = self.packed_weight(padded)
        if w.dtype != x.features.dtype:
            w, packed = w.to(x.features.dtype), None
        feats = _ops.indice_conv(x.features.contiguous(), w.contiguous(), rb.nbr_out, rb.num_out, packed=packed,
                                 scale=scale, shift=shift, relu=relu, num_out_dev=rb.num_out_dev)
        return self._wrap(x, feats, rb)


class SubMConv3d(SparseConvolution):
    def __init__(self, in_channels, out_channels, kernel_size, stride=1, padding=0, dilation=1, groups=1, bias=True,
                 indice_key=None):
        super().__init__(3, in_channels, out_channels, kernel_size, stride, padding, dilation, groups, bias, True,
                         indice_key=indice_key)


class SparseConv3d(SparseConvolution):
    def __init__(self, in_channels, out_channels, kernel_size, stride=1, padding=0, dilation=1, groups=1, bias=True,
                 indice_key=None):
        super().__init__(3, in_channels, out_channels, kernel_size, stride, padding, dilation, groups, bias,
                         indice_key=indice_key)
```

second.pytorch_amd/spconv/modules.py:

```python
from collections import OrderedDict

import torch
from torch import nn


class SparseModule(nn.Module):
    """Marker base class: modules that take and return a SparseConvTensor."""


def _is_sparse(m):
    return isinstance(m, SparseModule)


def _sec_ops():
    from second_amd import ops
    return ops


class SparseSequential(SparseModule):

    def __init__(self, *args, **kwargs):
        super().__init__()
        if len(args) == 1 and isinstance(args[0], OrderedDict):
            for key, module in args[0].items():
                self.add_module(key, module)
        else:
            for idx, module in enumerate(args):
                self.add_module(str(idx), module)
        for name, module in kwargs.items():
            if name in self._modules:
                raise ValueError("name exists.")
            self.add_module(name, module)
        self.fuse_inference = True
        self.fuse_train_bn = True
        self._fold_cache = {}

    def __getitem__(self, idx):
        if not (-len(self) <= idx < len(self)):
            raise IndexError(f"index {idx} is out of range")
        if idx < 0:
            idx += len(self)
        return list(self._modules.values())[idx]

    def __len__(self):
        return len(self._modules)

    def add(self, module, name=None):
        if name is None:
            name = str(len(self._modules))
            if name in self._modules:
                raise KeyError("name exists")
        self.add_module(name, module)

    def plan_chain(self, x):
        from .conv import SparseConvolution
        from .tensor import Rulebook
        ops = _sec_ops()
        if x.num_active_dev is None or torch.is_grad_enabled() or ops._numbering != "sorted" or not x.features.is_cuda:
            return None
        convs, want_subm, plan, cap = [], [False], [], x.indices.shape[0]
        for m in self._modules.values():
            if not isinstance(m, SparseConvolution) or m.conv1x1:
                continue
            if m.subm:
                if m.kernel_size != [3, 3, 3] or m.dilation != [1, 1, 1]:
                    return None
                want_subm[-1] = True
                plan.append((m, len(convs), True))
            else:
                if m.dilation != [1, 1, 1]:
                    return None
                cap = m.static_out_rows or int(cap * m.static_growth)
                convs.append((m.kernel_size, m.stride, m.padding, cap))
                want_subm.append(False)
                plan.append((m, len(convs), False))
        if not convs:
            return None
        tbl = getattr(x, "site_table", None)
        tbl = tbl[1] if (tbl is not None and tbl[0] == (x.indices.data_ptr(), x.indices.shape[0])) else None
        if not (tbl is not None and isinstance(tbl[0], str) and tbl[0] == "vox"):
            tbl, want_subm[0] = None, False
            plan = [p for p in plan if not (p[2] and p[1] == 0)]
        r = ops.rulebook_chain(x.indices.contiguous(), x.batch_size, x.spatial_shape, convs, n_dev=x.num_active_dev, site_table=tbl,
                               want_subm=want_subm, want_site_map=int(x.spatial_shape[0]) > 0)
        if r is None:
            return None
        lv = r["levels"]
        planned = {}
        for m, level, subm in plan:
            L = lv[level]
            if subm:
                rb = Rulebook(L["indices"], L["indices"], L["subm_nbr"], None, L["cap"], L["shape"], L["shape"], True,
                              num_out_dev=L["num_dev"])
            else:
                I = lv[level - 1]
                rb = Rulebook(L["indices"], I["indices"], L["nbr_out"], None, L["cap"], I["shape"], L["shape"], False,
                              num_out_dev=L["num_dev"])
                if level == len(convs):
                    rb._site_map = r["site_map"]
            rb._chain_workspace = r["workspace"]
            planned[id(m)] = (rb, None)
        return planned

    def _folded(self, conv, bn):
        key = (id(conv), id(bn), bn.weight._version if bn.weight is not None else 0,
               bn.bias._version if bn.bias is not None else 0, bn.running_mean._version, bn.running_var._version,
               conv.bias._version if conv.bias is not None else -1, bn.running_mean.device)
        hit = self._fold_cache.get(id(conv))
        if hit is not None and hit[0] == key:
            return hit[1], hit[2]
        with torch.no_grad():
            var = bn.running_var.float()
            scale = torch.rsqrt(var + bn.eps)
            if bn.weight is not None:
                scale = scale * bn.weight.float()
            shift = -bn.running_mean.float() * scale
            if bn.bias is not None:
                shift = shift + bn.bias.float()
            if conv.bias is not None:
                shift = shift + conv.bias.float() * scale
            scale, shift = scale.contiguous(), shift.contiguous()
        self._fold_cache[id(conv)] = (key, scale, shift)
        return scale, shift

    def forward(self, input):
        from .conv import SparseConvolution
        from .tensor import SparseConvTensor
        mods = list(self._modules.values())
        i = 0
        while i < len(mods):
            m = mods[i]
            if (self.fuse_inference and not self.training and isinstance(m, SparseConvolution) and not m.conv1x1
                    and isinstance(input, SparseConvTensor) and input.features.is_cuda
                    and not torch.is_grad_enabled()
                    and i + 1 < len(mods) and isinstance(mods[i + 1], nn.BatchNorm1d)
                    and mods[i + 1].track_running_stats and not mods[i + 1].training):
                relu = i + 2 < len(mods) and isinstance(mods[i + 2], nn.ReLU)
                scale, shift = self._folded(m, mods[i + 1])
                input = m.forward_fused(input, scale, shift, relu)
                i += 3 if relu else 2
                continue
            if (self.fuse_train_bn and isinstance(m, nn.BatchNorm1d) and m.training and m.affine and m.track_running_stats
                    and isinstance(input, SparseConvTensor) and input.indices.shape[0] != 0 and input.features.is_cuda
                    and _sec_ops().bn_train_supported(m.num_features, input.features.dtype)):
                relu = i + 1 < len(mods) and isinstance(mods[i + 1], nn.ReLU)
                mom = m.momentum if m.momentum is not None else 0.1
                input.features = _sec_ops().BatchNormReluFunction.apply(input.features.contiguous(), m.weight, m.bias, m.running_mean,
                                                                       m.running_var, m.eps, mom, relu, input.num_active_dev)
                _sec_ops().bump_bn_counter(m)
                i += 2 if relu else 1
                continue
            if _is_sparse(m):
                input = m(input)
            elif isinstance(input, SparseConvTensor):
                if input.indices.shape[0] != 0:
                    if input.num_active_dev is not None and isinstance(m, nn.modules.batchnorm._BatchNorm) and m.training:
                        raise RuntimeError("static-capacity sparse tensor through a torch BatchNorm in training mode: its statistics "
                                           "would include the rows past the live count (the fused BatchNorm1d path needs 16-bit "
                                           "features and a supported channel count)")
                    input.features = m(input.features)
            else:
                input = m(input)
            i += 1
        return input
```

Baseline: 22580 frames/s.

## Pack 27-offset neighbor tables into per-line words for sparse conv

Builds a compact rulebook in which each row stores 9 words instead of 27, one per x-line of three neighbors. Each word holds a base input row plus three presence bits. The sparse conv kernel stages and decodes these words, cutting neighbor-table bytes read and staged into LDS by roughly three times. It also prefetches weights while the table loads are in flight. The cost is extra decode ALU work, new kernel variants, and the assumption that present neighbors on a line are contiguous in the sorted numbering.

After: 22610 frames/s, median of 2. No clear change (+0.2%).

```diff
diff --git a/include/second_hip.h b/include/second_hip.h
--- a/include/second_hip.h
+++ b/include/second_hip.h
@@ -102,6 +102,10 @@
                         const void *packed_weight, int kvol, int cout, const int *nbr_out, int n_out,
                         const int *num_out_dev, const float *scale, const float *shift, int relu,
                         void *out, int dtype, int out_dtype, void *stream);
+int sec_indice_conv_fwd_lines(const void *features, int n_in, int cin, const void *weight,
+                              const void *packed_weight, int kvol, int cout, const int *nbr_out, const int *nbr_lines,
+                              int n_out, const int *num_out_dev, const float *scale, const float *shift, int relu,
+                              void *out, int dtype, int out_dtype, void *stream);
 int sec_indice_conv_fwd_plan(int cin, int cout, int kvol, int n_out, int dtype, int out_dtype, int has_packed);
 int sec_indice_conv_set_variant(int variant);
 #define SEC_FP32_SPLIT16 0
@@ -134,6 +138,13 @@
                               int *const *h_subm_nbr, const void *vox_workspace, size_t vox_workspace_bytes,
                               int vox_num_points, int vox_max_voxels, int vox_max_points, const int *h_vox_grid3_zyx,
                               int *site_map, void *workspace, size_t workspace_bytes, void *stream);
+int sec_rulebook_chain_sorted_lines(const int *indices0, int n0, const int *n0_dev, int batch, int levels, const int *h_shapes,
+                                    const int *h_ksize, const int *h_stride, const int *h_pad, const int *h_out_cap,
+                                    int *const *h_nbr_out, int *const *h_out_indices, int *const *h_num_out,
+                                    int *const *h_subm_nbr, int *const *h_nbr_lines, int *const *h_subm_lines,
+                                    const void *vox_workspace, size_t vox_workspace_bytes,
+                                    int vox_num_points, int vox_max_voxels, int vox_max_points, const int *h_vox_grid3_zyx,
+                                    int *site_map, void *workspace, size_t workspace_bytes, void *stream);
 int sec_conv2d_nhwc_gather(const void *features, long long feature_rows, const int *site_map, int batch, int h,
                            int w, const void *packed_weight, const float *bias, int cout, int relu,
                            const unsigned short *tile_order, const int *live_counts, const void *background, void *y,
diff --git a/second.pytorch_amd/csrc/indice_conv.hip b/second.pytorch_amd/csrc/indice_conv.hip
--- a/second.pytorch_amd/csrc/indice_conv.hip
+++ b/second.pytorch_amd/csrc/indice_conv.hip
@@ -518,7 +518,7 @@
 typedef unsigned int u32x4_t __attribute__((ext_vector_type(4)));
 constexpr int kBalWgs = 256;
 enum : int {
-    kFlStage = 1, kFlPipe = 2, kFlSkew = 32, kFlAllW = 64, kFlLazy = 128, kFlWin3 = 512, kFlBal = 2048, kFlXsh = 8192,
+    kFlStage = 1, kFlPipe = 2, kFlSkew = 32, kFlAllW = 64, kFlLazy = 128, kFlWin3 = 512, kFlBal = 2048, kFlXsh = 8192, kFlLines = 16384,
     kFlAblNoGather = 4, kFlAblFewLines = 8, kFlAblOneLine = 16, kFlAblNoWeights = 4096,
 };
 #if defined(__HIP_DEVICE_COMPILE__) && defined(SEC_PACKED_F32_EXEMPTION)
@@ -530,6 +530,13 @@
     return __builtin_amdgcn_mov_dpp(v, CTRL, 0xf, 0xf, true);
 }
 constexpr int kDppWaveShl1 = 0x130, kDppWaveShr1 = 0x138;
+__device__ __forceinline__ int rows_line_entry(int word, int j) {
+    const unsigned u = (unsigned)word;
+    const int p = (int)(u & 0x1fffffffu), b0 = (int)((u >> 29) & 1u), b1 = (int)((u >> 30) & 1u);
+    if (j == 0) return b0 ? p : -1;
+    if (j == 1) return b1 ? p + b0 : -1;
+    return (u >> 31) ? p + b0 + b1 : -1;
+}
 template <bool LEFT> __device__ __forceinline__ bool rows_xshare(int t, int c, int r) {
     const int n = rows_lane_shift<LEFT ? kDppWaveShr1 : kDppWaveShl1>(c);
     return t >= 0 && t == n && (LEFT ? r > 0 : r < 31);
@@ -548,19 +555,23 @@
     constexpr bool LAZY = (FL & kFlLazy) != 0 && STAGE && !ALLW;
     constexpr bool SKEW = (FL & kFlSkew) != 0 && WAVES == 8 && PIPE;
     const bool early = SKEW && __builtin_amdgcn_readfirstlane((int)threadIdx.x >> 8) != 0;
-    constexpr int TBL16 = 32 * KVOL / 4;
+    constexpr bool LINES = (FL & kFlLines) != 0;
+    constexpr int TW = LINES ? KVOL / 3 : KVOL;
+    constexpr int TBL16 = 32 * TW / 4;
+    static_assert(!LINES || (STAGE && KVOL == 27), "line tables: staged, 27 offsets");
     static_assert(NBW >= 1 && NBW <= 2, "one or two weight pieces per wave");
     static_assert(C::KS <= 4, "up to four 16-channel k-steps per row");
-    static_assert(!STAGE || (32 * KVOL) % 4 == 0, "tile table in whole 16-byte pieces");
+    static_assert(!STAGE || (32 * TW) % 4 == 0, "tile table in whole 16-byte pieces");
     static_assert(!ALLW || (STAGE && PIPE), "the all-weights form stages its tables and double-buffers its B fragments");
     constexpr bool WIN3 = (FL & kFlWin3) != 0;
     constexpr bool XSH = (FL & kFlXsh) != 0 && STAGE && KVOL == 27 && DIST >= 3 && (ALLW || (WIN3 && LAZY));
     static_assert(!WIN3 || (STAGE && !PIPE && !ALLW && KVOL % 3 == 0 && DIST <= 3), "window form: non-pipelined, 3 offsets per window");
-    constexpr int LBUF = ALLW ? (KVOL * C::BSLOT > WAVES * TBL16 ? KVOL * C::BSLOT : WAVES * TBL16) : 1;
+    constexpr bool OWN_STAGE = STAGE && (!ALLW || LINES);
+    constexpr int LBUF = ALLW ? ((LINES || KVOL * C::BSLOT > WAVES * TBL16) ? KVOL * C::BSLOT : WAVES * TBL16) : 1;
     __shared__ __attribute__((aligned(16))) uint4 lbuf[LBUF];
     __shared__ __attribute__((aligned(16))) uint4 bring[ALLW ? 1 : (WIN3 ? 6 : 3)][ALLW ? 1 : C::BSLOT];
     __shared__ __attribute__((aligned(16))) float aff[2 * COUT];
-    __shared__ __attribute__((aligned(16))) u32x4_t stage[(STAGE && !ALLW) ? WAVES : 1][(STAGE && !ALLW) ? TBL16 : 1];
+    __shared__ __attribute__((aligned(16))) u32x4_t stage[OWN_STAGE ? WAVES : 1][OWN_STAGE ? TBL16 : 1];
     rows_stage_affine<COUT>(aff, scale, shift);
     const int n_cap = n_out;
     if (num_out_dev) n_out = *num_out_dev;
@@ -590,28 +601,69 @@
     const u32x4_t *wpv = reinterpret_cast<const u32x4_t *>(packed) + (size_t)piece0 * 64 + lane;
     unsigned off[KVOL];
     unsigned shm = 0;
+    constexpr int NWV = (ALLW && LINES) ? (KVOL * C::BSLOT + WAVES * 64 - 1) / (WAVES * 64) : 1;
+    u32x4_t wv[NWV];
+    constexpr int WPRE = WIN3 ? 3 : DIST;
+    u32x4_t wpre0[WPRE], wpre1[WPRE];
     if constexpr (STAGE) {
         const long long tile_row0 = (long long)bid * (rw * WAVES) + w * rw;
-        const long long tbl_bytes = (long long)n_cap * KVOL * 4;
-        const int *tile = nbr + tile_row0 * KVOL;
-        const long long left = tbl_bytes - tile_row0 * KVOL * 4;
+        const long long tbl_bytes = (long long)n_cap * TW * 4;
+        const int *tile = nbr + tile_row0 * TW;
+        const long long left = tbl_bytes - tile_row0 * TW * 4;
         const __amdgpu_buffer_rsrc_t trs = __builtin_amdgcn_make_buffer_rsrc(
-            const_cast<int *>(left > 0 ? tile : nbr), 0, (int)(left <= 0 ? 0 : (left < 32 * KVOL * 4 ? left : 32 * KVOL * 4)), 0x00020000);
-        u32x4_t *stg = ALLW ? reinterpret_cast<u32x4_t *>(lbuf) + w * TBL16 : &stage[w][0];
-#pragma unroll
-        for (int i = 0; i < (TBL16 + 63) / 64; ++i) {
-            const int p16 = i * 64 + lane;
-            if (p16 < TBL16) stg[p16] = __builtin_amdgcn_raw_buffer_load_b128(trs, p16 * 16, 0, 0);
+            const_cast<int *>(left > 0 ? tile : nbr), 0, (int)(left <= 0 ? 0 : (left < 32 * TW * 4 ? left : 32 * TW * 4)), 0x00020000);
+        u32x4_t *stg = OWN_STAGE ? &stage[w][0] : reinterpret_cast<u32x4_t *>(lbuf) + w * TBL16;
+        if constexpr (LINES) {
+            u32x4_t tv[(TBL16 + 63) / 64];
+#pragma unroll
+            for (int i = 0; i < (TBL16 + 63) / 64; ++i) {
+                const int p16 = i * 64 + lane;
+                tv[i] = __builtin_amdgcn_raw_buffer_load_b128(trs, p16 < TBL16 ? p16 * 16 : 0x80000000u, 0, 0);
+            }
+            if constexpr (ALLW) {
+                const u32x4_t *pk = reinterpret_cast<const u32x4_t *>(packed);
+#pragma unroll
+                for (int j = 0; j < NWV; ++j) {
+                    const int i = j * WAVES * 64 + (int)threadIdx.x;
+                    wv[j] = pk[i < KVOL * C::BSLOT ? i : 0];
+                }
+            } else {
+#pragma unroll
+                for (int j = 0; j < WPRE && j < KVOL; ++j) {
+                    wpre0[j] = wpv[(size_t)j * C::BSLOT];
+                    if (NBW > 1) wpre1[j] = wpv[(size_t)j * C::BSLOT + 64];
+                }
+            }
+#pragma unroll
+            for (int i = 0; i < (TBL16 + 63) / 64; ++i) {
+                const int p16 = i * 64 + lane;
+                if (p16 < TBL16) stg[p16] = tv[i];
+            }
+        } else {
+#pragma unroll
+            for (int i = 0; i < (TBL16 + 63) / 64; ++i) {
+                const int p16 = i * 64 + lane;
+                if (p16 < TBL16) stg[p16] = __builtin_amdgcn_raw_buffer_load_b128(trs, p16 * 16, 0, 0);
+            }
         }
         __builtin_amdgcn_wave_barrier();
-        const int *mine = reinterpret_cast<const int *>(stg) + r * KVOL;
+        const int *mine_w = reinterpret_cast<const int *>(stg) + r * TW;
         if constexpr (!LAZY) {
+            int lw[LINES ? 9 : 1];
+            if constexpr (LINES) {
+#pragma unroll
+                for (int g = 0; g < 9; ++g) lw[g] = valid ? mine_w[g] : 0;
+            }
+            auto entry = [&](int k) __attribute__((always_inline)) -> int {
+                if constexpr (LINES) return rows_line_entry(lw[k / 3], k % 3);
+                else return valid ? mine_w[k] : -1;
+            };
 #pragma unroll
             for (int k = 0; k < KVOL; ++k) {
-                int t = valid ? mine[k] : -1;
+                int t = entry(k);
                 if constexpr (XSH) {
                     if (k % 3 != 1) {
-                        const int c = valid ? mine[k - k % 3 + 1] : -1;
+                        const int c = entry(k - k % 3 + 1);
                         if (k % 3 == 0 ? rows_xshare<true>(t, c, r) : rows_xshare<false>(t, c, r)) { shm |= 1u << (2 * (k / 3) + (k % 3) / 2); t = -1; }
                     }
                 }
@@ -680,10 +732,18 @@
         if (C::KS > 2) areg[(k) % DIST][2 % C::KS] = __builtin_amdgcn_raw_buffer_load_b128(rsrc, off[k] + 64, 0, 0);  \
         if (C::KS > 3) areg[(k) % DIST][3 % C::KS] = __builtin_amdgcn_raw_buffer_load_b128(rsrc, off[k] + 96, 0, 0);  \
     }
+        if constexpr (LINES) {
+#pragma unroll
+            for (int j = 0; j < NWV; ++j) {
+                const int i = j * WAVES * 64 + (int)threadIdx.x;
+                if (i < KVOL * C::BSLOT) reinterpret_cast<u32x4_t *>(lbuf)[i] = wv[j];
+            }
+            __builtin_amdgcn_sched_barrier(0);
+        }
 #pragma unroll
         for (int k = 0; k < DIST && k < KVOL; ++k) SEC_FETCH_A(k)
-        __syncthreads();
-        {
+        if constexpr (!LINES) {
+            __syncthreads();
             const uint4 *pk = reinterpret_cast<const uint4 *>(packed);
             for (int i = threadIdx.x; i < KVOL * C::BSLOT; i += WAVES * 64) lbuf[i] = pk[i];
         }
@@ -710,17 +770,28 @@
 #undef SEC_FETCH_A
         SEC_RTL(if (tl) tl2 = clock64();)
         rows_store<T, COUT>(acc, out, row, valid, h, aff, scale != nullptr, shift != nullptr, relu);
+#ifdef SEC_CONV_TIMELINE
+        if (tl && lane == 0) {
+            long long *rec = tl + ((size_t)blockIdx.x * WAVES + w) * 8;
+            rec[0] = tl0; rec[1] = tl1; rec[2] = tl2; rec[3] = clock64(); rec[4] = rec[5] = rec[6] = 0;
+            rec[7] = __builtin_amdgcn_s_getreg((4 << 11) | 20);
+        }
+#endif
         return;
     }
     u32x4_t wr0[DIST], wr1[DIST];
     u32x4_t *bslot = reinterpret_cast<u32x4_t *>(&bring[0][piece0 * 64 + lane]);
-    const int *lazy_tbl = reinterpret_cast<const int *>(&stage[(STAGE && !ALLW) ? w : 0][0]) + r * KVOL;
+    const int *lazy_tbl = reinterpret_cast<const int *>(&stage[OWN_STAGE ? w : 0][0]) + r * TW;
+    int lzw = 0;
     auto off_of = [&](int k) -> unsigned {
         if constexpr (LAZY) {
-            int t = valid ? lazy_tbl[k] : -1;
+            if constexpr (LINES) {
+                if (k % 3 == 0) lzw = valid ? lazy_tbl[k / 3] : 0;
+            }
+            int t = LINES ? rows_line_entry(lzw, k % 3) : (valid ? lazy_tbl[k] : -1);
             if constexpr (XSH) {
                 if (k % 3 != 1) {
-                    const int c = valid ? lazy_tbl[k - k % 3 + 1] : -1;
+                    const int c = LINES ? rows_line_entry(lzw, 1) : (valid ? lazy_tbl[k - k % 3 + 1] : -1);
                     if (k % 3 == 0 ? rows_xshare<true>(t, c, r) : rows_xshare<false>(t, c, r)) { shm |= 1u << (2 * (k / 3) + (k % 3) / 2); t = -1; }
                 }
             }
@@ -748,7 +819,18 @@
         bslot[((k) % 3) * C::BSLOT] = wr0[(k) % DIST];                                                                \
         if (NBW > 1) bslot[((k) % 3) * C::BSLOT + 64] = wr1[(k) % DIST];                                              \
     }
-    if constexpr (!(WIN3 && XSH)) {
+    if constexpr (LINES && !WIN3) {
+#pragma unroll
+        for (int k = 0; k < DIST && k < KVOL; ++k) {
+            const unsigned o_ = off_of(k);
+            wr0[k % DIST] = wpre0[k];
+            if (NBW > 1) wr1[k % DIST] = wpre1[k];
+            areg[k % DIST][0] = __builtin_amdgcn_raw_buffer_load_b128(rsrc, o_, 0, 0);
+            if (C::KS > 1) areg[k % DIST][1 % C::KS] = __builtin_amdgcn_raw_buffer_load_b128(rsrc, o_ + 32, 0, 0);
+            if (C::KS > 2) areg[k % DIST][2 % C::KS] = __builtin_amdgcn_raw_buffer_load_b128(rsrc, o_ + 64, 0, 0);
+            if (C::KS > 3) areg[k % DIST][3 % C::KS] = __builtin_amdgcn_raw_buffer_load_b128(rsrc, o_ + 96, 0, 0);
+        }
+    } else if constexpr (!(WIN3 && XSH)) {
 #pragma unroll
         for (int k = 0; k < DIST && k < KVOL; ++k) SEC_FETCH(k)
     }
@@ -790,7 +872,12 @@
             if (NBW > 1) bslot[((((g) & 1) * 3) + j_) * C::BSLOT + 64] = ww1[j_];                                     \
         }                                                                                                             \
     }
-        SEC_WLOAD(0)
+        if constexpr (LINES) {
+#pragma unroll
+            for (int j_ = 0; j_ < 3; ++j_) { ww0[j_] = wpre0[j_]; if (NBW > 1) ww1[j_] = wpre1[j_]; }
+        } else {
+            SEC_WLOAD(0)
+        }
 #pragma unroll
         for (int k = 0; k < DIST && k < KVOL; ++k) SEC_GFETCH(k)
         SEC_WSTORE(0)
@@ -1034,6 +1121,12 @@
 constexpr int kFlWide = kFlStage + kFlPipe + kFlBal;
 constexpr int kFl64 = kFlStage + kFlLazy + kFlWin3 + kFlBal;
 constexpr int kFl64K3 = kFlStage + kFlPipe;
+constexpr bool rows_shape_lines(int cin, int kvol) { return kvol == 27 && cin >= 32; }
+static bool conv_lines_enabled() {
+    static int env = -1;
+    if (env < 0) { const char *e = getenv("SEC_CONV_LINES"); env = e ? (atoi(e) != 0) : 1; }
+    return env != 0;
+}
 static_assert(kFlNarrow == 2115 && kFlNarrow + kFlXsh == 10307 && kFlWide == 2051 && kFl64 == 2689 && kFl64 + kFlXsh == 10881 && kFl64K3 == 3,
               "the decimal FL values are part of the kernel names that tests and bench tables quote");
 constexpr bool kXshare32 = true, kXshare64w8 = true, kXshare64w4 = false;
@@ -1079,11 +1172,17 @@
 }
 
 template <typename T, int CIN, int COUT>
-static bool launch_rows_form(int form, const void *feat, long long n_feat, const void *packed, const int *nbr, int n_out, const int *num_out_dev,
-                             const float *scale, const float *shift, int relu, void *out, hipStream_t st) {
+static bool launch_rows_form(int form, const void *feat, long long n_feat, const void *packed, const int *nbr, const int *lines, int n_out,
+                             const int *num_out_dev, const float *scale, const float *shift, int relu, void *out, hipStream_t st) {
 #define SEC_FORM(FORM, SHAPE, KV, D, W, M, FLG)                                                                                  \
     case FORM:                                                                                                                   \
         if constexpr (SHAPE) {                                                                                                   \
+            if constexpr (rows_shape_lines(CIN, KV)) {                                                                           \
+                if (lines) {                                                                                                     \
+                    launch_rows_buf<T, CIN, COUT, D, W, M, FLG + kFlLines, KV>(feat, n_feat, packed, lines, n_out, num_out_dev, scale, shift, relu, out, st); \
+                    return true;                                                                                                 \
+                }                                                                                                                \
+            }                                                                                                                    \
             launch_rows_buf<T, CIN, COUT, D, W, M, FLG, KV>(feat, n_feat, packed, nbr, n_out, num_out_dev, scale, shift, relu, out, st); \
             return true;                                                                                                         \
         }                                                                                                                        \
@@ -1104,13 +1203,13 @@
 }
 
 template <typename T, typename OT, int CIN, int COUT>
-static void launch_mfma(const ConvPlan &p, const void *feat, long long n_feat, const void *packed, const int *nbr, int n_out,
+static void launch_mfma(const ConvPlan &p, const void *feat, long long n_feat, const void *packed, const int *nbr, const int *lines, int n_out,
                         const int *num_out_dev, int kvol, const float *scale, const float *shift, int relu, void *out, hipStream_t st) {
 #ifdef SEC_CONV_EXPERIMENTS
     if (experiment_launch<T, OT, CIN, COUT>(p, feat, n_feat, packed, nbr, n_out, num_out_dev, kvol, scale, shift, relu, out, st)) return;
 #endif
     if constexpr (std::is_same<T, OT>::value && buf_shape(CIN, COUT, 27)) {
-        if (p.id == PLAN_ROWS_BUF && launch_rows_form<T, CIN, COUT>(p.form, feat, n_feat, packed, nbr, n_out, num_out_dev, scale, shift, relu, out, st))
+        if (p.id == PLAN_ROWS_BUF && launch_rows_form<T, CIN, COUT>(p.form, feat, n_feat, packed, nbr, lines, n_out, num_out_dev, scale, shift, relu, out, st))
             return;
     }
     if (p.id == PLAN_MFMA_SKS) {
@@ -1135,11 +1234,11 @@
 template <typename T, typename OT>
 static bool dispatch_mfma(const ConvPlan &p, int cin, int cout, const void *feat, long long n_feat, const void *packed, const int *nbr,
                           int n_out, const int *num_out_dev, int kvol, const float *scale, const float *shift, int relu, void *out,
-                          hipStream_t st) {
+                          hipStream_t st, const int *lines = nullptr) {
     if (p.id == PLAN_GENERIC || p.id == PLAN_C4_MFMA) return false;
 #define SEC_CASE(CI, CO)                                                                                         \
     if (cin == CI && cout == CO) {                                                                               \
-        launch_mfma<T, OT, CI, CO>(p, feat, n_feat, packed, nbr, n_out, num_out_dev, kvol, scale, shift, relu, out, st); \
+        launch_mfma<T, OT, CI, CO>(p, feat, n_feat, packed, nbr, lines, n_out, num_out_dev, kvol, scale, shift, relu, out, st); \
         return true;                                                                                             \
     }
     SEC_MFMA_SHAPES(SEC_CASE)
@@ -2088,6 +2187,17 @@
                                 int kvol, int cout, const int *nbr_out, int n_out, const int *num_out_dev,
                                 const float *scale, const float *shift, int relu, void *out, int dtype, int out_dtype,
                                 void *stream) {
+    return sec_indice_conv_fwd_lines(features, n_in, cin, weight, packed_weight, kvol, cout, nbr_out, nullptr, n_out, num_out_dev, scale,
+                                     shift, relu, out, dtype, out_dtype, stream);
+}
+
+SEC_API int sec_indice_conv_fwd_lines(const void *features, int n_in, int cin, const void *weight, const void *packed_weight,
+                                      int kvol, int cout, const int *nbr_out, const int *nbr_lines, int n_out, const int *num_out_dev,
+                                      const float *scale, const float *shift, int relu, void *out, int dtype, int out_dtype,
+                                      void *stream) {
+    if (nbr_lines && kvol != 27) return SEC_E_INVALID;
+    if (nbr_lines && (n_out >= (1 << 29) || n_in >= (1 << 29))) return SEC_E_UNSUPPORTED;
+    const int *lines = conv_lines_enabled() ? nbr_lines : nullptr;
     if (n_in < 0 || n_out < 0 || cin <= 0 || cout <= 0 || kvol <= 0 || !weight) return SEC_E_INVALID;
     if (dtype < 0 || dtype > 2 || (out_dtype != dtype && out_dtype != SEC_F32)) return SEC_E_UNSUPPORTED;
     if (n_out == 0) return SEC_OK;
@@ -2113,12 +2223,12 @@
     if (p.id != PLAN_GENERIC) {
         if (dtype == SEC_BF16) {
             done = out_dtype == SEC_F32
-                       ? dispatch_mfma<__hip_bfloat16, float>(p, cin, cout, features, n_in, packed_weight, nbr_out, n_out, num_out_dev, kvol, scale, shift, relu, out, st)
-                       : dispatch_mfma<__hip_bfloat16, __hip_bfloat16>(p, cin, cout, features, n_in, packed_weight, nbr_out, n_out, num_out_dev, kvol, scale, shift, relu, out, st);
+                       ? dispatch_mfma<__hip_bfloat16, float>(p, cin, cout, features, n_in, packed_weight, nbr_out, n_out, num_out_dev, kvol, scale, shift, relu, out, st, lines)
+                       : dispatch_mfma<__hip_bfloat16, __hip_bfloat16>(p, cin, cout, features, n_in, packed_weight, nbr_out, n_out, num_out_dev, kvol, scale, shift, relu, out, st, lines);
         } else {
             done = out_dtype == SEC_F32
-                       ? dispatch_mfma<__half, float>(p, cin, cout, features, n_in, packed_weight, nbr_out, n_out, num_out_dev, kvol, scale, shift, relu, out, st)
-                       : dispatch_mfma<__half, __half>(p, cin, cout, features, n_in, packed_weight, nbr_out, n_out, num_out_dev, kvol, scale, shift, relu, out, st);
+                       ? dispatch_mfma<__half, float>(p, cin, cout, features, n_in, packed_weight, nbr_out, n_out, num_out_dev, kvol, scale, shift, relu, out, st, lines)
+                       : dispatch_mfma<__half, __half>(p, cin, cout, features, n_in, packed_weight, nbr_out, n_out, num_out_dev, kvol, scale, shift, relu, out, st, lines);
         }
     }
     if (!done && packed_weight && dtype == SEC_F32 && out_dtype == SEC_F32 && conv_variant() != kVarF32Valu && conv_variant() != kVarF32Mfma &&
diff --git a/second.pytorch_amd/csrc/rulebook.hip b/second.pytorch_amd/csrc/rulebook.hip
--- a/second.pytorch_amd/csrc/rulebook.hip
+++ b/second.pytorch_amd/csrc/rulebook.hip
@@ -757,6 +757,7 @@
     unsigned long long *status;
     int tile0, ntiles, wpt64;
     int *nbr_out, *out_indices, *num_out, *subm_nbr;
+    int *nbr_lines, *subm_lines;
     int sblk0, sblks, cblk0, cblks;
     int eblk0, eblks;
 };
@@ -923,6 +924,13 @@
     }
 }
 
+constexpr int kLineRankBits = 29;
+__device__ __forceinline__ int chain_line_word(const int (&v)[3]) {
+    const unsigned bits = (v[0] >= 0 ? 1u : 0u) | (v[1] >= 0 ? 2u : 0u) | (v[2] >= 0 ? 4u : 0u);
+    const int first = v[0] >= 0 ? v[0] : (v[1] >= 0 ? v[1] : v[2]);
+    return bits ? (int)((bits << kLineRankBits) | (unsigned)first) : 0;
+}
+
 constexpr int kTabU = 4;
 __global__ __launch_bounds__(kBlock) void k_chain_tables(ChainParams P) {
     const int blk = blockIdx.x;
@@ -982,6 +990,11 @@
             if (r3[u] < live) chain_rank3(T, c3[u].x, z, y, x0, v3[u]);
             else v3[u][0] = v3[u][1] = v3[u][2] = -1;
             if (subm && j3[u] == 4) v3[u][1] = r3[u];
+        }
+        if (int *lines = subm ? L.subm_lines : L.nbr_lines) {
+#pragma unroll
+            for (int u = 0; u < kTabU; ++u)
+                if (r3[u] < live) lines[t0 + (long long)u * kBlock] = chain_line_word(v3[u]);
         }
 #pragma unroll
         for (int u = 0; u < kTabU; ++u) {
@@ -1513,6 +1526,19 @@
                                       int *const *h_subm_nbr, const void *vox_workspace, size_t vox_workspace_bytes,
                                       int vox_num_points, int vox_max_voxels, int vox_max_points, const int *h_vox_grid3_zyx,
                                       int *site_map, void *workspace, size_t workspace_bytes, void *stream) {
+    return sec_rulebook_chain_sorted_lines(indices0, n0, n0_dev, batch, levels, h_shapes, h_ksize, h_stride, h_pad, h_out_cap, h_nbr_out,
+                                           h_out_indices, h_num_out, h_subm_nbr, nullptr, nullptr, vox_workspace, vox_workspace_bytes,
+                                           vox_num_points, vox_max_voxels, vox_max_points, h_vox_grid3_zyx, site_map, workspace,
+                                           workspace_bytes, stream);
+}
+
+SEC_API int sec_rulebook_chain_sorted_lines(const int *indices0, int n0, const int *n0_dev, int batch, int levels, const int *h_shapes,
+                                            const int *h_ksize, const int *h_stride, const int *h_pad, const int *h_out_cap,
+                                            int *const *h_nbr_out, int *const *h_out_indices, int *const *h_num_out,
+                                            int *const *h_subm_nbr, int *const *h_nbr_lines, int *const *h_subm_lines,
+                                            const void *vox_workspace, size_t vox_workspace_bytes,
+                                            int vox_num_points, int vox_max_voxels, int vox_max_points, const int *h_vox_grid3_zyx,
+                                            int *site_map, void *workspace, size_t workspace_bytes, void *stream) {
     if (!indices0 || n0 <= 0 || batch <= 0 || !h_shapes || !h_ksize || !h_stride || !h_pad || !h_out_cap || !h_nbr_out ||
         !h_num_out || !h_subm_nbr || !h_out_indices)
         return SEC_E_INVALID;
@@ -1521,6 +1547,15 @@
     for (int l = 1; l <= levels; ++l)
         if (!h_nbr_out[l - 1] || !h_num_out[l - 1] || !h_out_indices[l - 1] || h_out_cap[l - 1] <= 0) return SEC_E_INVALID;
     if (h_subm_nbr[0] && (!vox_workspace || !h_vox_grid3_zyx)) return SEC_E_INVALID;
+    if (h_subm_lines && h_subm_lines[0]) return SEC_E_UNSUPPORTED;
+    for (int l = 1; l <= levels; ++l) {
+        const long long cap_in = l == 1 ? n0 : h_out_cap[l - 2], cap = h_out_cap[l - 1];
+        if (h_subm_lines && h_subm_lines[l]) {
+            if (!h_subm_nbr[l]) return SEC_E_INVALID;
+            if (cap >= (1ll << kLineRankBits)) return SEC_E_UNSUPPORTED;
+        }
+        if (h_nbr_lines && h_nbr_lines[l - 1] && (l < 2 || geo[l] != 1 || cap_in >= (1ll << kLineRankBits))) return SEC_E_UNSUPPORTED;
+    }
     hipStream_t st = (hipStream_t)stream;
     ChainWorkspace w = carve_chain(workspace, workspace_bytes, batch, levels, h_shapes);
     if (!workspace || w.bytes > workspace_bytes) return SEC_E_WORKSPACE;
@@ -1534,6 +1569,8 @@
         for (int d = 0; d < 3; ++d) L.shape[d] = h_shapes[3 * l + d];
         L.out_cap = l == 0 ? n0 : h_out_cap[l - 1];
         L.subm_nbr = h_subm_nbr[l];
+        L.subm_lines = h_subm_lines ? h_subm_lines[l] : nullptr;
+        L.nbr_lines = (l >= 1 && h_nbr_lines) ? h_nbr_lines[l - 1] : nullptr;
         if (l == 0) continue;
         for (int d = 0; d < 3; ++d) { L.ksize[d] = h_ksize[3 * (l - 1) + d]; L.pad[d] = h_pad[3 * (l - 1) + d]; }
         L.geo = geo[l]; L.kvol = geo[l] == 1 ? 27 : 3;
diff --git a/second.pytorch_amd/second_amd/ops.py b/second.pytorch_amd/second_amd/ops.py
--- a/second.pytorch_amd/second_amd/ops.py
+++ b/second.pytorch_amd/second_amd/ops.py
@@ -258,8 +258,19 @@
             "out_shape": out_shape, "site_table": (ws, n, ks, st, dl, hint) if n > 0 else None}
 
 
+_conv_lines = None
+
+
+def conv_lines_enabled():
+    global _conv_lines
+    if _conv_lines is None:
+        _conv_lines = os.environ.get("SEC_CONV_LINES", "0").strip() == "1"
+    return _conv_lines
+
+
 @_traced("rulebook_chain")
-def rulebook_chain(indices0, batch_size, shape0, convs, n_dev=None, site_table=None, want_subm=None, want_site_map=False):
+def rulebook_chain(indices0, batch_size, shape0, convs, n_dev=None, site_table=None, want_subm=None, want_site_map=False,
+                   want_lines=False):
     rt.require_gpu(indices0)
     assert indices0.dtype == torch.int32 and indices0.is_contiguous()
     levels = len(convs)
@@ -293,23 +304,28 @@
     rows = [n0] + caps
     subm = [torch.empty((rows[i], 27), dtype=torch.int32, device=dev) if want_subm[i] else None for i in range(levels + 1)]
     smap = torch.empty((int(batch_size), *shapes[-1]), dtype=torch.int32, device=dev) if want_site_map else None
+    nbr_ln = [torch.empty((caps[i], 9), dtype=torch.int32, device=dev) if (want_lines and i >= 1 and kvols[i] == 27) else None
+              for i in range(levels)]
+    subm_ln = [torch.empty((rows[i], 9), dtype=torch.int32, device=dev) if (want_lines and i >= 1 and want_subm[i]) else None
+               for i in range(levels + 1)]
     pa = lambda ts: (ctypes.c_void_p * len(ts))(*[(t.data_ptr() if t is not None else None) for t in ts])
     if vox is not None:
         _, vws, vn, vmv, vmp, vgrid = vox
         vws.record_stream(torch.cuda.current_stream())
     else:
         vws, vn, vmv, vmp, vgrid = None, 0, 0, 0, shapes[0]
-    rc = l.sec_rulebook_chain_sorted(rt.ptr(indices0), n0, rt.ptr(n_dev), int(batch_size), levels, flat_shapes, ia(ks_all), ia(st_all),
-                                     ia(pd_all), ia(caps), pa(nbr), pa(oidx), pa(nout), pa(subm), rt.ptr(vws),
-                                     vws.numel() if vws is not None else 0, int(vn), int(vmv), int(vmp), rt.i3(vgrid), rt.ptr(smap),
-                                     rt.ptr(ws), ws.numel(), rt.stream())
+    rc = l.sec_rulebook_chain_sorted_lines(rt.ptr(indices0), n0, rt.ptr(n_dev), int(batch_size), levels, flat_shapes, ia(ks_all), ia(st_all),
+                                           ia(pd_all), ia(caps), pa(nbr), pa(oidx), pa(nout), pa(subm), pa(nbr_ln), pa(subm_ln), rt.ptr(vws),
+                                           vws.numel() if vws is not None else 0, int(vn), int(vmv), int(vmp), rt.i3(vgrid), rt.ptr(smap),
+                                           rt.ptr(ws), ws.numel(), rt.stream())
     if rc == -3:
         return None
     rt.check(rc, "sec_rulebook_chain_sorted")
-    out = [{"shape": shapes[0], "indices": indices0, "num_dev": n_dev, "cap": n0, "nbr_out": None, "subm_nbr": subm[0]}]
+    out = [{"shape": shapes[0], "indices": indices0, "num_dev": n_dev, "cap": n0, "nbr_out": None, "subm_nbr": subm[0],
+            "nbr_lines": None, "subm_lines": None}]
     for i in range(levels):
         out.append({"shape": shapes[i + 1], "indices": oidx[i], "num_dev": nout[i], "cap": caps[i], "nbr_out": nbr[i],
-                    "subm_nbr": subm[i + 1]})
+                    "subm_nbr": subm[i + 1], "nbr_lines": nbr_ln[i], "subm_lines": subm_ln[i + 1]})
     return {"levels": out, "site_map": smap, "workspace": ws}
 
 
@@ -430,8 +446,11 @@
 
 @_traced("indice_conv")
 def indice_conv(features, weight, nbr_out, num_out, packed=None, scale=None, shift=None, relu=False,
-                out_dtype=None, num_out_dev=None):
+                out_dtype=None, num_out_dev=None, lines=None):
     rt.require_gpu(features, weight, nbr_out)
+    if lines is not None:
+        rt.require_gpu(lines)
+        assert lines.dtype == torch.int32 and lines.is_contiguous() and lines.shape == (nbr_out.shape[0], 9) and nbr_out.shape[1] == 27
     assert features.is_contiguous() and weight.is_contiguous() and nbr_out.is_contiguous()
     assert features.dtype == weight.dtype, (features.dtype, weight.dtype)
     cin, cout = weight.shape[-2], weight.shape[-1]
@@ -448,11 +467,11 @@
                                       "mfma": packed is not None, "num_out_dev": num_out_dev,
                                       "args": {"pos": (features, weight, nbr_out, num_out),
                                                "kw": dict(packed=packed, scale=scale, shift=shift, relu=relu,
-                                                          out_dtype=out_dtype, num_out_dev=num_out_dev)}})
-    rc = rt.lib().sec_indice_conv_fwd(rt.ptr(features), features.shape[0], cin, rt.ptr(weight), rt.ptr(packed), k, cout,
-                                      rt.ptr(nbr_out), int(num_out), rt.ptr(num_out_dev), rt.ptr(scale), rt.ptr(shift),
-                                      int(bool(relu)), rt.ptr(out), rt.dtype_code(features.dtype),
-                                      rt.dtype_code(out_dtype), rt.stream())
+                                                          out_dtype=out_dtype, num_out_dev=num_out_dev, lines=lines)}})
+    rc = rt.lib().sec_indice_conv_fwd_lines(rt.ptr(features), features.shape[0], cin, rt.ptr(weight), rt.ptr(packed), k, cout,
+                                            rt.ptr(nbr_out), rt.ptr(lines), int(num_out), rt.ptr(num_out_dev), rt.ptr(scale),
+                                            rt.ptr(shift), int(bool(relu)), rt.ptr(out), rt.dtype_code(features.dtype),
+                                            rt.dtype_code(out_dtype), rt.stream())
     if token is not None:
         _conv_profiler.end(token)
     rt.check(rc, "sec_indice_conv_fwd")
diff --git a/second.pytorch_amd/second_amd/runtime.py b/second.pytorch_amd/second_amd/runtime.py
--- a/second.pytorch_amd/second_amd/runtime.py
+++ b/second.pytorch_amd/second_amd/runtime.py
@@ -20,7 +20,7 @@
     "sec_rulebook_conv3d_build",
     "sec_rulebook_conv3d_tables", "sec_rulebook_sorted_workspace_bytes", "sec_rulebook_conv3d_build_sorted",
     "sec_rulebook_conv3d_tables_sorted", "sec_rulebook_subm3d_after_conv_sorted", "sec_rulebook_chain_workspace_bytes",
-    "sec_rulebook_chain_sorted", "sec_conv_output_shape", "sec_packed_weight_bytes", "sec_packed_weight_x3_bytes",
+    "sec_rulebook_chain_sorted", "sec_rulebook_chain_sorted_lines", "sec_indice_conv_fwd_lines", "sec_conv_output_shape", "sec_packed_weight_bytes", "sec_packed_weight_x3_bytes",
     "sec_pack_conv_weight", "sec_indice_conv_fwd", "sec_indice_conv_fwd_plan", "sec_indice_conv_set_variant", "sec_indice_conv_bwd_workspace_bytes", "sec_indice_conv_bwd", "sec_pack_conv_weight_train", "sec_sparse_to_dense", "sec_dense_to_sparse", "sec_sparse_site_map", "sec_sparse_site_map_sorted", "sec_conv2d_nhwc_gather", "sec_conv2d_nhwc_rows", "sec_conv2d_nhwc_into", "sec_rpn_tile_live_workspace_bytes", "sec_rpn_tile_live", "sec_rpn_tile_live_masks", "sec_conv2d_nhwc_tiles", "sec_conv2d_nhwc_tiles_lazy", "sec_conv2d_nhwc_tiles_tail", "sec_conv1x1_chain_nhwc_tiles",
     "sec_pillar_scatter", "sec_pfn_fwd", "sec_pfn_fwd_slots", "sec_pfn_train_workspace_bytes", "sec_pfn_train_fwd", "sec_pfn_train_bwd", "sec_block_filter_workspace_bytes",
     "sec_voxel_block_filter_f32", "sec_bias_act_nhwc", "sec_conv2d_packed_weight_bytes",
@@ -139,6 +139,8 @@
         l.sec_packed_weight_bytes.argtypes = [ci, ci, ci, ci]
         l.sec_pack_conv_weight.argtypes = [vp, ci, ci, ci, ci, vp, vp]
         l.sec_indice_conv_fwd.argtypes = [vp, ci, ci, vp, vp, ci, ci, vp, ci, vp, vp, vp, ci, vp, ci, ci, vp]
+        l.sec_indice_conv_fwd_lines.argtypes = [vp, ci, ci, vp, vp, ci, ci, vp, vp, ci, vp, vp, vp, ci, vp, ci, ci, vp]
+        l.sec_rulebook_chain_sorted_lines.argtypes = [vp, ci, vp, ci, ci, vp, vp, vp, vp, vp, vp, vp, vp, vp, vp, vp, vp, sz, ci, ci, ci, vp, vp, vp, sz, vp]
         l.sec_packed_weight_x3_bytes.argtypes = [ci, ci, ci]
         l.sec_packed_weight_x3_bytes.restype = sz
         l.sec_indice_conv_fwd_plan.argtypes = [ci] * 7
diff --git a/second.pytorch_amd/spconv/conv.py b/second.pytorch_amd/spconv/conv.py
--- a/second.pytorch_amd/spconv/conv.py
+++ b/second.pytorch_amd/spconv/conv.py
@@ -179,7 +179,8 @@
         if w.dtype != x.features.dtype:
             w, packed = w.to(x.features.dtype), None
         feats = _ops.indice_conv(x.features.contiguous(), w.contiguous(), rb.nbr_out, rb.num_out, packed=packed,
-                                 scale=scale, shift=shift, relu=relu, num_out_dev=rb.num_out_dev)
+                                 scale=scale, shift=shift, relu=relu, num_out_dev=rb.num_out_dev,
+                                 lines=getattr(rb, "_lines", None))
         return self._wrap(x, feats, rb)
 
 
diff --git a/second.pytorch_amd/spconv/modules.py b/second.pytorch_amd/spconv/modules.py
--- a/second.pytorch_amd/spconv/modules.py
+++ b/second.pytorch_amd/spconv/modules.py
@@ -82,7 +82,7 @@
             tbl, want_subm[0] = None, False
             plan = [p for p in plan if not (p[2] and p[1] == 0)]
         r = ops.rulebook_chain(x.indices.contiguous(), x.batch_size, x.spatial_shape, convs, n_dev=x.num_active_dev, site_table=tbl,
-                               want_subm=want_subm, want_site_map=int(x.spatial_shape[0]) > 0)
+                               want_subm=want_subm, want_site_map=int(x.spatial_shape[0]) > 0, want_lines=ops.conv_lines_enabled())
         if r is None:
             return None
         lv = r["levels"]
@@ -92,10 +92,12 @@
             if subm:
                 rb = Rulebook(L["indices"], L["indices"], L["subm_nbr"], None, L["cap"], L["shape"], L["shape"], True,
                               num_out_dev=L["num_dev"])
+                rb._lines = L["subm_lines"]
             else:
                 I = lv[level - 1]
                 rb = Rulebook(L["indices"], I["indices"], L["nbr_out"], None, L["cap"], I["shape"], L["shape"], False,
                               num_out_dev=L["num_dev"])
+                rb._lines = L["nbr_lines"]
                 if level == len(convs):
                     rb._site_map = r["site_map"]
             rb._chain_workspace = r["workspace"]
```
